# bencebecsy/pta_replicator

Hardware: AMD Instinct MI355X
Metric: realizations/sec, 68 psr x 5000 TOAs GWB+RN+WN (higher is better)
Workload: dtype f64; 1 GPU; BASELINE.json config 3: the 68 pulsars of ng15_dict.json x 5000 synthetic TOAs - HD GWB (gw_log10_A of the dict) + per-pulsar power-law RN (dict values, 30 components) + per-backend EFAC / t2EQUAD / ECORR (dict values), on-chip Philox draws, 1024 realisations per step per GPU; n_toa_total=340000, Nf=3000, npts=600, parallelism=replica-shard x1

## Files before the change

include/pta_replicator_amd.h:

```cpp
#ifndef PTA_REPLICATOR_AMD_H
#define PTA_REPLICATOR_AMD_H

#include <stdint.h>

#ifdef __cplusplus
extern "C" {
#endif

#define PTA_ABI_VERSION 8

#define PTA_OK 0
#define PTA_E_ARG (-1)
#define PTA_E_HIP (-2)
#define PTA_E_NOTPD (-3)

int pta_abi_version(void);
const char *pta_last_error(void);
int pta_device_info(int *cu_count, int *wavefront, char *arch, int arch_len);



int pta_rng_philox_raw(const uint32_t *ctr, const uint32_t *key, int n, uint32_t *out, void *stream);

int pta_rng_fill_normal(uint64_t seed, uint64_t r0, int R, uint32_t stream_id, int npairs, int interleave,
                        double *z0, double *z1, int64_t ld, int rng_fast, void *stream);
int pta_rng_fill_normal_blocks(uint64_t seed, uint64_t r0, int R, uint32_t stream_kind, int n_blocks, const int32_t *blk_n,
                               const int32_t *blk_zoff, int max_n, double *z, int64_t ld, int rng_fast, void *stream);

int pta_rn_basis(const double *t, int N, double t_ref, const double *f, const double *phase, int nmodes,
                 int cos_first, double *Ft, int64_t ldf, void *stream);

int pta_rn_synth(const double *Ft, int64_t ldf, int N, int K, const double *coef, int64_t ld_coef, int R, double *out,
                 int64_t ld_out, int accumulate, void *stream);

int pta_wn(const double *sigma, const double *efac, const double *equad, int N, int tnequad, const double *z1,
           const double *z2, int64_t ld_z, int R, double *out, int64_t ld_out, int accumulate, void *stream);

int pta_quantize_epochs(const double *times_host, int N, double dt, const int64_t *order_host,
                        int32_t *epoch_of_host, int32_t *first_index_host, int *n_epochs);

int pta_dot3_host(const double *x_host, int64_t n, const double *y_host, double *out_host);
int pta_pow_host(const double *x_host, double y, int64_t n, double *out_host);
int pta_legacy_randn(const uint32_t *seeds_host, const int64_t *counts_host, const int64_t *offsets_host, int n_streams,
                     double *out_host, uint32_t *last_key_host, int32_t *last_pos_has_host, double *last_gauss_host, int n_threads);

int pta_ecorr(const int32_t *epoch_of, const double *ecorr_epoch, int N, int E, const double *z, int64_t ld_z, int R,
              double *out, int64_t ld_out, int accumulate, void *stream);


int pta_orf_pair_arguments(const double *locs_host, int P, double *arg_host, uint8_t *same_host);

int pta_orf_hd(const double *locs, int P, double *orf, void *stream);

int pta_orf_basis(const double *locs, const double *zeta_cos, int P, int lmax, double *basis, void *stream);

int pta_orf_combine(const double *basis, const double *clm, int nbasis, int P, double *orf, void *stream);

int pta_potrf_batched(double *A, int n, int B, int32_t *info, void *stream);

#define PTA_POTRF_ZERO_UPPER 1
#define PTA_POTRF_NO_LOOKAHEAD 2
#define PTA_POTRF_NB(k) (((k) & 0xFF) << 8)
#define PTA_POTRF_CHAINS(c) (((c) & 0xF) << 16)
#define PTA_POTRF_VALU 8
#define PTA_POTRF_SUBSTITUTION 4
#define PTA_POTRF_REG_STAGING 32
#define PTA_POTRF_DIAG_AHEAD 128
#define PTA_POTRF_DIAG64 16
#define PTA_POTRF_LOCKSTEP 64
#define PTA_POTRF_EPI1 0x100000
#define PTA_POTRF_LEFT 0x200000
#define PTA_POTRF_LEFT_SPLIT 0x400000
#define PTA_POTRF_SOLVE_ROWS 0x800000
int pta_potrf_batched_ex(double *A, int n, int64_t lda, int64_t strideA, int B, int32_t *info, int flags, void *stream);

int64_t pta_potrf_workspace_doubles(int n, int B, int flags);
int pta_potrf_batched_ws(double *A, int n, int64_t lda, int64_t strideA, int B, int32_t *info, int flags, double *work,
                         int64_t work_doubles, void *stream);

int pta_potrf_warmup(int nchain);

int64_t pta_potrf_ragged_plan_words(int B);
int pta_potrf_ragged_plan(const int32_t *n, const int64_t *off, const int64_t *ld, int B, int flags, int64_t *plan_host,
                          int64_t *work_doubles);
int pta_potrf_ragged(double *A, const int64_t *plan_host, const int64_t *plan_dev, int32_t *info, double *work,
                     int64_t work_doubles, void *stream);



int pta_gwb_twiddle(const double *sqrtC, int Nf, int npts, int i0, double inv_dt, double *T, int64_t ldt, void *stream);

int pta_gwb_idft(const double *w, int64_t ldw, int M, int Nf, const double *T, int64_t ldt, int npts, double *G0,
                 int64_t ldg, int algo, void *stream);

int64_t pta_gwb_twiddle_sym_size(int Nf, int npts, int variant, int64_t *rot_doubles);
int pta_gwb_twiddle_sym(const double *sqrtC, int Nf, int npts, int i0, double inv_dt, double *Tsym, double *rot,
                        int variant, void *stream);
int pta_gwb_idft_rng(uint64_t seed, uint64_t r0, int R, int P, int Nf, const double *Tsym, const double *rot, int npts,
                     double *G0, int64_t ldg, int variant, int rng_fast, void *stream);

int pta_gwb_czt_fits(int Nf, int npts, int i0);
int pta_gwb_czt_setup(const double *sqrtC, int Nf, int npts, int i0, double inv_dt, double *pre, double *FB, double *tw,
                      double *post, void *stream);
int pta_gwb_czt(uint64_t seed, uint64_t r0, const double *w, int64_t ldw, int R, int P, int Nf, int npts, int i0,
                const double *pre, const double *FB, const double *tw, const double *post, double *G0, int64_t ldg,
                int variant, int rng_fast, void *stream);

int pta_gwb_czt_scaled(uint64_t seed, uint64_t r0, const double *w, int64_t ldw, int R, int P, int Nf, int npts, int i0,
                       const double *pre, const double *FB, const double *tw, const double *post, double *G0, int64_t ldg,
                       int variant, int rng_fast, const double *scale, int64_t ld_scale, void *stream);
int pta_gwb_idft_rng_scaled(uint64_t seed, uint64_t r0, int R, int P, int Nf, const double *Tsym, const double *rot, int npts,
                            double *G0, int64_t ldg, int variant, int rng_fast, const double *scale, int64_t ld_scale, void *stream);
int pta_gwb_spectrum_scale(const double *f, const double *hcf0, int Nf, int R, const double *log10_A, const double *gamma, int turnover,
                           double f0, double beta, double power, double *scale, int64_t ld_scale, void *stream);
int pta_gwb_spectrum_scale_user(const int32_t *seg, const double *dx, const double *dxp, const double *hcf0, int Nf, int M, int R,
                                const double *log10_hc, int64_t ld_hc, double *scale, int64_t ld_scale, void *stream);

int pta_gwb_mix(const double *Mchol, int P, const double *G0, int R, int npts, int64_t ldg, double *G, int variant, void *stream);

int pta_gwb_bracket(const double *ut, int npts, const double *toa_s, int N, int32_t *jlo, void *stream);

int pta_gwb_weights(const double *ut, int npts, const double *toa_s, const int32_t *jlo, int N, double *w, void *stream);

int pta_gwb_interp(const double *G, int64_t ldg, int P, int npts, const double *ut, const double *toa_s,
                   const int32_t *psr_of_toa, const int32_t *jlo, int N, int R, double scale, double *out,
                   int64_t ld_out, int accumulate, void *stream);

#define PTA_CGW_NPAR 18
int pta_cgw(const double *mjd, int N, const double *par_host, double *out, int accumulate, void *stream);

#define PTA_CW_NPAR 16
int pta_cw_catalog_workspace(int N, int ncw, int64_t *partial_doubles, int *nchunk);
int pta_cw_catalog(const double *mjd, int N, const double *par, int ncw, int psr_term, int mode, double tref,
                   double *partial_ws, double *out, int accumulate, void *stream);

#define PTA_ENGINE_TILE 256
#define PTA_ENGINE_EPMAX 132
typedef struct {
  int32_t n_toa;
  int32_t n_psr;
  int32_t rn_k;
  int32_t gw_npts;
  int32_t tnequad;
  int32_t n_tiles;
  const int32_t *tile_psr;
  const int32_t *tile_start;
  const int32_t *tile_count;
  const int32_t *tile_ep0;
  const int32_t *tile_epn;
  const int32_t *idx_in_psr;
  const double *Ft;
  int64_t ldf;
  const double *rn_coef;
  const double *gw_G;
  const int32_t *gw_jlo;
  const double *gw_w;
  const double *wn_a;
  const double *wn_b;
  const int32_t *epoch_of;
  const double *ecorr_toa;
  const double *det;
  const double *wn_c;
  int32_t rng_fast;
  int32_t synth_variant;
} pta_engine_plan;

int pta_engine_rn_coef(uint64_t seed, uint64_t r0, int R, int P, int K, const double *amp, double *coef, int rng_fast, void *stream);

int pta_engine_synth(const pta_engine_plan *plan_host, uint64_t seed, uint64_t r0, int R, double *out, int64_t ld_out,
                     void *stream);

typedef struct {
  const double *rn_amp;
  const double *Mchol;
  int32_t gw_nf;
  int32_t gw_i0;
  int32_t use_czt;
  int32_t czt_variant;
  const double *czt_pre, *czt_FB, *czt_tw, *czt_post;
  const double *Tsym, *rot;
  double *ws_coef;
  double *ws_G0;
  double *ws_G;
  int32_t idft_variant;
  int32_t mix_variant;
} pta_engine_tables;

int pta_engine_generate(const pta_engine_plan *plan_host, const pta_engine_tables *tables_host, uint64_t seed, uint64_t r0, int R,
                        double *out, int64_t ld_out, void *stream);

int pta_hyper_uniform(uint64_t seed, uint64_t r0, int R, int n_par, const double *lo, const double *hi, double *out, void *stream);
int pta_hyper_uniform_field(uint64_t seed, uint64_t r0, int R, int n_par, int field, const double *lo, const double *hi, double *out,
                            void *stream);

int pta_engine_rn_coef_hyper(uint64_t seed, uint64_t r0, int R, int P, int K, const double *rn_f, const double *rn_tspan,
                             const double *log10_A, const double *gamma, const double *amp_fixed, double *coef, int rng_fast,
                             void *stream);

typedef struct {
  const double *gw_scale;
  int64_t ld_gw_scale;
  const double *gw_log10_A;
  const double *gw_gamma;
  const double *gw_f;
  const double *gw_hcf0;
  int32_t gw_turnover;
  double gw_f0, gw_beta, gw_power;
  double *ws_scale;
  const double *rn_f;
  const double *rn_tspan;
  const double *rn_log10_A;
  const double *rn_gamma;
} pta_engine_hyper;

int pta_engine_generate_hyper(const pta_engine_plan *plan_host, const pta_engine_tables *tables_host, const pta_engine_hyper *hyper_host,
                              uint64_t seed, uint64_t r0, int R, double *out, int64_t ld_out, void *stream);

int pta_cw_uniform(uint64_t seed, uint64_t r0, int R, int n_par, const double *lo, const double *hi, double *out, void *stream);

#define PTA_CW_ENGINE_NPAR 16
typedef struct {
  int32_t n_psr;
  int32_t mode;
  int32_t psr_term;
  int32_t amp_is_h;
  int32_t has_pdist;
  double tref;
  const double *phat;
  const double *pdist;
  const double *toa_s;
  const double *src;
  int64_t ld_src;
  double *par;
} pta_cw_engine;

int pta_engine_cw_params(const pta_cw_engine *cw_host, int R, void *stream);

int pta_engine_cw_add(const pta_engine_plan *plan_host, const pta_cw_engine *cw_host, int R, double *out, int64_t ld_out, int accumulate,
                      void *stream);

int pta_cw_catalog_uniform(uint64_t seed, uint64_t r0, int R, int S, const double *lo, const double *hi, double *out, void *stream);

#define PTA_CW_CATALOG_NPAR_EVOLVE 16
#define PTA_CW_CATALOG_NPAR_FOLDED 8
typedef struct {
  int32_t n_psr;
  int32_t n_src;
  int32_t mode;
  int32_t psr_term;
  int32_t amp_is_h;
  int32_t has_pdist;
  double tref;
  const double *phat;
  const double *pdist;
  int64_t ld_pdist;
  const double *toa_s;
  const double *src;
  int64_t ld_src;
  const int32_t *count;
  double *par;
} pta_cw_catalog_engine;

int pta_engine_cw_catalog_params(const pta_cw_catalog_engine *cw_host, int R, void *stream);

int pta_engine_cw_catalog_add(const pta_engine_plan *plan_host, const pta_cw_catalog_engine *cw_host, int R, double *out, int64_t ld_out,
                              int accumulate, void *stream);

int pta_td_cov_assemble(const double *Ft, int64_t ldf, int N, int K, const double *phi, const double *sigma2,
                        const int32_t *epoch_of, const double *ecorr2, double *C, int64_t ldc, void *stream);

int pta_td_cov_assemble_all(const double *Ft, int64_t ldf, int K, const double *phi, const double *sigma2,
                            const int32_t *epoch_of, const double *ecorr2, double *Cbase, const int64_t *blk_pos,
                            const int32_t *blk_ld, const int32_t *blk_n, const int32_t *blk_off, int n_blocks, int max_n,
                            void *stream);

int64_t pta_td_cov_walk_items(const int32_t *blk_n_host, int n_blocks, int K, int variant, int32_t *item0_host);
int pta_td_cov_assemble_walk(const double *Ft, int64_t ldf, int K, const double *phi, const double *sigma2,
                             const int32_t *epoch_of, const double *ecorr2, double *Cbase, const int64_t *blk_pos,
                             const int32_t *blk_ld, const int32_t *blk_n, const int32_t *blk_off, int n_blocks,
                             const int32_t *item0, int64_t n_items, const int32_t *epoch_first, int variant, void *stream);

int pta_td_assemble_potrf(const double *Fr, const double *Gr, int kf, const double *sigma2, const int32_t *epoch_of, const double *ecorr2,
                          double *A, int n, int64_t lda, int64_t strideA, int B, int32_t *info, int flags, double *work,
                          int64_t work_doubles, void *stream);

int pta_td_trmm(const double *L, int64_t ldl, int N, const double *z, int64_t ld_z, int R, double *out, int64_t ld_out,
                int accumulate, int algo, void *stream);

#define PTA_TD_STRIP 256
typedef struct {
  const double *Lbase;
  const int64_t *blk_pos;
  const int32_t *blk_ld;
  const int32_t *blk_n;
  const int32_t *blk_off;
  const int32_t *item_blk;
  const int32_t *item_n0;
  int32_t n_blocks;
  int32_t n_items;
  int32_t rows_per_real;
  uint32_t stream_kind;
  int32_t rng_fast;
  int32_t gw_npts;
  const double *gw_G;
  const int32_t *gw_jlo;
  const double *gw_w;
  const double *det;
  const double *z;
  int64_t ld_z;
  const int32_t *blk_zoff;
  const int32_t *item_rows;
} pta_td_plan;

int pta_td_trmm_rng(const pta_td_plan *plan_host, uint64_t seed, uint64_t r0, int M, double *out, int64_t ld_out, void *stream);

int pta_tm_project(const double *Qt, const double *Mt, int64_t ld, int m, const int32_t *psr_off, int P, double *rows, int64_t ld_rows, int R,
                   void *stream);

int pta_os_project(const double *Wt, int64_t ldw, int C, const int32_t *psr_off, int P, const double *rows, int64_t ld_rows, int R, double *Y,
                   int64_t ld_y, void *stream);
int pta_os_pairs(const double *Y, int64_t ld_y, int P, int C, int R, const int32_t *pair_a, const int32_t *pair_b, int n_pairs, const double *wt,
                 int n_orf, double *A2, int64_t ld_a2, const double *den, double *pair_out, int64_t ld_pair, void *stream);

int pta_os_matched_prior(int R, int P, int K_rn, int C, const double *rn_f, const double *rn_tspan, const double *rn_phi, const double *rn_log10_A,
                         const double *rn_gamma, double T, const double *gw_log10_A, const double *gw_gamma, const double *s, double *b,
                         void *stream);
int pta_os_matched_prior_spec(int R, int P, int K_rn, int C, const double *rn_f, const double *rn_tspan, const double *rn_phi,
                              const double *rn_log10_A, const double *rn_gamma, double T, const int32_t *seg, const double *dx, const double *dxp,
                              int M, const double *log10_hc, int64_t ld_hc, const double *s, double *b, void *stream);
int pta_os_matched_solve(const double *A, int P, int K, int C, int R, const double *b, const double *q, int64_t ld_q, int q_block, const double *S,
                         const double *s, double *X, double *Z, void *stream);
int pta_os_matched_pairs(const double *X, const double *Z, int P, int C, int R, const int32_t *pair_a, const int32_t *pair_b, int n_pairs,
                         const double *G, const double *G2, int n_orf, double *A2, int64_t ld_a2, double *sigma, int64_t ld_sigma, double *rho,
                         double *sigma_pair, int64_t ld_pair, void *stream);

int pta_os_pairs_pf(const double *Y, int64_t ld_y, int P, int C, int R, const int32_t *pair_a, const int32_t *pair_b, int n_pairs,
                    const double *G, int n_orf, const double *op, int mode, double *a2, int64_t ld_a2, void *stream);
int pta_os_matched_pairs_pf(const double *X, const double *Z, int P, int C, int R, const int32_t *pair_a, const int32_t *pair_b, int n_pairs,
                            const double *G, const double *G2, int n_orf, int mode, double *a2, int64_t ld_a2, double *sigma,
                            int64_t ld_sigma, double *fisher, int64_t ld_fisher, void *stream);

int pta_lnl_quad(const double *rows, int64_t ld_rows, int R, const int32_t *psr_off, int P, const double *dinv, const int32_t *psr_ep,
                 const int32_t *ep_ptr, const int32_t *ep_idx, const double *ep_g, const double *q, int64_t ld_q, int q_block, int K, int m,
                 const double *Ht, int64_t ldh, double *r0, void *stream);
int pta_lnl_factor(const double *A, int P, int K, int C, int G, const double *b, double *Lt, double *logdet, void *stream);
int pta_lnl_apply(const double *Lt, const double *logdet, const double *b, int P, int K, int C, int G, const double *q, int64_t ld_q, int q_block,
                  int Kt, int R, const double *r0, const double *s, const double *c, double *lnl_pulsar, int64_t ld_g, int64_t ld_a, void *stream);
int pta_lnl_reduce(const double *lnl_pulsar, int64_t ld_g, int64_t ld_a, int P, int G, int R, double *lnl, int64_t ld_lnl, void *stream);

#define PTA_FSTAT_CMAX 4096
#define PTA_FSTAT_PMAX 128
#define PTA_FSTAT_SKY_TILE 64
int pta_fstat_project(const double *Wt, int64_t ldw, int C, const int32_t *psr_off, int P, const double *rows, int64_t ld_rows, int R, double *Q,
                      int64_t ld_q, void *stream);
int pta_fstat_fp(const double *Q, int64_t ld_q, int P, int J, int R, const double *Ginv, double *fp, int64_t ld_fp, void *stream);
int64_t pta_fstat_fe_tiles(int S);
int pta_fstat_fe(const double *Q, int64_t ld_q, int P, int J, int R, const double *phi, int S, const double *Minv, double *fe, int64_t ld_fe,
                 double *fe_max, int64_t ld_max, int32_t *fe_arg, int64_t ld_arg, double *part_val, int32_t *part_arg, void *stream);

int pta_gather_rank0(void *comm, int rank, int world, int dst, const double *local, int64_t total_rows, int64_t n_cols,
                     int64_t ld_local, double *out, int64_t ld_out, void *stream);

int pta_dgemm(int transB, int M, int N, int K, double alpha, const double *A, int64_t lda, int64_t ska,
              const double *B, int64_t ldb, double beta, double *C, int64_t ldc, int lower_only, int batch,
              int64_t strideA, int64_t strideB, int64_t strideC, int algo, void *stream);

int pta_microbench(int kind, int64_t bytes, int iters, int option, double *result_host);

int pta_clock_probe(uint64_t *samples, int max_samples, int us, int period_us, void *stream);

int pta_selftest_mfma_f64(double *max_err_host);

#ifdef __cplusplus
}
#endif
#endif
```

pta_replicator_amd/_lib.py:

```python
import ctypes
import os
from ctypes import POINTER, c_char_p, c_double, c_int, c_int32, c_int64, c_uint32, c_uint64, c_void_p

import torch

_HERE = os.path.dirname(os.path.abspath(__file__))
LIB_PATH = os.environ.get("PTA_REPLICATOR_AMD_LIB") or os.path.join(_HERE, "libpta_replicator_amd.so")


class PtaError(RuntimeError):
    """A call into libpta_replicator_amd.so returned a PTA_E_* code."""


if not os.path.exists(LIB_PATH):
    raise ImportError(
        f"{LIB_PATH} is missing: build the HIP library first (python -m pta_replicator_amd.build, or "
        "__graft_entry__.build()). pta_replicator_amd has no CPU fallback.")

lib = ctypes.CDLL(LIB_PATH)

_P = c_void_p


class EnginePlan(ctypes.Structure):
    _fields_ = [
        ("n_toa", c_int32), ("n_psr", c_int32), ("rn_k", c_int32), ("gw_npts", c_int32), ("tnequad", c_int32),
        ("n_tiles", c_int32),
        ("tile_psr", _P), ("tile_start", _P), ("tile_count", _P), ("tile_ep0", _P), ("tile_epn", _P),
        ("idx_in_psr", _P), ("Ft", _P), ("ldf", c_int64), ("rn_coef", _P), ("gw_G", _P),
        ("gw_jlo", _P), ("gw_w", _P), ("wn_a", _P), ("wn_b", _P), ("epoch_of", _P),
        ("ecorr_toa", _P), ("det", _P), ("wn_c", _P), ("rng_fast", c_int32), ("synth_variant", c_int32),
    ]


class EngineTables(ctypes.Structure):
    _fields_ = [
        ("rn_amp", _P), ("Mchol", _P), ("gw_nf", c_int32), ("gw_i0", c_int32), ("use_czt", c_int32), ("czt_variant", c_int32),
        ("czt_pre", _P), ("czt_FB", _P), ("czt_tw", _P), ("czt_post", _P), ("Tsym", _P), ("rot", _P),
        ("ws_coef", _P), ("ws_G0", _P), ("ws_G", _P), ("idft_variant", c_int32), ("mix_variant", c_int32),
    ]


class TdPlan(ctypes.Structure):
    _fields_ = [
        ("Lbase", _P), ("blk_pos", _P), ("blk_ld", _P), ("blk_n", _P), ("blk_off", _P), ("item_blk", _P), ("item_n0", _P),
        ("n_blocks", c_int32), ("n_items", c_int32), ("rows_per_real", c_int32), ("stream_kind", c_uint32),
        ("rng_fast", c_int32), ("gw_npts", c_int32),
        ("gw_G", _P), ("gw_jlo", _P), ("gw_w", _P), ("det", _P), ("z", _P), ("ld_z", c_int64), ("blk_zoff", _P), ("item_rows", _P),
    ]


class EngineHyper(ctypes.Structure):
    _fields_ = [
        ("gw_scale", _P), ("ld_gw_scale", c_int64), ("gw_log10_A", _P), ("gw_gamma", _P), ("gw_f", _P), ("gw_hcf0", _P),
        ("gw_turnover", c_int32), ("gw_f0", c_double), ("gw_beta", c_double), ("gw_power", c_double), ("ws_scale", _P),
        ("rn_f", _P), ("rn_tspan", _P), ("rn_log10_A", _P), ("rn_gamma", _P),
    ]


class CwEngine(ctypes.Structure):
    _fields_ = [
        ("n_psr", c_int32), ("mode", c_int32), ("psr_term", c_int32), ("amp_is_h", c_int32), ("has_pdist", c_int32), ("tref", c_double),
        ("phat", _P), ("pdist", _P), ("toa_s", _P), ("src", _P), ("ld_src", c_int64), ("par", _P),
    ]


class CwCatalogEngine(ctypes.Structure):
    _fields_ = [
        ("n_psr", c_int32), ("n_src", c_int32), ("mode", c_int32), ("psr_term", c_int32), ("amp_is_h", c_int32), ("has_pdist", c_int32),
        ("tref", c_double), ("phat", _P), ("pdist", _P), ("ld_pdist", c_int64), ("toa_s", _P), ("src", _P), ("ld_src", c_int64),
        ("count", _P), ("par", _P),
    ]


_SIGNATURES = {
    "pta_abi_version": (c_int, []),
    "pta_last_error": (c_char_p, []),
    "pta_device_info": (c_int, [POINTER(c_int), POINTER(c_int), c_char_p, c_int]),
    "pta_rng_philox_raw": (c_int, [_P, _P, c_int, _P, _P]),
    "pta_rng_fill_normal": (c_int, [c_uint64, c_uint64, c_int, c_uint32, c_int, c_int, _P, _P, c_int64, c_int, _P]),
    "pta_rng_fill_normal_blocks": (c_int, [c_uint64, c_uint64, c_int, c_uint32, c_int, _P, _P, c_int, _P, c_int64, c_int, _P]),
    "pta_rn_basis": (c_int, [_P, c_int, c_double, _P, _P, c_int, c_int, _P, c_int64, _P]),
    "pta_rn_synth": (c_int, [_P, c_int64, c_int, c_int, _P, c_int64, c_int, _P, c_int64, c_int, _P]),
    "pta_wn": (c_int, [_P, _P, _P, c_int, c_int, _P, _P, c_int64, c_int, _P, c_int64, c_int, _P]),
    "pta_quantize_epochs": (c_int, [_P, c_int, c_double, _P, _P, _P, POINTER(c_int)]),
    "pta_dot3_host": (c_int, [_P, c_int64, _P, _P]),
    "pta_pow_host": (c_int, [_P, c_double, c_int64, _P]),
    "pta_legacy_randn": (c_int, [_P, _P, _P, c_int, _P, _P, _P, _P, c_int]),
    "pta_ecorr": (c_int, [_P, _P, c_int, c_int, _P, c_int64, c_int, _P, c_int64, c_int, _P]),
    "pta_orf_pair_arguments": (c_int, [_P, c_int, _P, _P]),
    "pta_orf_hd": (c_int, [_P, c_int, _P, _P]),
    "pta_orf_basis": (c_int, [_P, _P, c_int, c_int, _P, _P]),
    "pta_orf_combine": (c_int, [_P, _P, c_int, c_int, _P, _P]),
    "pta_potrf_batched": (c_int, [_P, c_int, c_int, _P, _P]),
    "pta_potrf_batched_ex": (c_int, [_P, c_int, c_int64, c_int64, c_int, _P, c_int, _P]),
    "pta_potrf_workspace_doubles": (c_int64, [c_int, c_int, c_int]),
    "pta_potrf_batched_ws": (c_int, [_P, c_int, c_int64, c_int64, c_int, _P, c_int, _P, c_int64, _P]),
    "pta_potrf_warmup": (c_int, [c_int]),
    "pta_td_assemble_potrf": (c_int, [_P, _P, c_int, _P, _P, _P, _P, c_int, c_int64, c_int64, c_int, _P, c_int, _P, c_int64, _P]),
    "pta_potrf_ragged_plan_words": (c_int64, [c_int]),
    "pta_potrf_ragged_plan": (c_int, [_P, _P, _P, c_int, c_int, _P, POINTER(c_int64)]),
    "pta_potrf_ragged": (c_int, [_P, _P, _P, _P, _P, c_int64, _P]),
    "pta_gwb_twiddle": (c_int, [_P, c_int, c_int, c_int, c_double, _P, c_int64, _P]),
    "pta_gwb_idft": (c_int, [_P, c_int64, c_int, c_int, _P, c_int64, c_int, _P, c_int64, c_int, _P]),
    "pta_gwb_twiddle_sym_size": (c_int64, [c_int, c_int, c_int, POINTER(c_int64)]),
    "pta_gwb_twiddle_sym": (c_int, [_P, c_int, c_int, c_int, c_double, _P, _P, c_int, _P]),
    "pta_gwb_idft_rng": (c_int, [c_uint64, c_uint64, c_int, c_int, c_int, _P, _P, c_int, _P, c_int64, c_int, c_int, _P]),
    "pta_gwb_czt_fits": (c_int, [c_int, c_int, c_int]),
    "pta_gwb_czt_setup": (c_int, [_P, c_int, c_int, c_int, c_double, _P, _P, _P, _P, _P]),
    "pta_gwb_czt": (c_int, [c_uint64, c_uint64, _P, c_int64, c_int, c_int, c_int, c_int, c_int, _P, _P, _P, _P, _P, c_int64, c_int, c_int, _P]),
    "pta_gwb_czt_scaled": (c_int, [c_uint64, c_uint64, _P, c_int64, c_int, c_int, c_int, c_int, c_int, _P, _P, _P, _P, _P, c_int64, c_int, c_int,
                                   _P, c_int64, _P]),
    "pta_gwb_idft_rng_scaled": (c_int, [c_uint64, c_uint64, c_int, c_int, c_int, _P, _P, c_int, _P, c_int64, c_int, c_int, _P, c_int64, _P]),
    "pta_gwb_spectrum_scale": (c_int, [_P, _P, c_int, c_int, _P, _P, c_int, c_double, c_double, c_double, _P, c_int64, _P]),
    "pta_gwb_mix": (c_int, [_P, c_int, _P, c_int, c_int, c_int64, _P, c_int, _P]),
    "pta_gwb_bracket": (c_int, [_P, c_int, _P, c_int, _P, _P]),
    "pta_gwb_weights": (c_int, [_P, c_int, _P, _P, c_int, _P, _P]),
    "pta_gwb_interp": (c_int, [_P, c_int64, c_int, c_int, _P, _P, _P, _P, c_int, c_int, c_double, _P, c_int64, c_int, _P]),
    "pta_cgw": (c_int, [_P, c_int, _P, _P, c_int, _P]),
    "pta_cw_catalog_workspace": (c_int, [c_int, c_int, POINTER(c_int64), POINTER(c_int)]),
    "pta_cw_catalog": (c_int, [_P, c_int, _P, c_int, c_int, c_int, c_double, _P, _P, c_int, _P]),
    "pta_engine_rn_coef": (c_int, [c_uint64, c_uint64, c_int, c_int, c_int, _P, _P, c_int, _P]),
    "pta_engine_generate": (c_int, [POINTER(EnginePlan), POINTER(EngineTables), c_uint64, c_uint64, c_int, _P, c_int64, _P]),
    "pta_hyper_uniform": (c_int, [c_uint64, c_uint64, c_int, c_int, _P, _P, _P, _P]),
    "pta_engine_rn_coef_hyper": (c_int, [c_uint64, c_uint64, c_int, c_int, c_int, _P, _P, _P, _P, _P, _P, c_int, _P]),
    "pta_engine_generate_hyper": (c_int, [POINTER(EnginePlan), POINTER(EngineTables), POINTER(EngineHyper), c_uint64, c_uint64, c_int, _P,
                                          c_int64, _P]),
    "pta_cw_uniform": (c_int, [c_uint64, c_uint64, c_int, c_int, _P, _P, _P, _P]),
    "pta_engine_cw_params": (c_int, [POINTER(CwEngine), c_int, _P]),
    "pta_engine_cw_add": (c_int, [POINTER(EnginePlan), POINTER(CwEngine), c_int, _P, c_int64, c_int, _P]),
    "pta_cw_catalog_uniform": (c_int, [c_uint64, c_uint64, c_int, c_int, _P, _P, _P, _P]),
    "pta_engine_cw_catalog_params": (c_int, [POINTER(CwCatalogEngine), c_int, _P]),
    "pta_engine_cw_catalog_add": (c_int, [POINTER(EnginePlan), POINTER(CwCatalogEngine), c_int, _P, c_int64, c_int, _P]),
    "pta_engine_synth": (c_int, [POINTER(EnginePlan), c_uint64, c_uint64, c_int, _P, c_int64, _P]),
    "pta_td_cov_assemble": (c_int, [_P, c_int64, c_int, c_int, _P, _P, _P, _P, _P, c_int64, _P]),
    "pta_td_cov_assemble_all": (c_int, [_P, c_int64, c_int, _P, _P, _P, _P, _P, _P, _P, _P, _P, c_int, c_int, _P]),
    "pta_td_cov_walk_items": (c_int64, [_P, c_int, c_int, c_int, _P]),
    "pta_td_cov_assemble_walk": (c_int, [_P, c_int64, c_int, _P, _P, _P, _P, _P, _P, _P, _P, _P, c_int, _P, c_int64, _P, c_int, _P]),
    "pta_td_trmm": (c_int, [_P, c_int64, c_int, _P, c_int64, c_int, _P, c_int64, c_int, c_int, _P]),
    "pta_td_trmm_rng": (c_int, [POINTER(TdPlan), c_uint64, c_uint64, c_int, _P, c_int64, _P]),
    "pta_tm_project": (c_int, [_P, _P, c_int64, c_int, _P, c_int, _P, c_int64, c_int, _P]),
    "pta_os_project": (c_int, [_P, c_int64, c_int, _P, c_int, _P, c_int64, c_int, _P, c_int64, _P]),
    "pta_os_pairs": (c_int, [_P, c_int64, c_int, c_int, c_int, _P, _P, c_int, _P, c_int, _P, c_int64, _P, _P, c_int64, _P]),
    "pta_os_matched_prior": (c_int, [c_int, c_int, c_int, c_int, _P, _P, _P, _P, _P, c_double, _P, _P, _P, _P, _P]),
    "pta_os_matched_solve": (c_int, [_P, c_int, c_int, c_int, c_int, _P, _P, c_int64, c_int, _P, _P, _P, _P, _P]),
    "pta_os_matched_pairs": (c_int, [_P, _P, c_int, c_int, c_int, _P, _P, c_int, _P, _P, c_int, _P, c_int64, _P, c_int64, _P, _P, c_int64, _P]),
    "pta_os_pairs_pf": (c_int, [_P, c_int64, c_int, c_int, c_int, _P, _P, c_int, _P, c_int, _P, c_int, _P, c_int64, _P]),
    "pta_os_matched_pairs_pf": (c_int, [_P, _P, c_int, c_int, c_int, _P, _P, c_int, _P, _P, c_int, c_int, _P, c_int64, _P, c_int64, _P, c_int64, _P]),
    "pta_lnl_quad": (c_int, [_P, c_int64, c_int, _P, c_int, _P, _P, _P, _P, _P, _P, c_int64, c_int, c_int, c_int, _P, c_int64, _P, _P]),
    "pta_lnl_factor": (c_int, [_P, c_int, c_int, c_int, c_int, _P, _P, _P, _P]),
    "pta_lnl_apply": (c_int, [_P, _P, _P, c_int, c_int, c_int, c_int, _P, c_int64, c_int, c_int, c_int, _P, _P, _P, _P, c_int64, c_int64, _P]),
    "pta_lnl_reduce": (c_int, [_P, c_int64, c_int64, c_int, c_int, c_int, _P, c_int64, _P]),
    "pta_fstat_project": (c_int, [_P, c_int64, c_int, _P, c_int, _P, c_int64, c_int, _P, c_int64, _P]),
    "pta_fstat_fp": (c_int, [_P, c_int64, c_int, c_int, c_int, _P, _P, c_int64, _P]),
    "pta_fstat_fe_tiles": (c_int64, [c_int]),
    "pta_fstat_fe": (c_int, [_P, c_int64, c_int, c_int, c_int, _P, c_int, _P, _P, c_int64, _P, c_int64, _P, c_int64, _P, _P, _P]),
    "pta_gather_rank0":(c_int, [_P, c_int, c_int, c_int, _P, c_int64, c_int64, c_int64, _P, c_int64, _P]),
    "pta_dgemm": (c_int, [c_int, c_int, c_int, c_int, c_double, _P, c_int64, c_int64, _P, c_int64, c_double, _P, c_int64,
                          c_int, c_int, c_int64, c_int64, c_int64, c_int, _P]),
    "pta_microbench": (c_int, [c_int, c_int64, c_int, c_int, POINTER(c_double)]),
    "pta_clock_probe": (c_int, [_P, c_int, c_int, c_int, _P]),
    "pta_selftest_mfma_f64": (c_int, [POINTER(c_double)]),
    "pta_gwb_spectrum_scale_user": (c_int, [_P, _P, _P, _P, c_int, c_int, c_int, _P, c_int64, _P, c_int64, _P]),
    "pta_hyper_uniform_field": (c_int, [c_uint64, c_uint64, c_int, c_int, c_int, _P, _P, _P, _P]),
    "pta_os_matched_prior_spec": (c_int, [c_int, c_int, c_int, c_int, _P, _P, _P, _P, _P, c_double, _P, _P, _P, c_int, _P, c_int64, _P, _P, _P]),
}

ENGINE_TILE = 256
ENGINE_EPMAX = 132
CW_ENGINE_NPAR = 16
CW_CATALOG_NPAR = (16, 8, 8)
OS_CMAX = 64
OSM_KMAX = 128
LNL_KMAX = 128
LNL_MMAX = 16
FSTAT_CMAX = 4096
FSTAT_PMAX = 128
TD_STRIP = 256
POTRF_ZERO_UPPER, POTRF_NO_LOOKAHEAD, POTRF_SUBSTITUTION, POTRF_VALU, POTRF_REG_STAGING, POTRF_LOCKSTEP, POTRF_DIAG_AHEAD, POTRF_DIAG64 = 1, 2, 4, 8, 32, 64, 128, 16
POTRF_EPI1 = 0x100000
POTRF_LEFT, POTRF_LEFT_SPLIT, POTRF_SOLVE_ROWS = 0x200000, 0x400000, 0x800000


def POTRF_CHAINS(c):
    return (int(c) & 0xF) << 16


def POTRF_NB(k):
    return (int(k) & 0xFF) << 8

EXPORTS = tuple(_SIGNATURES)

for _name, (_res, _args) in _SIGNATURES.items():
    _fn = getattr(lib, _name)
    _fn.restype = _res
    _fn.argtypes = _args

if lib.pta_abi_version() != 8:
    raise ImportError("libpta_replicator_amd.so has an unexpected ABI version: rebuild it")


def last_error():
    msg = lib.pta_last_error()
    return msg.decode() if msg else ""


def check(rc, what=""):
    if rc != 0:
        raise PtaError(f"{what or 'libpta_replicator_amd'} failed (code {rc}): {last_error()}")


def call(name, *args):
    check(getattr(lib, name)(*args), name)
```

pta_replicator_amd/csrc/pta_czt_kernels.hip:

```cpp
#include "pta_common.h"
#include "pta_fft.h"

__global__ __launch_bounds__(PTA_FFT_THREADS) void k_czt_setup(const double *__restrict__ sqrtC, int Nf, int npts, int i0,
                                                               double inv_dt, double *__restrict__ pre,
                                                               double *__restrict__ FB, double *__restrict__ tw,
                                                               double *__restrict__ post) {
  __shared__ double re[PTA_FFT_PLANE], im[PTA_FFT_PLANE];
  const int tid = threadIdx.x;
  const int Kf = Nf - 2;
  const int64_t n = 2 * (int64_t)Nf - 2;
  for (int m = tid; m < PTA_FFT_N; m += PTA_FFT_THREADS) {
    double s, c;
    sincospi((double)(2 * m) / (double)PTA_FFT_N, &s, &c);
    tw[2 * m] = c;
    tw[2 * m + 1] = -s;
    double pr = 0.0, pi_ = 0.0;
    if (m < Kf) {
      int64_t k = m + 1, q = (k * k) % (2 * n);
      sincospi((double)q / (double)n, &s, &c);
      pr = sqrtC[k] * c;
      pi_ = sqrtC[k] * s;
    }
    pre[2 * m] = pr;
    pre[2 * m + 1] = pi_;
    int64_t u = m;
    bool used = (m <= i0 + npts - 2);
    if (!used && m >= PTA_FFT_N - (Kf - i0)) {
      u = (int64_t)m - PTA_FFT_N;
      used = true;
    }
    double br = 0.0, bi = 0.0;
    if (used) {
      int64_t q = (u * u) % (2 * n);
      sincospi((double)q / (double)n, &s, &c);
      br = c;
      bi = -s;
    }
    re[PTA_FFT_PHYS(m)] = br;
    im[PTA_FFT_PHYS(m)] = bi;
  }
  for (int jj = tid; jj < npts; jj += PTA_FFT_THREADS) {
    int64_t j = i0 + jj, q = (j * j) % (2 * n);
    double s, c;
    sincospi((double)q / (double)n, &s, &c);
    double amp = 2.0 * inv_dt / (double)n;
    post[2 * jj] = amp * c;
    post[2 * jj + 1] = amp * s;
  }
  __threadfence_block();
  __syncthreads();
  pta_fft_pass<false, 9>(re, im, tw, tid);
  __syncthreads();
  pta_fft_pass<false, 6>(re, im, tw, tid);
  __syncthreads();
  pta_fft_pass<false, 3>(re, im, tw, tid);
  __syncthreads();
  pta_fft_pass<false, 0>(re, im, tw, tid);
  __syncthreads();
  for (int m = tid; m < PTA_FFT_N; m += PTA_FFT_THREADS) {
    const int slot = (m & 7) * (PTA_FFT_N / 8) + (m >> 3);
    FB[2 * slot] = re[PTA_FFT_PHYS(m)] * (1.0 / PTA_FFT_N);
    FB[2 * slot + 1] = im[PTA_FFT_PHYS(m)] * (1.0 / PTA_FFT_N);
  }
}

static bool czt_fits(int Nf, int npts, int i0) { return Nf >= 3 && (Nf - 2) + npts - 2 < PTA_FFT_N && i0 >= 1 && (Nf - 2) <= PTA_FFT_N; }

extern "C" int pta_gwb_czt_setup(const double *sqrtC, int Nf, int npts, int i0, double inv_dt, double *pre, double *FB, double *tw,
                                 double *post, void *stream) {
  PTA_REQUIRE(sqrtC && pre && FB && tw && post, PTA_E_ARG, "pta_gwb_czt_setup: NULL argument");
  PTA_REQUIRE(czt_fits(Nf, npts, i0), PTA_E_ARG, "pta_gwb_czt_setup: Nf=%d npts=%d does not fit one 4096-point convolution", Nf, npts);
  hipLaunchKernelGGL(k_czt_setup, dim3(1), dim3(PTA_FFT_THREADS), 0, pta_stream(stream), sqrtC, Nf, npts, i0, inv_dt, pre, FB, tw, post);
  PTA_LAUNCH_CHECK();
  return PTA_OK;
}

extern "C" int pta_gwb_czt_fits(int Nf, int npts, int i0) { return czt_fits(Nf, npts, i0) ? 1 : 0; }

#define PTA_CZT_FUSE_DEFAULT (15 + 16 + 64)
static int czt_last2(int npts, int i0) { return i0 - 2 + npts < 1024 ? 1 : 0; }

template <bool RNG, bool FAST, int FUSE, bool SCALED>
__global__ __launch_bounds__(PTA_FFT_THREADS, 4) void k_gwb_czt(uint64_t seed, uint64_t r0, const double *__restrict__ w, int64_t ldw,
                                                                  int M, int P, int Nf, int npts, int i0,
                                                                  const double *__restrict__ pre, const double *__restrict__ FB,
                                                                  const double *__restrict__ tw, const double *__restrict__ post,
                                                                  double *__restrict__ G0, int64_t ldg,
                                                                  const double *__restrict__ scale, int64_t ld_scale, int last2) {
  static_assert(!(FUSE & 16) || (FUSE & 6) == 6, "bit 4 carries the twiddles from the register-fed first butterfly to the storing last one");
  static_assert(!(FUSE & 32) || (FUSE & 8), "bit 5 tabulates the squared twiddles of bit 3");
  static_assert(!(FUSE & 64) || (FUSE & 2), "bit 6 prunes the storing last butterfly");
  __shared__ double re[PTA_FFT_PLANE], im[PTA_FFT_PLANE];
  constexpr bool TAB = (FUSE & 32) != 0;
  __shared__ pta_cplx tw8[7][8];
  __shared__ pta_cplx tw64[3][64];
  const int tid = threadIdx.x;
  const int row = blockIdx.x;
  const int Kf = Nf - 2;
  if (TAB) {
    if (tid < 64) {
      pta_cplx tq[8];
      pta_fft_twiddles<6, 1>(tw, tid, tq);
      tw64[0][tid] = tq[1];
      tw64[1][tid] = tq[2];
      tw64[2][tid] = tq[4];
    } else if (tid < 72) {
      pta_cplx tq[8];
      pta_fft_twiddles<3, 1>(tw, tid - 64, tq);
#pragma unroll
      for (int q = 1; q < 8; ++q) tw8[q - 1][tid - 64] = tq[q];
    }
  }
  if (RNG) {
    pta_rng_stage_tables();
    __syncthreads();
  }
  const uint64_t real = r0 + (uint64_t)(row / P);
  const uint32_t strm = pta_stream_id(PTA_STREAM_GWB, (uint32_t)(row % P));
  const pta_cplx *pre2 = reinterpret_cast<const pta_cplx *>(pre);
  constexpr int TW = (FUSE & 8) ? 1 : 3;
  const double *twi = tw;
  asm volatile("" : "+s"(twi));
  pta_cplx tv[8];
  if (FUSE & 4) {
    int b, o;
    pta_cplx v[8];
    pta_fft_map<9>(tid, b, o);
    pta_fft_twiddles<9, TW>(tw, o, tv);
#pragma unroll
    for (int q = 0; q < 8; ++q) {
      const int t = o + 512 * q;
      v[q] = {0.0, 0.0};
      if (t < Kf) {
        double wr, wi;
        if (RNG) {
          pta_normal_pair(seed, real, strm, (uint32_t)(t + 1), wr, wi, FAST ? 1 : 0);
        } else {
          wr = w[(int64_t)row * ldw + 2 * (t + 1)];
          wi = w[(int64_t)row * ldw + 2 * (t + 1) + 1];
        }
        if (SCALED) {
          const double sc = scale[(int64_t)(row / P) * ld_scale + t + 1];
          wr *= sc;
          wi *= sc;
        }
        const pta_cplx pc = pre2[t];
        v[q] = {wr * pc.re - wi * pc.im, wr * pc.im + wi * pc.re};
      }
    }
    pta_fft_core<false, 9>(v, tv);
    pta_fft_store<9>(re, im, b, o, v);
  } else {
#pragma unroll 1
    for (int i = 0; i < PTA_FFT_N / PTA_FFT_THREADS; ++i) {
      const int t = tid + PTA_FFT_THREADS * i;
      double ar = 0.0, ai = 0.0;
      if (t < Kf) {
        double wr, wi;
        if (RNG) {
          pta_normal_pair(seed, real, strm, (uint32_t)(t + 1), wr, wi, FAST ? 1 : 0);
        } else {
          wr = w[(int64_t)row * ldw + 2 * (t + 1)];
          wi = w[(int64_t)row * ldw + 2 * (t + 1) + 1];
        }
        if (SCALED) {
          const double sc = scale[(int64_t)(row / P) * ld_scale + t + 1];
          wr *= sc;
          wi *= sc;
        }
        const pta_cplx pc = pre2[t];
        ar = wr * pc.re - wi * pc.im;
        ai = wr * pc.im + wi * pc.re;
      }
      re[PTA_FFT_PHYS(t)] = ar;
      im[PTA_FFT_PHYS(t)] = ai;
    }
    __syncthreads();
    pta_fft_pass<false, 9, TW>(re, im, tw, tid);
  }
  __syncthreads();
  auto tab64 = [&](pta_cplx *wq) {
    const int o = 8 * (tid >> 6) + (tid & 7);
    wq[1] = tw64[0][o];
    wq[2] = tw64[1][o];
    wq[4] = tw64[2][o];
    pta_fft_twiddle_products(wq);
  };
  auto tab8 = [&](pta_cplx *wq) {
#pragma unroll
    for (int q = 1; q < 8; ++q) wq[q] = tw8[q - 1][tid & 7];
  };
  if (TAB) {
    pta_cplx wq[8];
    tab64(wq);
    pta_fft_pass_w<false, 6>(re, im, tid, wq);
    __syncthreads();
    tab8(wq);
    pta_fft_pass_w<false, 3>(re, im, tid, wq);
  } else {
    pta_fft_pass<false, 6, TW>(re, im, tw, tid);
    __syncthreads();
    pta_fft_pass<false, 3, TW>(re, im, tw, tid);
  }
  __syncthreads();
  if (FUSE & 1) {
    int b, o;
    pta_cplx v[8], fv[8];
    pta_fft_map<0>(tid, b, o);
    const pta_cplx *fb = reinterpret_cast<const pta_cplx *>(FB) + b;
#pragma unroll
    for (int q = 0; q < 8; ++q) fv[q] = fb[q * (PTA_FFT_N / 8)];
    pta_fft_load<0>(re, im, b, o, v);
    pta_dft8<false>(v);
#pragma unroll
    for (int q = 0; q < 8; ++q) v[q] = pta_cmul(v[q], fv[q]);
    pta_dft8<true>(v);
    pta_fft_store<0>(re, im, b, o, v);
  } else {
    pta_fft_pass<false, 0, TW>(re, im, tw, tid);
    __syncthreads();
#pragma unroll 4
    for (int i = 0; i < PTA_FFT_N / PTA_FFT_THREADS; ++i) {
      const int t = tid + PTA_FFT_THREADS * i;
      const int p = PTA_FFT_PHYS(t);
      const int slot = (t & 7) * (PTA_FFT_N / 8) + (t >> 3);
      const double xr = re[p], xi = im[p], fr = FB[2 * slot], fi = FB[2 * slot + 1];
      re[p] = xr * fr - xi * fi;
      im[p] = xr * fi + xi * fr;
    }
    __syncthreads();
    pta_fft_pass<true, 0, TW>(re, im, twi, tid);
  }
  __syncthreads();
  if (TAB) {
    pta_cplx wq[8];
    tab8(wq);
    pta_fft_pass_w<true, 3>(re, im, tid, wq);
    __syncthreads();
    tab64(wq);
    pta_fft_pass_w<true, 6>(re, im, tid, wq);
  } else {
    pta_fft_pass<true, 3, TW>(re, im, twi, tid);
    __syncthreads();
    pta_fft_pass<true, 6, TW>(re, im, twi, tid);
  }
  __syncthreads();
  const pta_cplx *post2 = reinterpret_cast<const pta_cplx *>(post);
  if (FUSE & 2) {
    int b, o;
    pta_cplx v[8];
    pta_fft_map<9>(tid, b, o);
    if (!(FUSE & 16)) pta_fft_twiddles<9, TW>(twi, o, tv);
    pta_fft_load<9>(re, im, b, o, v);
    auto put = [&](int q) {
      const int jj = o + 512 * q - (i0 - 1);
      if (jj >= 0 && jj < npts) {
        const pta_cplx pp = post2[jj];
        G0[(int64_t)row * ldg + jj] = v[q].re * pp.re - v[q].im * pp.im;
      }
    };
    if ((FUSE & 64) && last2) {
      pta_fft_core_inv_out01<9>(v, tv);
      put(0);
      put(1);
    } else {
      pta_fft_core<true, 9>(v, tv);
#pragma unroll
      for (int q = 0; q < 8; ++q) put(q);
    }
  } else {
    pta_fft_pass<true, 9, TW>(re, im, twi, tid);
    __syncthreads();
    for (int jj = tid; jj < npts; jj += PTA_FFT_THREADS) {
      const int p = PTA_FFT_PHYS(i0 - 1 + jj);
      G0[(int64_t)row * ldg + jj] = re[p] * post2[jj].re - im[p] * post2[jj].im;
    }
  }
}

extern "C" int pta_gwb_czt(uint64_t seed, uint64_t r0, const double *w, int64_t ldw, int R, int P, int Nf, int npts, int i0,
                           const double *pre, const double *FB, const double *tw, const double *post, double *G0, int64_t ldg,
                           int variant, int rng_fast, void *stream) {
  PTA_REQUIRE(pre && FB && tw && post && G0, PTA_E_ARG, "pta_gwb_czt: NULL argument");
  PTA_REQUIRE(R > 0 && P > 0 && P < (1 << 24) && npts > 0 && ldg >= npts, PTA_E_ARG, "pta_gwb_czt: R=%d P=%d npts=%d", R, P, npts);
  PTA_REQUIRE(czt_fits(Nf, npts, i0), PTA_E_ARG, "pta_gwb_czt: Nf=%d npts=%d does not fit one 4096-point convolution", Nf, npts);
  PTA_REQUIRE(!w || ldw == 0 || ldw >= 2 * (int64_t)Nf, PTA_E_ARG, "pta_gwb_czt: ldw too small");
  int64_t M64 = (int64_t)R * P;
  PTA_REQUIRE(M64 < (1LL << 31), PTA_E_ARG, "pta_gwb_czt: R*P too large");
  const int M = (int)M64;
  const int fastm = rng_fast ? 1 : 0;
  const int fuse = variant == 0 ? PTA_CZT_FUSE_DEFAULT : (variant == 1 ? 0 : variant - 10);
  const int last2 = czt_last2(npts, i0);
#define PTA_CZT_X(RNGV, FASTV, FUSEV)                                                                                                  \
  hipLaunchKernelGGL((k_gwb_czt<RNGV, FASTV, FUSEV, false>), dim3(M), dim3(PTA_FFT_THREADS), 0, pta_stream(stream), seed, r0, w, ldw, \
                     M, P, Nf, npts, i0, pre, FB, tw, post, G0, ldg, nullptr, 0, last2)
#define PTA_CZT_XF(FUSEV)              \
  if (w)                               \
    PTA_CZT_X(false, false, FUSEV);    \
  else if (fastm)                      \
    PTA_CZT_X(true, true, FUSEV);      \
  else                                 \
    PTA_CZT_X(true, false, FUSEV)
  switch (fuse) {
    case PTA_CZT_FUSE_DEFAULT: PTA_CZT_XF(PTA_CZT_FUSE_DEFAULT); break;
    case 15 + 16 + 32 + 64: PTA_CZT_XF(15 + 16 + 32 + 64); break;
    case 15: PTA_CZT_XF(15); break;
    case 15 + 16: PTA_CZT_XF(15 + 16); break;
    case 15 + 32: PTA_CZT_XF(15 + 32); break;
    case 15 + 64: PTA_CZT_XF(15 + 64); break;
    case 0: PTA_CZT_XF(0); break;
    case 1: PTA_CZT_XF(1); break;
    case 3: PTA_CZT_XF(3); break;
    case 7: PTA_CZT_XF(7); break;
    case 8: PTA_CZT_XF(8); break;
    default: pta_set_error("pta_gwb_czt: unknown variant %d", variant); return PTA_E_ARG;
  }
#undef PTA_CZT_XF
#undef PTA_CZT_X
  PTA_LAUNCH_CHECK();
  return PTA_OK;
}

extern "C" int pta_gwb_czt_scaled(uint64_t seed, uint64_t r0, const double *w, int64_t ldw, int R, int P, int Nf, int npts, int i0,
                                  const double *pre, const double *FB, const double *tw, const double *post, double *G0, int64_t ldg,
                                  int variant, int rng_fast, const double *scale, int64_t ld_scale, void *stream) {
  PTA_REQUIRE(pre && FB && tw && post && G0 && scale, PTA_E_ARG, "pta_gwb_czt_scaled: NULL argument");
  PTA_REQUIRE(!w, PTA_E_ARG, "pta_gwb_czt_scaled: draws are generated on chip (w must be NULL)");
  (void)ldw;
  PTA_REQUIRE(R > 0 && P > 0 && P < (1 << 24) && npts > 0 && ldg >= npts, PTA_E_ARG, "pta_gwb_czt_scaled: R=%d P=%d npts=%d", R, P,
              npts);
  PTA_REQUIRE(czt_fits(Nf, npts, i0), PTA_E_ARG, "pta_gwb_czt_scaled: Nf=%d npts=%d does not fit one 4096-point convolution", Nf,
              npts);
  PTA_REQUIRE(ld_scale >= Nf - 1, PTA_E_ARG, "pta_gwb_czt_scaled: ld_scale=%lld < Nf - 1", (long long)ld_scale);
  int64_t M64 = (int64_t)R * P;
  PTA_REQUIRE(M64 < (1LL << 31), PTA_E_ARG, "pta_gwb_czt_scaled: R*P too large");
  const int M = (int)M64;
  PTA_REQUIRE(variant == 0 || variant == 1, PTA_E_ARG, "pta_gwb_czt_scaled: variant %d (0 or 1)", variant);
#define PTA_CZT_S(FASTV, FUSEV)                                                                                                     \
  hipLaunchKernelGGL((k_gwb_czt<true, FASTV, FUSEV, true>), dim3(M), dim3(PTA_FFT_THREADS), 0, pta_stream(stream), seed, r0, nullptr, \
                     0, M, P, Nf, npts, i0, pre, FB, tw, post, G0, ldg, scale, ld_scale, czt_last2(npts, i0))
  if (variant == 0) {
    if (rng_fast)
      PTA_CZT_S(true, PTA_CZT_FUSE_DEFAULT);
    else
      PTA_CZT_S(false, PTA_CZT_FUSE_DEFAULT);
  } else {
    if (rng_fast)
      PTA_CZT_S(true, 0);
    else
      PTA_CZT_S(false, 0);
  }
#undef PTA_CZT_S
  PTA_LAUNCH_CHECK();
  return PTA_OK;
}
```

pta_replicator_amd/csrc/pta_engine_kernels.hip:

```cpp
#include "pta_common.h"
#include "pta_rng.h"
#include "pta_mfma.h"

__global__ void k_engine_rn_coef(uint64_t seed, uint64_t r0, int R, int P, int K, const double *__restrict__ amp,
                                 double *__restrict__ coef, int fast) {
  pta_rng_stage_tables();
  __syncthreads();
  int idx = blockIdx.x * blockDim.x + threadIdx.x;
  int hp = K / 2;
  int total = R * P * hp;
  if (idx >= total) return;
  int p = idx % hp, ra = idx / hp;
  int a = ra % P, r = ra / P;
  double z0, z1;
  pta_normal_pair(seed, r0 + (uint64_t)r, pta_stream_id(PTA_STREAM_RN, (uint32_t)a), (uint32_t)p, z0, z1, fast);
  int64_t o = (int64_t)ra * K + 2 * p;
  coef[o] = amp[(int64_t)a * K + 2 * p] * z0;
  coef[o + 1] = amp[(int64_t)a * K + 2 * p + 1] * z1;
}

extern "C" int pta_engine_rn_coef(uint64_t seed, uint64_t r0, int R, int P, int K, const double *amp, double *coef, int rng_fast,
                                  void *stream) {
  PTA_REQUIRE(amp && coef, PTA_E_ARG, "pta_engine_rn_coef: NULL argument");
  PTA_REQUIRE(R > 0 && P > 0 && K > 0 && (K % 2) == 0, PTA_E_ARG, "pta_engine_rn_coef: R=%d P=%d K=%d (K must be even)", R, P, K);
  int64_t total = (int64_t)R * P * (K / 2);
  PTA_REQUIRE(total < (1LL << 31), PTA_E_ARG, "pta_engine_rn_coef: problem too large");
  hipLaunchKernelGGL(k_engine_rn_coef, dim3(pta_cdiv(total, 256)), dim3(256), 0, pta_stream(stream), seed, r0, R, P, K, amp, coef, rng_fast ? 1 : 0);
  PTA_LAUNCH_CHECK();
  return PTA_OK;
}

#define ENG_RB 8

template <int MINW>
__global__ __launch_bounds__(PTA_ENGINE_TILE, MINW) void k_engine_synth(pta_engine_plan pl, uint64_t seed, uint64_t r0, int R,
                                                                  double *__restrict__ out, int64_t ld_out, int fast) {
  __shared__ double zec[ENG_RB][2 * PTA_ENGINE_EPMAX];
  pta_rng_stage_tables();
  __syncthreads();
  const int tile = blockIdx.y;
  const int rb = blockIdx.x * ENG_RB;
  const int a = pl.tile_psr[tile];
  const int start = pl.tile_start[tile];
  const int count = pl.tile_count[tile];
  const int t = threadIdx.x;
  const int P = pl.n_psr;
  const bool has_ec = pl.ecorr_toa != nullptr;
  const int epn = has_ec ? pl.tile_epn[tile] : 0;
  const int ep0 = has_ec ? pl.tile_ep0[tile] : 0;
  if (epn > 0) {
    const uint32_t strm = pta_stream_id(PTA_STREAM_ECORR, (uint32_t)a);
    for (int idx = t; idx < epn * ENG_RB; idx += PTA_ENGINE_TILE) {
      int q = idx / epn, p = idx - q * epn;
      double z0, z1;
      pta_normal_pair(seed, r0 + (uint64_t)(rb + q), strm, (uint32_t)(ep0 + p), z0, z1, fast);
      zec[q][2 * p] = z0;
      zec[q][2 * p + 1] = z1;
    }
    __syncthreads();
  }
  if (t >= count) return;
  const int i = start + t;
  double v[ENG_RB];
#pragma unroll
  for (int q = 0; q < ENG_RB; ++q) v[q] = 0.0;

  if (pl.rn_k > 0) {
    const int K = pl.rn_k;
    const double *__restrict__ Fcol = pl.Ft + i;
    const double *__restrict__ cf = pl.rn_coef + ((int64_t)rb * P + a) * K;
    const int64_t rstride = (int64_t)P * K;
    for (int c = 0; c < K; ++c) {
      double fv = Fcol[(int64_t)c * pl.ldf];
#pragma unroll
      for (int q = 0; q < ENG_RB; ++q) {
        int qq = (rb + q < R) ? q : 0;
        v[q] = fma(fv, cf[qq * rstride + c], v[q]);
      }
    }
  }
  if (pl.gw_npts > 0) {
    const int j = pl.gw_jlo[i];
    const double wgt = pl.gw_w[i];
    const double *__restrict__ gbase = pl.gw_G + ((int64_t)rb * P + a) * pl.gw_npts;
    const int64_t rstride = (int64_t)P * pl.gw_npts;
#pragma unroll
    for (int q = 0; q < ENG_RB; ++q) {
      int qq = (rb + q < R) ? q : 0;
      const double *g = gbase + qq * rstride;
      v[q] = v[q] + ((g[j + 1] - g[j]) * wgt + g[j]);
    }
  }
  if (pl.wn_a) {
    const double wa = pl.wn_a[i], wb = pl.wn_b[i];
    const uint32_t strm = pta_stream_id(PTA_STREAM_WN, (uint32_t)a);
    const uint32_t pair = (uint32_t)pl.idx_in_psr[i];
#pragma unroll
    for (int q = 0; q < ENG_RB; ++q) {
      double z1, z2;
      pta_normal_pair(seed, r0 + (uint64_t)(rb + q), strm, pair, z1, z2, fast);
      v[q] = v[q] + (wa * z1 + wb * z2);
    }
  }
  if (has_ec) {
    const double ec = pl.ecorr_toa[i];
    const int e = pl.epoch_of[i];
    if (epn > 0) {
      const int o = e - 2 * ep0;
#pragma unroll
      for (int q = 0; q < ENG_RB; ++q) v[q] = v[q] + ec * zec[q][o];
    } else if (ec != 0.0) {
      const uint32_t strm = pta_stream_id(PTA_STREAM_ECORR, (uint32_t)a);
#pragma unroll
      for (int q = 0; q < ENG_RB; ++q) v[q] = v[q] + ec * pta_normal_single(seed, r0 + (uint64_t)(rb + q), strm, (uint32_t)e, fast);
    }
  }
  const double det = pl.det ? pl.det[i] : 0.0;
#pragma unroll
  for (int q = 0; q < ENG_RB; ++q)
    if (rb + q < R) out[(int64_t)(rb + q) * ld_out + i] = v[q] + det;
}

typedef double pta_f64x2_a8 __attribute__((ext_vector_type(2), aligned(8)));
#define ENG_MR 16
#define ENG_ZPITCH (2 * PTA_ENGINE_EPMAX + 8)

template <bool FAST, bool SINGLE, bool RNIDX, bool ALL>
__global__ __launch_bounds__(PTA_ENGINE_TILE, SINGLE ? 3 : 4) void k_engine_synth_mfma(pta_engine_plan pl, uint64_t seed, uint64_t r0, int R,
                                                                                     double *__restrict__ out, int64_t ld_out, int xcd_aware) {
  constexpr int fast = FAST ? 1 : 0;
  __shared__ double zec[ENG_MR][ENG_ZPITCH];
  const int nrg = (R + ENG_MR - 1) / ENG_MR;
  const int64_t total = (int64_t)nrg * pl.n_tiles, chunk = (total + 7) >> 3;
  const int64_t item = xcd_aware ? (int64_t)(blockIdx.x & 7) * chunk + (blockIdx.x >> 3) : (int64_t)blockIdx.x;
  if (item >= total) return;
  pta_rng_stage_tables();
  __syncthreads();
  const int t = threadIdx.x, l = t & 63, wv = t >> 6;
  const int P = pl.n_psr;
  const bool has_ec = ALL || pl.ecorr_toa != nullptr;
  constexpr bool wn_single = SINGLE;
  const int col = l & 15, quad = l >> 4;
  const int tbase = wv * 64 + col;
  constexpr bool WIDE = RNIDX && !SINGLE;
  const int t2 = wv * 64 + 2 * col;
  auto toa = [&](int j) { return WIDE ? t2 + 32 * (j >> 1) + (j & 1) : tbase + 16 * j; };
  const int tile = (int)(item / nrg);
  const int rb = (int)(item - (int64_t)tile * nrg) * ENG_MR;
  const int a = pl.tile_psr[tile];
  const int start = pl.tile_start[tile];
  const int count = pl.tile_count[tile];
  const int epn = has_ec ? pl.tile_epn[tile] : 0;
  const int ep0 = has_ec ? pl.tile_ep0[tile] : 0;
  if (epn > 0) {
    const uint32_t strm = pta_stream_id(PTA_STREAM_ECORR, (uint32_t)a);
    if (WIDE) {
      const int q = t >> 4;
      for (int p = t & 15; p < epn; p += PTA_ENGINE_TILE / ENG_MR) {
        double z0, z1;
        pta_normal_pair(seed, r0 + (uint64_t)(rb + q), strm, (uint32_t)(ep0 + p), z0, z1, fast);
        zec[q][2 * p] = z0;
        zec[q][2 * p + 1] = z1;
      }
    } else {
      for (int idx = t; idx < epn * ENG_MR; idx += PTA_ENGINE_TILE) {
        int q = idx / epn, p = idx - q * epn;
        double z0, z1;
        pta_normal_pair(seed, r0 + (uint64_t)(rb + q), strm, (uint32_t)(ep0 + p), z0, z1, fast);
        zec[q][2 * p] = z0;
        zec[q][2 * p + 1] = z1;
      }
    }
    __syncthreads();
  }
  if (WIDE && wv * 64 >= count) return;
  int rq[4];
#pragma unroll
  for (int g = 0; g < 4; ++g) rq[g] = min(quad + 4 * g, R - 1 - rb);
  int jl4[4];
#pragma unroll
  for (int j = 0; j < 4; ++j) jl4[j] = pl.gw_npts > 0 ? pl.gw_jlo[start + min(toa(j), count - 1)] : 0;
  pta_f64x4 acc[4];
#pragma unroll
  for (int j = 0; j < 4; ++j) acc[j] = pta_f64x4{0.0, 0.0, 0.0, 0.0};
  const bool has_gw = ALL || pl.gw_npts > 0, has_wn = ALL || pl.wn_a != nullptr || wn_single;
  if (pl.rn_k > 0) {
    const int K = pl.rn_k;
    const int ra = min(rb + col, R - 1);
    const double *__restrict__ cf = pl.rn_coef + ((int64_t)ra * P + a) * K;
    const double *__restrict__ Fb = pl.Ft + start;
    int tcl[4];
#pragma unroll
    for (int j = 0; j < 4; ++j) tcl[j] = min(toa(j), count - 1);
    auto ld = [&](int k0, double &av, double (&bv)[4]) {
      const int k = k0 + quad, kc = min(k, K - 1);
      const double a_ld = cf[kc];
      av = (k < K) ? a_ld : 0.0;
      const double *__restrict__ Fk = Fb + (int64_t)kc * pl.ldf;
#pragma unroll
      for (int j = 0; j < 4; ++j) bv[j] = Fk[tcl[j]];
    };
    auto mm = [&](double av, const double (&bv)[4]) {
#pragma unroll
      for (int j = 0; j < 4; ++j) acc[j] = pta_mfma_f64(av, bv[j], acc[j]);
    };
    auto run = [&](auto &&ldx) {
      double a0, a1, a2, b0[4], b1[4], b2[4];
      ldx(0, a0, b0);
      ldx(4, a1, b1);
      for (int k0 = 0; k0 < K; k0 += 12) {
        ldx(k0 + 8, a2, b2);
        mm(a0, b0);
        ldx(k0 + 12, a0, b0);
        mm(a1, b1);
        ldx(k0 + 16, a1, b1);
        mm(a2, b2);
      }
    };
    if (RNIDX) {
      const int klast = (K - 1) & ~3;
      const char *__restrict__ Fbytes = reinterpret_cast<const char *>(Fb);
      const char *__restrict__ cbytes = reinterpret_cast<const char *>(pl.rn_coef);
      const uint32_t ldfb = (uint32_t)pl.ldf * 8u;
      uint32_t offF[4];
#pragma unroll
      for (int j = 0; j < 4; ++j) offF[j] = (uint32_t)quad * ldfb + (uint32_t)tcl[j] * 8u;
      const uint32_t offC = (uint32_t)(((int64_t)ra * P + a) * K + quad) * 8u;
      const int kq = K - quad;
      auto ldu = [&](int k0, auto rowF, auto rowC, double &av, double (&bv)[4]) {
        const double a_ld = *reinterpret_cast<const double *>(cbytes + (uint32_t)(offC + rowC));
        av = (k0 < kq) ? a_ld : 0.0;
#pragma unroll
        for (int j = 0; j < 4; ++j) bv[j] = *reinterpret_cast<const double *>(Fbytes + (uint32_t)(offF[j] + rowF));
      };
      auto lduw = [&](int k0, auto rowF, auto rowC, double &av, double (&bv)[4]) {
        const double a_ld = *reinterpret_cast<const double *>(cbytes + (uint32_t)(offC + rowC));
        av = (k0 < kq) ? a_ld : 0.0;
        const char *__restrict__ src = Fbytes + (uint32_t)(offF[0] + rowF);
        const pta_f64x2_a8 lo = *reinterpret_cast<const pta_f64x2_a8 *>(src), hi = *reinterpret_cast<const pta_f64x2_a8 *>(src + 256);
        bv[0] = lo.x, bv[1] = lo.y, bv[2] = hi.x, bv[3] = hi.y;
      };
      auto rows = [&](auto &&ldx) {
        if ((K & 3) == 0) {
          run([&](int k0, double &av, double (&bv)[4]) {
            const uint32_t kg = (uint32_t)min(k0, klast);
            ldx(k0, kg * ldfb, kg * 8u, av, bv);
          });
        } else {
          const uint32_t dq = (uint32_t)(quad - min(quad, K - 1 - klast));
          run([&](int k0, double &av, double (&bv)[4]) {
            const uint32_t kg = (uint32_t)min(k0, klast);
            const uint32_t back = k0 >= klast ? dq : 0u;
            ldx(k0, kg * ldfb - back * ldfb, kg * 8u - back * 8u, av, bv);
          });
        }
      };
      if (WIDE && count == PTA_ENGINE_TILE) rows(lduw);
      else rows(ldu);
    } else {
      run(ld);
    }
  }
  const uint32_t strm_wn = pta_stream_id(PTA_STREAM_WN, (uint32_t)a);
  const uint32_t strm_ec = pta_stream_id(PTA_STREAM_ECORR, (uint32_t)a);
  const bool wn_share = wn_single && count == PTA_ENGINE_TILE;
  double zs[4] = {0.0, 0.0, 0.0, 0.0};
  double pend[4] = {0.0, 0.0, 0.0, 0.0};
  int pend_i = 0;
  auto store_half = [&](int j0) {
    if (count == PTA_ENGINE_TILE) {
#pragma unroll
      for (int g = 0; g < 4; ++g)
        *reinterpret_cast<pta_f64x2_a8 *>(out + (int64_t)(rb + rq[g]) * ld_out + (start + toa(j0))) = pta_f64x2_a8{acc[j0][g], acc[j0 + 1][g]};
    } else {
#pragma unroll
      for (int g = 0; g < 4; ++g) {
        out[(int64_t)(rb + rq[g]) * ld_out + (start + min(toa(j0), count - 1))] = acc[j0][g];
        out[(int64_t)(rb + rq[g]) * ld_out + (start + min(toa(j0 + 1), count - 1))] = acc[j0 + 1][g];
      }
    }
  };
#pragma unroll
  for (int j = 0; j < 4; ++j) {
    const int i = start + min(toa(j), count - 1);
    const double wgt = has_gw ? pl.gw_w[i] : 0.0;
    pta_f64x2_a8 y[4];
    const int64_t jlo = jl4[j];
    if (has_gw) {
#pragma unroll
      for (int g = 0; g < 4; ++g)
        y[g] = *reinterpret_cast<const pta_f64x2_a8 *>(pl.gw_G + ((int64_t)(rb + rq[g]) * P + a) * pl.gw_npts + jlo);
    }
    const double wa = has_wn ? (wn_single ? pl.wn_c[i] : pl.wn_a[i]) : 0.0, wb = (has_wn && !wn_single) ? pl.wn_b[i] : 0.0;
    const uint32_t pair = (uint32_t)pl.idx_in_psr[i];
    const double ec = has_ec ? pl.ecorr_toa[i] : 0.0;
    const int e = has_ec ? pl.epoch_of[i] : 0;
    const double det = pl.det ? pl.det[i] : 0.0;
    if (!WIDE && j > 0) {
#pragma unroll
      for (int g = 0; g < 4; ++g) out[(int64_t)(rb + rq[g]) * ld_out + pend_i] = pend[g];
    }
    if (WIDE && j == 2) store_half(0);
    double v[4];
#pragma unroll
    for (int g = 0; g < 4; ++g) v[g] = acc[j][g];
    if (has_gw) {
#pragma unroll
      for (int g = 0; g < 4; ++g) v[g] = v[g] + ((y[g].y - y[g].x) * wgt + y[g].x);
    }
    if (has_wn && !wn_single) {
#pragma unroll
      for (int g = 0; g < 4; ++g) {
        double z1, z2;
        pta_normal_pair(seed, r0 + (uint64_t)(rb + rq[g]), strm_wn, pair, z1, z2, fast);
        v[g] = v[g] + (wa * z1 + wb * z2);
      }
    } else if (wn_single) {
      const uint32_t pid = pair & ~16u;
      const bool br = (pair & 16u) != 0;
      const bool fresh = (j & 1) == 0 || !wn_share;
      if (fresh) {
#pragma unroll
        for (int g = 0; g < 4; ++g) {
          double z0, z1;
          pta_normal_pair(seed, r0 + (uint64_t)(rb + rq[g]), strm_wn, pid, z0, z1, fast);
          v[g] = v[g] + wa * (br ? z1 : z0);
          zs[g] = br ? z0 : z1;
        }
      } else {
#pragma unroll
        for (int g = 0; g < 4; ++g) v[g] = v[g] + wa * zs[g];
      }
    }
    if (has_ec) {
      if (epn > 0) {
        const int o = e - 2 * ep0;
#pragma unroll
        for (int g = 0; g < 4; ++g) v[g] = v[g] + ec * zec[rq[g]][o];
      }
#ifndef PTA_ISA_TABLE_MAIN_PATH_ONLY
      else if (ec != 0.0) {
#pragma unroll
        for (int g = 0; g < 4; ++g) v[g] = v[g] + ec * pta_normal_single(seed, r0 + (uint64_t)(rb + rq[g]), strm_ec, (uint32_t)e, fast);
      }
#endif
    }
    if (WIDE) {
#pragma unroll
      for (int g = 0; g < 4; ++g) acc[j][g] = v[g] + det;
    } else {
#pragma unroll
      for (int g = 0; g < 4; ++g) pend[g] = v[g] + det;
      pend_i = i;
    }
  }
  if (WIDE) {
    store_half(2);
  } else {
#pragma unroll
    for (int g = 0; g < 4; ++g) out[(int64_t)(rb + rq[g]) * ld_out + pend_i] = pend[g];
  }
}

typedef void (*pta_synth_fn)(pta_engine_plan, uint64_t, uint64_t, int, double *, int64_t, int);
static pta_synth_fn synth_kernel(bool rng_fast, bool single, bool rnidx, bool all) {
#define PTA_SYNTH_COPIES(F, S)                                                                     \
  {{k_engine_synth_mfma<F, S, false, false>, k_engine_synth_mfma<F, S, false, true>},             \
   {k_engine_synth_mfma<F, S, true, false>, k_engine_synth_mfma<F, S, true, true>}}
  static const pta_synth_fn kern[2][2][2][2] = {{PTA_SYNTH_COPIES(false, false), PTA_SYNTH_COPIES(false, true)},
                                                {PTA_SYNTH_COPIES(true, false), PTA_SYNTH_COPIES(true, true)}};
#undef PTA_SYNTH_COPIES
  return kern[rng_fast][single][rnidx][all];
}

extern "C" int pta_engine_synth(const pta_engine_plan *plan_host, uint64_t seed, uint64_t r0, int R, double *out, int64_t ld_out,
                                void *stream) {
  PTA_REQUIRE(plan_host && out, PTA_E_ARG, "pta_engine_synth: NULL argument");
  const pta_engine_plan &p = *plan_host;
  PTA_REQUIRE(p.n_toa > 0 && p.n_psr > 0 && R > 0 && ld_out >= p.n_toa, PTA_E_ARG, "pta_engine_synth: n_toa=%d n_psr=%d R=%d", p.n_toa,
              p.n_psr, R);
  PTA_REQUIRE(p.n_tiles > 0 && p.tile_psr && p.tile_start && p.tile_count && p.tile_ep0 && p.tile_epn && p.idx_in_psr, PTA_E_ARG,
              "pta_engine_synth: tile table / idx_in_psr missing");
  PTA_REQUIRE(p.rn_k == 0 || (p.Ft && p.rn_coef && p.ldf >= p.n_toa), PTA_E_ARG, "pta_engine_synth: red-noise inputs missing");
  PTA_REQUIRE(p.gw_npts == 0 || (p.gw_G && p.gw_jlo && p.gw_w && p.gw_npts >= 2), PTA_E_ARG,
              "pta_engine_synth: GWB inputs missing");
  PTA_REQUIRE(!p.wn_a || p.wn_b, PTA_E_ARG, "pta_engine_synth: wn_b missing");
  PTA_REQUIRE(!p.wn_c || !p.wn_a, PTA_E_ARG, "pta_engine_synth: wn_c (single-deviate white noise) replaces wn_a / wn_b - pass one or the other");
  PTA_REQUIRE(!p.ecorr_toa || p.epoch_of, PTA_E_ARG, "pta_engine_synth: epoch_of missing");
  const int variant = p.synth_variant;
  const bool copies = variant == 16 || variant == 32 || variant == 48 || variant == 64;
  PTA_REQUIRE(variant == 0 || variant == 1 || variant == 2 || variant == 6 || copies || (variant >= 100 && variant <= 164), PTA_E_ARG,
              "pta_engine_synth: synth_variant %d does not exist (0, 1, 2, 6, 16, 32, 48, 64, 100 .. 164)", variant);
  if (variant != 6) {
    const int xcd = variant == 1 ? 0 : 1;
    const unsigned pad = variant >= 100 ? (unsigned)(variant - 100) * 1024u : 0u;
    const int64_t total = (int64_t)pta_cdiv(R, ENG_MR) * p.n_tiles, nwg = ((total + 7) >> 3) << 3;
    PTA_REQUIRE(nwg < (1LL << 31), PTA_E_ARG, "pta_engine_synth: %lld workgroups exceed one launch", (long long)nwg);
    const bool noidx = variant == 2 || (copies && ((variant - 16) & 16));
    const bool rnidx = !noidx && p.rn_k > 0 && p.ldf < (1LL << 28) && ((int64_t)p.rn_k * p.ldf + PTA_ENGINE_TILE) * 8 + 24 < (1LL << 32) &&
                       (int64_t)R * p.n_psr * p.rn_k * 8 < (1LL << 32);
    const bool generic = variant == 2 || (copies && ((variant - 16) & 32));
    const bool all = !generic && p.gw_npts > 0 && (p.wn_a || p.wn_c) && p.ecorr_toa;
    hipLaunchKernelGGL(synth_kernel(p.rng_fast != 0, p.wn_c != nullptr, rnidx, all), dim3((unsigned)nwg), dim3(PTA_ENGINE_TILE), pad,
                       pta_stream(stream), p, seed, r0, R, out, ld_out, xcd);
    PTA_LAUNCH_CHECK();
    return PTA_OK;
  }
  PTA_REQUIRE(!p.wn_c, PTA_E_ARG, "pta_engine_synth: the single-deviate white noise exists in the MFMA kernel only");
  PTA_REQUIRE(p.n_tiles <= 65535, PTA_E_ARG, "pta_engine_synth: %d tiles exceed the 2-D launch of the all-VALU kernel", p.n_tiles);
  hipLaunchKernelGGL(k_engine_synth<6>, dim3(pta_cdiv(R, ENG_RB), p.n_tiles), dim3(PTA_ENGINE_TILE), 0, pta_stream(stream), p, seed, r0, R,
                     out, ld_out, p.rng_fast ? 1 : 0);
  PTA_LAUNCH_CHECK();
  return PTA_OK;
}

extern "C" int pta_gwb_czt(uint64_t seed, uint64_t r0, const double *w, int64_t ldw, int R, int P, int Nf, int npts, int i0,
                           const double *pre, const double *FB, const double *tw, const double *post, double *G0, int64_t ldg,
                           int variant, int rng_fast, void *stream);
extern "C" int pta_gwb_idft_rng(uint64_t seed, uint64_t r0, int R, int P, int Nf, const double *Tsym, const double *rot, int npts,
                                double *G0, int64_t ldg, int variant, int rng_fast, void *stream);
extern "C" int pta_gwb_mix(const double *Mchol, int P, const double *G0, int R, int npts, int64_t ldg, double *G, int variant,
                           void *stream);

static int engine_generate(const char *fn, const pta_engine_plan *plan_host, const pta_engine_tables *tables_host,
                           const pta_engine_hyper *hyper, uint64_t seed, uint64_t r0, int R, double *out, int64_t ld_out, void *stream) {
  PTA_REQUIRE(plan_host && tables_host && out, PTA_E_ARG, "%s: NULL argument", fn);
  const pta_engine_hyper fixed{};
  const pta_engine_hyper &h = hyper ? *hyper : fixed;
  pta_engine_plan p = *plan_host;
  const pta_engine_tables &tb = *tables_host;
  int rc;
  if (p.rn_k > 0) {
    PTA_REQUIRE(tb.rn_amp && tb.ws_coef, PTA_E_ARG, "%s: red-noise amplitudes / workspace missing", fn);
    if (h.rn_log10_A) {
      PTA_REQUIRE(h.rn_gamma && h.rn_f && h.rn_tspan, PTA_E_ARG, "%s: rn_gamma / rn_f / rn_tspan missing", fn);
      rc = pta_engine_rn_coef_hyper(seed, r0, R, p.n_psr, p.rn_k, h.rn_f, h.rn_tspan, h.rn_log10_A, h.rn_gamma, tb.rn_amp, tb.ws_coef,
                                    p.rng_fast, stream);
    } else {
      rc = pta_engine_rn_coef(seed, r0, R, p.n_psr, p.rn_k, tb.rn_amp, tb.ws_coef, p.rng_fast, stream);
    }
    if (rc != PTA_OK) return rc;
    p.rn_coef = tb.ws_coef;
  }
  if (p.gw_npts > 0) {
    PTA_REQUIRE(tb.Mchol && tb.ws_G0 && tb.ws_G, PTA_E_ARG, "%s: GWB factor / workspace missing", fn);
    const double *scale = h.gw_scale;
    if (!scale && h.gw_log10_A) {
      PTA_REQUIRE(h.gw_gamma && h.gw_f && h.gw_hcf0 && h.ws_scale, PTA_E_ARG, "%s: gw_gamma / gw_f / gw_hcf0 / ws_scale missing", fn);
      rc = pta_gwb_spectrum_scale(h.gw_f, h.gw_hcf0, tb.gw_nf, R, h.gw_log10_A, h.gw_gamma, h.gw_turnover, h.gw_f0, h.gw_beta,
                                  h.gw_power, h.ws_scale, h.ld_gw_scale, stream);
      if (rc != PTA_OK) return rc;
      scale = h.ws_scale;
    }
    if (tb.use_czt) {
      PTA_REQUIRE(tb.czt_pre && tb.czt_FB && tb.czt_tw && tb.czt_post, PTA_E_ARG, "%s: chirp-z tables missing", fn);
      rc = scale ? pta_gwb_czt_scaled(seed, r0, nullptr, 0, R, p.n_psr, tb.gw_nf, p.gw_npts, tb.gw_i0, tb.czt_pre, tb.czt_FB, tb.czt_tw,
                                      tb.czt_post, tb.ws_G0, p.gw_npts, tb.czt_variant, p.rng_fast, scale, h.ld_gw_scale, stream)
                 : pta_gwb_czt(seed, r0, nullptr, 0, R, p.n_psr, tb.gw_nf, p.gw_npts, tb.gw_i0, tb.czt_pre, tb.czt_FB, tb.czt_tw,
                               tb.czt_post, tb.ws_G0, p.gw_npts, tb.czt_variant, p.rng_fast, stream);
    } else {
      PTA_REQUIRE(tb.Tsym && tb.rot, PTA_E_ARG, "%s: DFT-GEMM tables missing", fn);
      rc = scale ? pta_gwb_idft_rng_scaled(seed, r0, R, p.n_psr, tb.gw_nf, tb.Tsym, tb.rot, p.gw_npts, tb.ws_G0, p.gw_npts, tb.idft_variant,
                                           p.rng_fast, scale, h.ld_gw_scale, stream)
                 : pta_gwb_idft_rng(seed, r0, R, p.n_psr, tb.gw_nf, tb.Tsym, tb.rot, p.gw_npts, tb.ws_G0, p.gw_npts, tb.idft_variant,
                                    p.rng_fast, stream);
    }
    if (rc != PTA_OK) return rc;
    rc = pta_gwb_mix(tb.Mchol, p.n_psr, tb.ws_G0, R, p.gw_npts, p.gw_npts, tb.ws_G, tb.mix_variant, stream);
    if (rc != PTA_OK) return rc;
    p.gw_G = tb.ws_G;
  }
  return pta_engine_synth(&p, seed, r0, R, out, ld_out, stream);
}

extern "C" int pta_engine_generate(const pta_engine_plan *plan_host, const pta_engine_tables *tables_host, uint64_t seed, uint64_t r0,
                                   int R, double *out, int64_t ld_out, void *stream) {
  return engine_generate("pta_engine_generate", plan_host, tables_host, nullptr, seed, r0, R, out, ld_out, stream);
}

extern "C" int pta_engine_generate_hyper(const pta_engine_plan *plan_host, const pta_engine_tables *tables_host,
                                         const pta_engine_hyper *hyper_host, uint64_t seed, uint64_t r0, int R, double *out,
                                         int64_t ld_out, void *stream) {
  PTA_REQUIRE(hyper_host, PTA_E_ARG, "pta_engine_generate_hyper: NULL argument");
  return engine_generate("pta_engine_generate_hyper", plan_host, tables_host, hyper_host, seed, r0, R, out, ld_out, stream);
}
```

pta_replicator_amd/csrc/pta_gwb_kernels.hip:

```cpp
#include "pta_common.h"
#include "pta_mfma.h"
#include "pta_rng.h"


__global__ void k_gwb_twiddle(const double *__restrict__ sqrtC, int Nf, int npts, int i0, double inv_dt,
                              double *__restrict__ T, int64_t ldt) {
  int jj = blockIdx.x * blockDim.x + threadIdx.x;
  int kq = blockIdx.y;
  if (jj >= ldt) return;
  const int Kf = Nf - 2;
  double c = 0.0, s = 0.0;
  if (jj < npts) {
    const int64_t n = 2 * (int64_t)Nf - 2;
    int64_t m = ((int64_t)(i0 + jj) * (int64_t)(kq + 1)) % n;
    double sn, cs;
    sincospi((double)(2 * m) / (double)n, &sn, &cs);
    double amp = 2.0 * inv_dt / (double)n * sqrtC[kq + 1];
    c = amp * cs;
    s = -(amp * sn);
  }
  T[(int64_t)kq * ldt + jj] = c;
  T[((int64_t)Kf + kq) * ldt + jj] = s;
}

extern "C" int pta_gwb_twiddle(const double *sqrtC, int Nf, int npts, int i0, double inv_dt, double *T, int64_t ldt,
                               void *stream) {
  PTA_REQUIRE(sqrtC && T, PTA_E_ARG, "pta_gwb_twiddle: NULL argument");
  PTA_REQUIRE(Nf >= 3 && Nf - 2 <= 65535 && npts > 0 && ldt >= npts && i0 >= 0, PTA_E_ARG, "pta_gwb_twiddle: Nf=%d npts=%d ldt=%lld", Nf,
              npts, (long long)ldt);
  hipLaunchKernelGGL(k_gwb_twiddle, dim3(pta_cdiv(ldt, 128), Nf - 2), dim3(128), 0, pta_stream(stream), sqrtC, Nf, npts, i0,
                     inv_dt, T, ldt);
  PTA_LAUNCH_CHECK();
  return PTA_OK;
}

extern "C" int pta_gwb_idft(const double *w, int64_t ldw, int M, int Nf, const double *T, int64_t ldt, int npts, double *G0,
                            int64_t ldg, int algo, void *stream) {
  PTA_REQUIRE(w && T && G0, PTA_E_ARG, "pta_gwb_idft: NULL argument");
  PTA_REQUIRE(M > 0 && Nf >= 3 && npts > 0 && ldw >= 2 * (int64_t)Nf && ldt >= npts && ldg >= npts, PTA_E_ARG,
              "pta_gwb_idft: M=%d Nf=%d npts=%d", M, Nf, npts);
  const int Kf = Nf - 2;
  hipStream_t s = pta_stream(stream);
  for (int m0 = 0; m0 < M; m0 += 32768) {
    int mc = (M - m0 < 32768) ? (M - m0) : 32768;
    const double *wr = w + (int64_t)m0 * ldw;
    double *g = G0 + (int64_t)m0 * ldg;
    int rc = pta_dgemm_launch(0, mc, npts, Kf, 1.0, wr + 2, ldw, 2, T, ldt, 0.0, g, ldg, 0, 1, 0, 0, 0, algo, s);
    if (rc != PTA_OK) return rc;
    rc = pta_dgemm_launch(0, mc, npts, Kf, 1.0, wr + 3, ldw, 2, T + (int64_t)Kf * ldt, ldt, 1.0, g, ldg, 0, 1, 0, 0, 0, algo, s);
    if (rc != PTA_OK) return rc;
  }
  return PTA_OK;
}

template <int NT>
struct pta_sym_cfg {
  static constexpr int COLS = NT * 16;
  static constexpr int PITCH = (NT % 2) ? COLS : COLS + 16;
  static constexpr int SLAB = 8 * PITCH;
  static constexpr int NLD = (SLAB / 2 + 255) / 256;
  static constexpr int SLAB_PAD = NLD * 512;
};

template <int NT>
__global__ void k_gwb_twiddle_sym(const double *__restrict__ sqrtC, int Nf, int npts, int i0, double inv_dt,
                                  double *__restrict__ Tsym, double *__restrict__ rot) {
  using C = pta_sym_cfg<NT>;
  const int Kf = Nf - 2, nstep = (Kf + 3) >> 2;
  const int half = (npts + 1) >> 1;
  const int col = blockIdx.x * blockDim.x + threadIdx.x;
  const int kq = blockIdx.y;
  const int chunk = blockIdx.z;
  if (col >= C::PITCH) return;
  const int64_t n = 2 * (int64_t)Nf - 2;
  const int p = chunk * C::COLS + col;
  double c = 0.0, s = 0.0;
  if (kq < Kf && col < C::COLS && p < half) {
    int64_t twoj = (npts & 1) ? 2 * (int64_t)p : 2 * (int64_t)p + 1;
    int64_t m2 = (twoj * (int64_t)(kq + 1)) % (2 * n);
    double sn, cs;
    sincospi((double)m2 / (double)n, &sn, &cs);
    double amp = 2.0 * inv_dt / (double)n * sqrtC[kq + 1];
    c = amp * cs;
    s = amp * sn;
  }
  const int ks = kq >> 2, kk = kq & 3;
  double *slab = Tsym + ((int64_t)chunk * nstep + ks) * C::SLAB_PAD;
  slab[(0 * 4 + kk) * C::PITCH + col] = c;
  slab[(1 * 4 + kk) * C::PITCH + col] = s;
  if (chunk == 0 && col == 0) {
    double sn = 0.0, cs = 0.0;
    if (kq < Kf) {
      int64_t m2 = ((2 * (int64_t)i0 + npts - 1) * (int64_t)(kq + 1)) % (2 * n);
      sincospi((double)m2 / (double)n, &sn, &cs);
    }
    rot[2 * kq] = cs;
    rot[2 * kq + 1] = sn;
  }
}

template <int NT, int MINW, bool SCALED>
__global__ __launch_bounds__(256, MINW) void k_gwb_idft_sym_rng(uint64_t seed, uint64_t r0, int M, int P, int Nf,
                                                                const double *__restrict__ Tsym,
                                                                const double *__restrict__ rot, int npts,
                                                                double *__restrict__ G0, int64_t ldg, int fast,
                                                                const double *__restrict__ scale, int64_t ld_scale) {
  using C = pta_sym_cfg<NT>;
  extern __shared__ __attribute__((aligned(16))) double lds[];
  const int t = threadIdx.x, l = t & 63, wv = t >> 6;
  const int Kf = Nf - 2, nstep = (Kf + 3) >> 2;
  const int chunk = blockIdx.y;
  const int m = blockIdx.x * 64 + wv * 16 + (l & 15);
  const int mr = min(m, M - 1);
  const uint64_t real = r0 + (uint64_t)(mr / P);
  const uint32_t strm = pta_stream_id(PTA_STREAM_GWB, (uint32_t)(mr % P));
  pta_f64x4 accE[NT], accO[NT];
#pragma unroll
  for (int i = 0; i < NT; ++i) {
    accE[i] = pta_f64x4{0.0, 0.0, 0.0, 0.0};
    accO[i] = pta_f64x4{0.0, 0.0, 0.0, 0.0};
  }
  const double2 *src = reinterpret_cast<const double2 *>(Tsym + (int64_t)chunk * nstep * C::SLAB_PAD) + t;
  double2 *lds2 = reinterpret_cast<double2 *>(lds) + t;
  double2 regs[C::NLD];
#pragma unroll
  for (int q = 0; q < C::NLD; ++q) lds2[q * 256] = src[q * 256];
  pta_rng_stage_tables();
  __syncthreads();
  const int kk = l >> 4;
  for (int ks = 0; ks < nstep; ++ks) {
    const double *cur = lds + (ks & 1) * C::SLAB_PAD;
    double2 *nxt = lds2 + ((ks + 1) & 1) * (C::SLAB_PAD / 2);
    const int ksn = min(ks + 1, nstep - 1);
#pragma unroll
    for (int q = 0; q < C::NLD; ++q) regs[q] = src[(int64_t)ksn * (C::SLAB_PAD / 2) + q * 256];
    double re, im;
    pta_normal_pair(seed, real, strm, (uint32_t)(ks * 4 + kk + 1), re, im, fast);
    if (SCALED) {
      const double sc = scale[(int64_t)(mr / P) * ld_scale + min(ks * 4 + kk + 1, Kf)];
      re *= sc;
      im *= sc;
    }
    const double2 cs = reinterpret_cast<const double2 *>(rot)[ks * 4 + kk];
    const double ar = re * cs.x - im * cs.y;
    const double br = re * cs.y + im * cs.x;
    const double *bc = cur + kk * C::PITCH + (l & 15);
    const double *bs = bc + 4 * C::PITCH;
#pragma unroll
    for (int i = 0; i < NT; ++i) accE[i] = pta_mfma_f64(ar, bc[i * 16], accE[i]);
#pragma unroll
    for (int i = 0; i < NT; ++i) accO[i] = pta_mfma_f64(br, bs[i * 16], accO[i]);
#pragma unroll
    for (int q = 0; q < C::NLD; ++q) nxt[q * 256] = regs[q];
    __syncthreads();
  }
  const int half = (npts + 1) >> 1;
  const int hi0 = npts >> 1;
  const int lo0 = (npts & 1) ? hi0 : hi0 - 1;
#pragma unroll
  for (int i = 0; i < NT; ++i) {
#pragma unroll
    for (int r = 0; r < 4; ++r) {
      int row = blockIdx.x * 64 + wv * 16 + pta_mfma_row(l, r);
      int p = chunk * C::COLS + i * 16 + pta_mfma_col(l);
      if (row < M && p < half) {
        double e = accE[i][r], o = accO[i][r];
        G0[(int64_t)row * ldg + hi0 + p] = e - o;
        G0[(int64_t)row * ldg + lo0 - p] = e + o;
      }
    }
  }
}

static int sym_nt(int variant) { return variant == 1 ? 10 : (variant == 2 ? 7 : 19); }
static int sym_pitch(int nt) { return (nt % 2) ? nt * 16 : nt * 16 + 16; }
static int sym_slab_pad(int nt) { return ((8 * sym_pitch(nt) / 2 + 255) / 256) * 512; }

extern "C" int64_t pta_gwb_twiddle_sym_size(int Nf, int npts, int variant, int64_t *rot_doubles) {
  const int nt = sym_nt(variant);
  const int nstep = (Nf - 2 + 3) >> 2;
  const int half = (npts + 1) >> 1;
  const int nchunk = (half + nt * 16 - 1) / (nt * 16);
  if (rot_doubles) *rot_doubles = (int64_t)nstep * 8;
  return (int64_t)nchunk * nstep * sym_slab_pad(nt);
}

extern "C" int pta_gwb_twiddle_sym(const double *sqrtC, int Nf, int npts, int i0, double inv_dt, double *Tsym, double *rot,
                                   int variant, void *stream) {
  PTA_REQUIRE(sqrtC && Tsym && rot, PTA_E_ARG, "pta_gwb_twiddle_sym: NULL argument");
  PTA_REQUIRE(Nf >= 3 && npts > 0 && i0 >= 0, PTA_E_ARG, "pta_gwb_twiddle_sym: Nf=%d npts=%d", Nf, npts);
  const int nt = sym_nt(variant);
  const int nstep = (Nf - 2 + 3) >> 2;
  const int half = (npts + 1) >> 1;
  const int nchunk = (half + nt * 16 - 1) / (nt * 16);
  PTA_REQUIRE(nstep * 4 <= 65535 && nchunk <= 65535, PTA_E_ARG, "pta_gwb_twiddle_sym: problem too large");
  dim3 g(pta_cdiv(sym_pitch(nt), 64), nstep * 4, nchunk);
  if (nt == 19)
    hipLaunchKernelGGL(k_gwb_twiddle_sym<19>, g, dim3(64), 0, pta_stream(stream), sqrtC, Nf, npts, i0, inv_dt, Tsym, rot);
  else if (nt == 10)
    hipLaunchKernelGGL(k_gwb_twiddle_sym<10>, g, dim3(64), 0, pta_stream(stream), sqrtC, Nf, npts, i0, inv_dt, Tsym, rot);
  else
    hipLaunchKernelGGL(k_gwb_twiddle_sym<7>, g, dim3(64), 0, pta_stream(stream), sqrtC, Nf, npts, i0, inv_dt, Tsym, rot);
  PTA_LAUNCH_CHECK();
  return PTA_OK;
}

static int idft_rng_launch(uint64_t seed, uint64_t r0, int R, int P, int Nf, const double *Tsym, const double *rot, int npts, double *G0,
                           int64_t ldg, int variant, int rng_fast, const double *scale, int64_t ld_scale, void *stream) {
  const int M = R * P;
  const int nt = sym_nt(variant);
  rng_fast = rng_fast ? 1 : 0;
  const int half = (npts + 1) >> 1;
  const int nchunk = (half + nt * 16 - 1) / (nt * 16);
  const size_t shmem = 2 * (size_t)sym_slab_pad(nt) * sizeof(double);
  dim3 g(pta_cdiv(M, 64), nchunk);
#define PTA_IDFT_X(NTV, MINWV, SCV)                                                                                                     \
  do {                                                                                                                                 \
    auto kern = k_gwb_idft_sym_rng<NTV, MINWV, SCV>;                                                                                  \
    PTA_HIP(hipFuncSetAttribute((const void *)kern, hipFuncAttributeMaxDynamicSharedMemorySize, (int)shmem));                          \
    hipLaunchKernelGGL(kern, g, dim3(256), shmem, pta_stream(stream), seed, r0, M, P, Nf, Tsym, rot, npts, G0, ldg, rng_fast, scale, \
                       ld_scale);                                                                                                      \
  } while (0)
  if (scale) {
    if (nt == 19)
      PTA_IDFT_X(19, 1, true);
    else if (nt == 10)
      PTA_IDFT_X(10, 2, true);
    else
      PTA_IDFT_X(7, 2, true);
  } else {
    if (nt == 19)
      PTA_IDFT_X(19, 1, false);
    else if (nt == 10)
      PTA_IDFT_X(10, 2, false);
    else
      PTA_IDFT_X(7, 2, false);
  }
#undef PTA_IDFT_X
  PTA_LAUNCH_CHECK();
  return PTA_OK;
}

extern "C" int pta_gwb_idft_rng(uint64_t seed, uint64_t r0, int R, int P, int Nf, const double *Tsym, const double *rot,
                                int npts, double *G0, int64_t ldg, int variant, int rng_fast, void *stream) {
  PTA_REQUIRE(Tsym && rot && G0, PTA_E_ARG, "pta_gwb_idft_rng: NULL argument");
  PTA_REQUIRE(R > 0 && P > 0 && P < (1 << 24) && Nf >= 3 && npts > 0 && ldg >= npts, PTA_E_ARG,
              "pta_gwb_idft_rng: R=%d P=%d Nf=%d npts=%d", R, P, Nf, npts);
  int64_t M64 = (int64_t)R * P;
  PTA_REQUIRE(M64 < (1LL << 31), PTA_E_ARG, "pta_gwb_idft_rng: R*P too large");
  return idft_rng_launch(seed, r0, R, P, Nf, Tsym, rot, npts, G0, ldg, variant, rng_fast, nullptr, 0, stream);
}

extern "C" int pta_gwb_idft_rng_scaled(uint64_t seed, uint64_t r0, int R, int P, int Nf, const double *Tsym, const double *rot,
                                       int npts, double *G0, int64_t ldg, int variant, int rng_fast, const double *scale,
                                       int64_t ld_scale, void *stream) {
  PTA_REQUIRE(Tsym && rot && G0 && scale, PTA_E_ARG, "pta_gwb_idft_rng_scaled: NULL argument");
  PTA_REQUIRE(R > 0 && P > 0 && P < (1 << 24) && Nf >= 3 && npts > 0 && ldg >= npts, PTA_E_ARG,
              "pta_gwb_idft_rng_scaled: R=%d P=%d Nf=%d npts=%d", R, P, Nf, npts);
  PTA_REQUIRE(ld_scale >= Nf - 1, PTA_E_ARG, "pta_gwb_idft_rng_scaled: ld_scale=%lld < Nf - 1", (long long)ld_scale);
  int64_t M64 = (int64_t)R * P;
  PTA_REQUIRE(M64 < (1LL << 31), PTA_E_ARG, "pta_gwb_idft_rng_scaled: R*P too large");
  return idft_rng_launch(seed, r0, R, P, Nf, Tsym, rot, npts, G0, ldg, variant, rng_fast, scale, ld_scale, stream);
}

#define MIX_JT 64
template <int NTA>
__global__ __launch_bounds__(256) void k_gwb_mix_small(const double *__restrict__ Mchol, int P, const double *__restrict__ G0, int R,
                                                       int npts, int64_t ldg, double *__restrict__ G, int rpw) {
  extern __shared__ double Ms[];
  constexpr int MP = NTA * 16;
  const int KP = (P + 3) & ~3;
  const int t = threadIdx.x, l = t & 63, wv = t >> 6;
  for (int idx = t; idx < KP * MP; idx += 256) {
    const int b = idx / MP, a = idx - b * MP;
    Ms[idx] = (a < P && b < P) ? Mchol[(int64_t)a * P + b] : 0.0;
  }
  __syncthreads();
  const int col = l & 15, quad = l >> 4;
  const int jj = blockIdx.x * MIX_JT + wv * 16 + col;
  const bool jin = jj < npts;
  for (int rr = 0; rr < rpw; ++rr) {
    const int r = blockIdx.y * rpw + rr;
    if (r >= R) break;
    const double *__restrict__ g0 = G0 + (int64_t)r * P * ldg;
    pta_f64x4 acc[NTA];
#pragma unroll
    for (int i = 0; i < NTA; ++i) acc[i] = pta_f64x4{0.0, 0.0, 0.0, 0.0};
    double bv[NTA * 4];
#pragma unroll
    for (int s4 = 0; s4 < NTA * 4; ++s4) {
      const int b = 4 * s4 + quad;
      bv[s4] = (b < P && jin) ? g0[(int64_t)b * ldg + jj] : 0.0;
    }
#pragma unroll
    for (int s4 = 0; s4 < NTA * 4; ++s4) {
      if (4 * s4 < KP) {
        const int b = 4 * s4 + quad;
#pragma unroll
        for (int i = 0; i < NTA; ++i) acc[i] = pta_mfma_f64(Ms[b * MP + i * 16 + col], bv[s4], acc[i]);
      }
    }
    if (jin) {
#pragma unroll
      for (int i = 0; i < NTA; ++i)
#pragma unroll
        for (int rg = 0; rg < 4; ++rg) {
          const int a = i * 16 + pta_mfma_row(l, rg);
          if (a < P) G[((int64_t)r * P + a) * ldg + jj] = acc[i][rg];
        }
    }
  }
}

extern "C" int pta_gwb_mix(const double *Mchol, int P, const double *G0, int R, int npts, int64_t ldg, double *G, int variant,
                           void *stream) {
  PTA_REQUIRE(Mchol && G0 && G, PTA_E_ARG, "pta_gwb_mix: NULL argument");
  PTA_REQUIRE(P > 0 && R > 0 && npts > 0 && ldg >= npts, PTA_E_ARG, "pta_gwb_mix: P=%d R=%d npts=%d", P, R, npts);
  const int64_t sr = (int64_t)P * ldg;
  if (variant == 0 && P <= 80) {
    const int nta = (P + 15) / 16, kp = (P + 3) & ~3;
    const int rpw = 4;
    const size_t shmem = (size_t)kp * nta * 16 * sizeof(double);
    dim3 g(pta_cdiv(npts, MIX_JT), pta_cdiv(R, rpw));
    PTA_REQUIRE(g.y <= 65535u, PTA_E_ARG, "pta_gwb_mix: R=%d too large for one launch", R);
#define PTA_MIX(N) hipLaunchKernelGGL(k_gwb_mix_small<N>, g, dim3(256), shmem, pta_stream(stream), Mchol, P, G0, R, npts, ldg, G, rpw)
    switch (nta) {
      case 1: PTA_MIX(1); break;
      case 2: PTA_MIX(2); break;
      case 3: PTA_MIX(3); break;
      case 4: PTA_MIX(4); break;
      default: PTA_MIX(5); break;
    }
#undef PTA_MIX
    PTA_LAUNCH_CHECK();
    return PTA_OK;
  }
  for (int rb = 0; rb < R; rb += 32768) {
    int rc_ = (R - rb < 32768) ? (R - rb) : 32768;
    int rc = pta_dgemm_launch(0, P, npts, P, 1.0, Mchol, P, 1, G0 + rb * sr, ldg, 0.0, G + rb * sr, ldg, 0, rc_, 0, sr, sr,
                              variant == 2 ? 0 : 1, pta_stream(stream));
    if (rc != PTA_OK) return rc;
  }
  return PTA_OK;
}

__global__ void k_gwb_bracket(const double *__restrict__ ut, int npts, const double *__restrict__ toa_s, int N,
                              int32_t *__restrict__ jlo) {
  int i = blockIdx.x * blockDim.x + threadIdx.x;
  if (i >= N) return;
  double x = toa_s[i];
  double step = (ut[npts - 1] - ut[0]) / (double)(npts - 1);
  int j = (int)floor((x - ut[0]) / step);
  j = max(0, min(j, npts - 2));
  while (j > 0 && ut[j] > x) --j;
  while (j < npts - 2 && ut[j + 1] <= x) ++j;
  jlo[i] = j;
}

extern "C" int pta_gwb_bracket(const double *ut, int npts, const double *toa_s, int N, int32_t *jlo, void *stream) {
  PTA_REQUIRE(ut && toa_s && jlo, PTA_E_ARG, "pta_gwb_bracket: NULL argument");
  PTA_REQUIRE(npts >= 2 && N > 0, PTA_E_ARG, "pta_gwb_bracket: npts=%d N=%d", npts, N);
  hipLaunchKernelGGL(k_gwb_bracket, dim3(pta_cdiv(N, 256)), dim3(256), 0, pta_stream(stream), ut, npts, toa_s, N, jlo);
  PTA_LAUNCH_CHECK();
  return PTA_OK;
}

__global__ void k_gwb_weights(const double *__restrict__ ut, int npts, const double *__restrict__ toa_s,
                              const int32_t *__restrict__ jlo, int N, double *__restrict__ w) {
  int i = blockIdx.x * blockDim.x + threadIdx.x;
  if (i >= N) return;
  int j = max(0, min(jlo[i], npts - 2));
  w[i] = (toa_s[i] - ut[j]) / (ut[j + 1] - ut[j]);
}

extern "C" int pta_gwb_weights(const double *ut, int npts, const double *toa_s, const int32_t *jlo, int N, double *w, void *stream) {
  PTA_REQUIRE(ut && toa_s && jlo && w, PTA_E_ARG, "pta_gwb_weights: NULL argument");
  PTA_REQUIRE(npts >= 2 && N > 0, PTA_E_ARG, "pta_gwb_weights: npts=%d N=%d", npts, N);
  hipLaunchKernelGGL(k_gwb_weights, dim3(pta_cdiv(N, 256)), dim3(256), 0, pta_stream(stream), ut, npts, toa_s, jlo, N, w);
  PTA_LAUNCH_CHECK();
  return PTA_OK;
}

__device__ __forceinline__ double pta_lerp(const double *__restrict__ g, const double *__restrict__ ut, int j, double x) {
  double slope = (g[j + 1] - g[j]) / (ut[j + 1] - ut[j]);
  return slope * (x - ut[j]) + g[j];
}

__global__ void k_gwb_interp(const double *__restrict__ G, int64_t ldg, int P, const double *__restrict__ ut,
                             const double *__restrict__ toa_s, const int32_t *__restrict__ psr_of_toa,
                             const int32_t *__restrict__ jlo, int N, double scale, double *__restrict__ out, int64_t ld_out,
                             int accumulate) {
  int i = blockIdx.x * blockDim.x + threadIdx.x;
  int r = blockIdx.y;
  if (i >= N) return;
  const double *g = G + ((int64_t)r * P + psr_of_toa[i]) * ldg;
  double v = pta_lerp(g, ut, jlo[i], toa_s[i]);
  if (scale != 1.0) v = v * scale;
  int64_t o = (int64_t)r * ld_out + i;
  out[o] = accumulate ? out[o] + v : v;
}

extern "C" int pta_gwb_interp(const double *G, int64_t ldg, int P, int npts, const double *ut, const double *toa_s,
                              const int32_t *psr_of_toa, const int32_t *jlo, int N, int R, double scale, double *out,
                              int64_t ld_out, int accumulate, void *stream) {
  PTA_REQUIRE(G && ut && toa_s && psr_of_toa && jlo && out, PTA_E_ARG, "pta_gwb_interp: NULL argument");
  PTA_REQUIRE(P > 0 && npts >= 2 && N > 0 && R > 0 && R <= 65535 && ldg >= npts && ld_out >= N, PTA_E_ARG,
              "pta_gwb_interp: P=%d npts=%d N=%d R=%d", P, npts, N, R);
  hipLaunchKernelGGL(k_gwb_interp, dim3(pta_cdiv(N, 256), R), dim3(256), 0, pta_stream(stream), G, ldg, P, ut, toa_s,
                     psr_of_toa, jlo, N, scale, out, ld_out, accumulate);
  PTA_LAUNCH_CHECK();
  return PTA_OK;
}
```

pta_replicator_amd/engine.py:

```python
import ctypes

import numpy as np
import torch

from . import _cw, _hyper, _lib, device as dv
from . import deterministic as det
from . import red_noise as rn
from . import white_noise as wn
from ._position import ra_dec
from .constants import DAY_IN_SEC, YEAR_IN_SEC
from .engine_fstat import FStatisticMixin
from .engine_lnl import LikelihoodMixin
from .engine_os import OptimalStatisticMixin
from .engine_td import TimeDomainMixin

STREAM_GWB, STREAM_RN, STREAM_WN, STREAM_ECORR, STREAM_TD, STREAM_TDGW = 1, 2, 3, 4, 5, 6
STREAM_HYPER = 7
STREAM_CW = 8


def stream_id(kind, pulsar):
    return ((kind << 24) | (pulsar & 0xFFFFFF)) & 0xFFFFFFFF


class ReplicaEngine(TimeDomainMixin, OptimalStatisticMixin, LikelihoodMixin, FStatisticMixin):
    def __init__(self, psrs, seed=0):
        from .simulate import as_simulated
        self.psrs = [as_simulated(p) for p in psrs]
        self.P = len(self.psrs)
        self.seed = int(seed) & 0xFFFFFFFFFFFFFFFF
        self.names = [p.name for p in self.psrs]
        self.mjd = [np.asarray(p.toas.get_mjds().value, dtype=np.float64) for p in self.psrs]
        self.tdb_s = [np.array(p.toas.table["tdbld"], dtype="float64") * DAY_IN_SEC for p in self.psrs]
        self.sigma_s = [np.asarray(p.toas.get_errors().to("s").value, dtype=np.float64) for p in self.psrs]
        self.counts = np.array([len(m) for m in self.mjd])
        self.off = np.concatenate([[0], np.cumsum(self.counts)]).astype(np.int64)
        self.n_toa = int(self.off[-1])
        self._rn = None
        self._wn = None
        self._ec = None
        self._gw = None
        self._det = None
        self._delays = None
        self._cw = None
        self._prepared = False
        self.gwb_transform = "auto"
        self.rng_fast = 0
        self.synth_variant = 0
        self.czt_variant = 0
        self.mix_variant = 0
        self.idft_variant = 1
        self.gwb_mode = "fourier"
        self.wn_mode = "reference"
        self.workspace_bytes = 8 << 30

    def set_red_noise(self, log10_amplitude, spectral_index, components=30, libstempo_convention=False):
        self._rn = dict(A=list(np.broadcast_to(np.asarray(log10_amplitude, dtype=object), (self.P,))),
                        g=list(np.broadcast_to(np.asarray(spectral_index, dtype=object), (self.P,))),
                        components=int(components), libstempo=bool(libstempo_convention))
        self._prepared = False

    def set_white_noise(self, efac=1.0, log10_equad=None, flagid="f", flags=None, tnequad=False):
        self._wn = dict(efac=efac, log10_equad=log10_equad, flagid=flagid, flags=flags, tnequad=bool(tnequad))
        self._prepared = False

    def set_jitter(self, log10_ecorr, flagid="f", flags=None, coarsegrain=0.1):
        self._ec = dict(log10_ecorr=log10_ecorr, flagid=flagid, flags=flags, coarsegrain=float(coarsegrain))
        self._prepared = False

    def set_gwb(self, log10_amplitude, spectral_index, no_correlations=False, turnover=False,
                clm=(np.sqrt(4.0 * np.pi),), lmax=0, f0=1e-9, beta=1, power=1, userSpec=None, npts=600, howml=10):
        self._gw = dict(A=log10_amplitude, g=spectral_index, no_correlations=no_correlations, turnover=turnover, clm=clm,
                        lmax=lmax, f0=f0, beta=beta, power=power, userSpec=userSpec, npts=npts, howml=howml)
        self._prepared = False

    def add_cgw(self, **kw):
        self._det = (self._det or []) + [kw]
        self._prepared = False

    def set_cw(self, psrTerm=True, evolve=True, phase_approx=False, tref=0.0, pdist=1.0):
        self._cw = _cw.make_config(self.P, psrTerm, evolve, phase_approx, tref, pdist)
        self._cwt = None
        return self

    def add_delays(self, delays):
        d = np.concatenate([np.asarray(x, dtype=np.float64).ravel() for x in delays]) if isinstance(delays, (list, tuple)) \
            else np.asarray(delays, dtype=np.float64).ravel()
        if d.shape != (self.n_toa,):
            raise ValueError("delays must cover all {} TOAs, got {}".format(self.n_toa, d.shape))
        self._delays = d if getattr(self, "_delays", None) is None else self._delays + d
        self._prepared = False

    def _flag_array(self, a, flagid):
        return np.array([f[flagid] for f in self.psrs[a].toas.table["flags"].data])

    def prepare(self):
        dev = dv.require_gpu()
        self._ws = None
        self._hy = None
        self._td_prepared = False
        self._gw_grid_ready = False
        s = dv.stream_ptr()
        P, N = self.P, self.n_toa
        self.d_psr_of = dv.i32(np.repeat(np.arange(P), self.counts))
        self.d_idx_in = dv.i32(np.concatenate([np.arange(c) for c in self.counts]))
        self.d_toa_s = dv.f64(np.concatenate([m.astype(float) * 86400 for m in self.mjd]))
        self.plan = _lib.EnginePlan()
        pl = self.plan
        pl.n_toa, pl.n_psr = N, P
        pl.idx_in_psr = self.d_idx_in.data_ptr()

        pl.rn_k = 0
        if self._rn is not None:
            nm = self._rn["components"]
            K = 2 * nm
            self.K = K
            self.d_Ft = dv.zeros((K, N))
            amp = np.zeros((P, K))
            self.rn_freqs = []
            for a in range(P):
                lA, g = self._rn["A"][a], self._rn["g"][a]
                toas = self.tdb_s[a]
                Tspan = toas.max() - toas.min()
                f = 1.0 * np.arange(1, nm + 1) / Tspan
                self.rn_freqs.append(f)
                if lA is None or g is None:
                    continue
                freqs = np.repeat(f, 2)
                fyr = 1 / YEAR_IN_SEC
                prior = (10 ** lA) ** 2 * (freqs / fyr) ** (-g) / (12 * np.pi ** 2 * Tspan) * YEAR_IN_SEC ** 3
                amp[a] = np.sqrt(prior)
                t_d, f_d = dv.f64(toas), dv.f64(f)
                lib_conv = self._rn["libstempo"]
                t_ref = float(toas[0]) if lib_conv else 0.0
                _lib.call("pta_rn_basis", dv.ptr(t_d), len(toas), ctypes.c_double(t_ref), dv.ptr(f_d), None, nm,
                          1 if lib_conv else 0, ctypes.c_void_p(self.d_Ft.data_ptr() + 8 * int(self.off[a])), N, s)
            torch.cuda.current_stream().synchronize()
            self.rn_amp = amp
            self.d_amp = dv.f64(amp)
            pl.rn_k, pl.Ft, pl.ldf = K, self.d_Ft.data_ptr(), N

        pl.wn_a = pl.wn_b = pl.wn_c = None
        if self._wn is not None:
            c = self._wn
            wa, wb = np.zeros(N), np.zeros(N)
            self.efacvec, self.equadvec = [], []
            for a in range(P):
                n = self.counts[a]
                efac = self._pick(c["efac"], a)
                l10 = self._pick(c["log10_equad"], a)
                flags = self._pick_flags(c["flags"], a)
                equad = 10 ** np.asarray(l10, dtype=float) if l10 is not None else 0.0
                if flags is None:
                    if not np.isscalar(efac) or np.ndim(equad) != 0:
                        raise ValueError("ERROR: If flags is None, efac and equad must be a scalar")
                    ev, qv = np.ones(n) * efac, np.ones(n) * float(equad)
                else:
                    ev, qv = np.zeros(n), np.zeros(n)
                    if not (len(efac) == len(flags) and len(equad) == len(flags)):
                        raise ValueError("ERROR: flags must be same length as efac and log10_equad")
                    tf = self._flag_array(a, c["flagid"])
                    for ct, flag in enumerate(flags):
                        ev[flag == tf] = efac[ct]
                        qv[flag == tf] = equad[ct]
                self.efacvec.append(ev)
                self.equadvec.append(qv)
                sl = slice(self.off[a], self.off[a + 1])
                wa[sl] = ev * self.sigma_s[a]
                wb[sl] = qv if c["tnequad"] else ev * qv
            self.d_wn_a, self.d_wn_b, self.d_wn_c = dv.f64(wa), dv.f64(wb), dv.f64(np.hypot(wa, wb))
            pl.wn_a, pl.wn_b, pl.tnequad = self.d_wn_a.data_ptr(), self.d_wn_b.data_ptr(), int(c["tnequad"])

        pl.epoch_of = pl.ecorr_toa = None
        if self._ec is not None:
            c = self._ec
            ep_all, ec_all = np.zeros(N, dtype=np.int32), np.zeros(N)
            self.epoch_of, self.ecorrvec = [], []
            for a in range(P):
                l10 = self._pick(c["log10_ecorr"], a)
                flags = self._pick_flags(c["flags"], a)
                epoch_of, first = wn.epoch_map(self.mjd[a], c["coarsegrain"])
                ne = len(first)
                if l10 is None:
                    vec = np.zeros(ne)
                elif flags is None:
                    if not np.isscalar(l10):
                        raise ValueError("ERROR: If flags is None, jitter must be a scalar")
                    vec = np.ones(ne) * 10 ** l10
                else:
                    ecorr = 10 ** np.asarray(l10, dtype=float)
                    if len(ecorr) != len(flags):
                        raise ValueError("ERROR: flags must be same length as jitter")
                    aveflags = self._flag_array(a, c["flagid"])[first]
                    vec = np.zeros(ne)
                    for ct, flag in enumerate(flags):
                        vec[flag == aveflags] = ecorr[ct]
                self.epoch_of.append(epoch_of)
                self.ecorrvec.append(vec)
                sl = slice(self.off[a], self.off[a + 1])
                ep_all[sl] = epoch_of
                ec_all[sl] = vec[epoch_of]
            self.d_epoch_of, self.d_ecorr_toa = dv.i32(ep_all), dv.f64(ec_all)
            pl.epoch_of, pl.ecorr_toa = self.d_epoch_of.data_ptr(), self.d_ecorr_toa.data_ptr()

        T = _lib.ENGINE_TILE
        t_psr, t_start, t_count, t_ep0, t_epn = [], [], [], [], []
        for a in range(P):
            for s0 in range(0, int(self.counts[a]), T):
                cnt = min(T, int(self.counts[a]) - s0)
                t_psr.append(a); t_start.append(int(self.off[a]) + s0); t_count.append(cnt)
                if self._ec is not None:
                    e = self.epoch_of[a][s0:s0 + cnt]
                    p0, p1 = int(e.min()) >> 1, int(e.max()) >> 1
                    t_ep0.append(p0); t_epn.append(p1 - p0 + 1 if p1 - p0 + 1 <= _lib.ENGINE_EPMAX else 0)
                else:
                    t_ep0.append(0); t_epn.append(0)
        self.d_tiles = [dv.i32(x) for x in (t_psr, t_start, t_count, t_ep0, t_epn)]
        pl.n_tiles = len(t_psr)
        pl.tile_psr, pl.tile_start, pl.tile_count, pl.tile_ep0, pl.tile_epn = [x.data_ptr() for x in self.d_tiles]

        pl.gw_npts = 0
        if self._gw is not None:
            c = self._gw
            grid = rn.gwb_time_grid(self.psrs_ideal_view(), c["npts"], c["howml"])
            self.grid = grid
            npts, Nf = grid["npts"], grid["Nf"]
            ORF = rn.gwb_orf_device(self.psrs, c["no_correlations"], c["clm"], c["lmax"])
            self.ORF = ORF.clone()
            self.d_M = rn.cholesky_device(ORF)
            self.C = rn.gwb_spectrum(grid["f"], grid["dur"], c["howml"], c["A"], c["g"], c["turnover"], c["f0"], c["beta"],
                                     c["power"], c["userSpec"])
            self.ldt = rn.pad16(npts)
            self.d_T = dv.empty((2 * (Nf - 2), self.ldt))
            sqrtC = dv.f64(self.C ** 0.5)
            _lib.call("pta_gwb_twiddle", dv.ptr(sqrtC), Nf, npts, 10, ctypes.c_double(1.0 / grid["dt"]), dv.ptr(self.d_T), self.ldt, s)
            nrot = ctypes.c_int64(0)
            nsym = _lib.lib.pta_gwb_twiddle_sym_size(Nf, npts, self.idft_variant, ctypes.byref(nrot))
            self._idft_variant_built = self.idft_variant
            self.d_Tsym, self.d_rot = dv.empty((nsym,)), dv.empty((nrot.value,))
            _lib.call("pta_gwb_twiddle_sym", dv.ptr(sqrtC), Nf, npts, 10, ctypes.c_double(1.0 / grid["dt"]), dv.ptr(self.d_Tsym),
                      dv.ptr(self.d_rot), self.idft_variant, s)
            self.use_czt = bool(_lib.lib.pta_gwb_czt_fits(Nf, npts, 10)) and self.gwb_transform != "gemm"
            self.d_czt = None
            if self.use_czt:
                self.d_czt = [dv.empty((2 * 4096,)), dv.empty((2 * 4096,)), dv.empty((2 * 4096,)), dv.empty((2 * npts,))]
                _lib.call("pta_gwb_czt_setup", dv.ptr(sqrtC), Nf, npts, 10, ctypes.c_double(1.0 / grid["dt"]),
                          *[dv.ptr(x) for x in self.d_czt], s)
            self.d_ut = dv.f64(grid["ut"])
            self.d_jlo = dv.empty((N,), dtype=torch.int32)
            _lib.call("pta_gwb_bracket", dv.ptr(self.d_ut), npts, dv.ptr(self.d_toa_s), N, dv.ptr(self.d_jlo), s)
            torch.cuda.current_stream().synchronize()
            self.d_gw_w = dv.empty((N,))
            _lib.call("pta_gwb_weights", dv.ptr(self.d_ut), npts, dv.ptr(self.d_toa_s), dv.ptr(self.d_jlo), N, dv.ptr(self.d_gw_w), s)
            torch.cuda.current_stream().synchronize()
            pl.gw_npts, pl.gw_jlo, pl.gw_w = npts, self.d_jlo.data_ptr(), self.d_gw_w.data_ptr()

        pl.det = None
        extra = getattr(self, "_delays", None)
        if self._det or extra is not None:
            self.d_det = dv.zeros((N,)) if extra is None else dv.f64(extra)
            mjd_all = dv.f64(np.concatenate(self.mjd)) if self._det else None
            for kw in self._det or []:
                for a in range(P):
                    ra, dec = ra_dec(self.psrs[a])
                    par, _, _, _ = det.cgw_parameters(np.pi / 2 - dec, ra, **{k: v for k, v in kw.items() if k != "signal_name"})
                    par = np.ascontiguousarray(par)
                    o = int(self.off[a])
                    _lib.call("pta_cgw", ctypes.c_void_p(mjd_all.data_ptr() + 8 * o), len(self.mjd[a]), dv.hptr(par),
                              ctypes.c_void_p(self.d_det.data_ptr() + 8 * o), 1, s)
            if self._det:
                torch.cuda.current_stream().synchronize()
            pl.det = self.d_det.data_ptr()
        self._prepared = True
        if self._wn is not None and getattr(self, "td_warmup", True):
            _lib.call("pta_potrf_warmup", 2)
        return self

    def psrs_ideal_view(self):
        class _V:
            pass
        out = []
        for m in self.mjd:
            v = _V()
            v.toas = _V()
            v.toas.first_MJD = _V()
            v.toas.last_MJD = _V()
            v.toas.first_MJD.value = float(m.min())
            v.toas.last_MJD.value = float(m.max())
            out.append(v)
        return out

    def _pick(self, val, a):
        if val is None or np.isscalar(val):
            return val
        if len(val) != self.P:
            raise ValueError(f"expected a scalar or one entry per pulsar ({self.P}), got {len(val)}")
        return val[a]

    def _pick_flags(self, flags, a):
        if flags is None:
            return None
        if len(flags) != self.P:
            raise ValueError("flags must be a per-pulsar list of flag lists")
        return flags[a]

    def workspace(self, R):
        ws = getattr(self, "_ws", None)
        if ws is None or ws["R"] < R:
            ws = {"R": R}
            tb = _lib.EngineTables()
            if self.plan.rn_k:
                ws["coef"] = dv.empty((R, self.P, self.K))
                tb.rn_amp, tb.ws_coef = self.d_amp.data_ptr(), ws["coef"].data_ptr()
            if self.plan.gw_npts:
                ws["G0"] = dv.empty((R, self.P, self.plan.gw_npts))
                ws["G"] = dv.empty((R, self.P, self.plan.gw_npts))
                tb.Mchol, tb.ws_G0, tb.ws_G = self.d_M.data_ptr(), ws["G0"].data_ptr(), ws["G"].data_ptr()
                tb.gw_nf, tb.gw_i0 = self.grid["Nf"], 10
                if getattr(self, "d_czt", None) is not None:
                    tb.czt_pre, tb.czt_FB, tb.czt_tw, tb.czt_post = (x.data_ptr() for x in self.d_czt)
                tb.Tsym, tb.rot = self.d_Tsym.data_ptr(), self.d_rot.data_ptr()
                tb.idft_variant = self._idft_variant_built
            ws["tables"] = tb
            self._ws = ws
        ws["tables"].czt_variant, ws["tables"].mix_variant = int(self.czt_variant), int(self.mix_variant)
        if self.plan.gw_npts:
            if self.use_czt and getattr(self, "d_czt", None) is None:
                raise ValueError("use_czt was switched on after prepare(): the chirp-z tables were not built")
            ws["tables"].use_czt = 1 if self.use_czt else 0
        self.plan.rng_fast, self.plan.synth_variant = int(self.rng_fast), int(self.synth_variant)
        return ws

    def max_batch(self, hyper=False, cw=False):
        per_real = 8 * self.P * ((self.K if self.plan.rn_k else 0) + 2 * self.plan.gw_npts)
        if hyper and self.plan.gw_npts:
            per_real += 8 * self.grid["Nf"]
        cap = 65536
        if cw:
            S = 1 if cw is True else int(cw)
            if S < 1:
                raise ValueError(f"max_batch: cw must be True, False or a source count >= 1, got {cw!r}")
            per_real += 8 * (self.P * S * _lib.CW_ENGINE_NPAR + _cw.N_SRC * S + self.P)
            cap = min(cap, ((1 << 31) - 1) // (self.P * S))
        return int(max(1 if cap < 16 else 16, min(cap, self.workspace_bytes // max(per_real, 1))))

    def generate(self, R, r0=0, out=None, theta=None):
        hyper, cw = self._theta_parts(theta, R)
        return self._generate(R, r0, out, hyper, cw)

    def _theta_parts(self, theta, R, td=False, check_values=True):
        if theta is None:
            return None, {}
        rest, cw = _cw.split(theta)
        if td and (rest or not cw):
            raise ValueError("per-realisation theta is not supported in TD mode (the dense factors are built for one covariance; only "
                             "cw_* keys are): use generate(theta=...) or generate_sampled()")
        cw = _cw.check_theta(cw, R, self.P, self._cw, check_values)
        if cw and not rest:
            return None, cw
        return _hyper.check_theta(rest, R, self.P, self._gw, self._rn, self.gwb_mode, check_values), cw

    def _generate(self, R, r0, out, hyper, cw, mask_unconfigured=True):
        if not self._prepared:
            self.prepare()
        dev = None if hyper is None else self._theta_device(hyper, R, mask_unconfigured)
        if out is None:
            out = dv.empty((R, self.n_toa))
        step = self.max_batch(hyper=hyper is not None, cw=_cw.n_sources(cw))
        ws = self.workspace(min(R, step))
        hy = None if dev is None else self._hyper_tables()
        gw_theta = dev is not None and dev["gwb_log10_A"] is not None
        spec = None if dev is None else dev[_hyper.SPEC_KEY]
        if (gw_theta or spec is not None) and ("scale" not in ws or ws["scale"].shape[0] < ws["R"]):
            ws["scale"] = dv.empty((ws["R"], self.grid["Nf"]))
        grid_mode = self.gwb_mode == "grid" and self.plan.gw_npts
        if grid_mode:
            self._prepare_gw_grid_factor()
            self.tdgw_plan.rng_fast = int(self.rng_fast)
            self.tdgw_plan.z, self.tdgw_plan.ld_z, self.tdgw_plan.blk_zoff = None, 0, None
        s = dv.stream_ptr()
        P = self.P
        at = dv.row_ptr
        for lo in range(0, R, step):
            n = min(step, R - lo)
            optr = at(out, lo)
            h = None
            if dev is not None:
                h = _lib.EngineHyper()
                if self.plan.rn_k:
                    h.rn_f, h.rn_tspan = hy["rn_f"].data_ptr(), hy["rn_tspan"].data_ptr()
                    h.rn_log10_A, h.rn_gamma = at(dev["rn_log10_A"], lo), at(dev["rn_gamma"], lo)
                if gw_theta:
                    h.ld_gw_scale, h.ws_scale = self.grid["Nf"], ws["scale"].data_ptr()
                    h.gw_log10_A, h.gw_gamma = at(dev["gwb_log10_A"], lo), at(dev["gwb_gamma"], lo)
                    h.gw_f, h.gw_hcf0 = hy["gw_f"].data_ptr(), hy["gw_hcf0"].data_ptr()
                    c = self._gw
                    h.gw_turnover, h.gw_f0, h.gw_beta, h.gw_power = int(bool(c["turnover"])), float(c["f0"]), float(c["beta"]), float(c["power"])
                if spec is not None:
                    Nf, M = self.grid["Nf"], spec.shape[1]
                    _lib.call("pta_gwb_spectrum_scale_user", dv.ptr(hy["spec_seg"]), dv.ptr(hy["spec_dx"]), dv.ptr(hy["spec_dxp"]),
                              dv.ptr(hy["gw_hcf0"]), Nf, M, n, at(spec, lo), M, dv.ptr(ws["scale"]), Nf, s)
                    h.gw_scale, h.ld_gw_scale = ws["scale"].data_ptr(), Nf
            if not grid_mode:
                args = (self.seed, r0 + lo, n, optr, out.stride(0), s)
                if h is None:
                    _lib.call("pta_engine_generate", ctypes.byref(self._plan_for_mode()), ctypes.byref(ws["tables"]), *args)
                else:
                    _lib.call("pta_engine_generate_hyper", ctypes.byref(self._plan_for_mode()), ctypes.byref(ws["tables"]), ctypes.byref(h), *args)
                continue
            pl = _lib.EnginePlan.from_buffer_copy(self._plan_for_mode())
            if pl.rn_k:
                if h is not None and h.rn_log10_A:
                    _lib.call("pta_engine_rn_coef_hyper", self.seed, r0 + lo, n, P, self.K, h.rn_f, h.rn_tspan, h.rn_log10_A, h.rn_gamma,
                              dv.ptr(self.d_amp), dv.ptr(ws["coef"]), int(self.rng_fast), s)
                else:
                    _lib.call("pta_engine_rn_coef", self.seed, r0 + lo, n, P, self.K, dv.ptr(self.d_amp), dv.ptr(ws["coef"]), int(self.rng_fast), s)
                pl.rn_coef = ws["coef"].data_ptr()
            _lib.call("pta_td_trmm_rng", ctypes.byref(self.tdgw_plan), self.seed, r0 + lo, n * P, dv.ptr(ws["G0"]), pl.gw_npts, s)
            _lib.call("pta_gwb_mix", dv.ptr(self.d_M), P, dv.ptr(ws["G0"]), n, pl.gw_npts, pl.gw_npts, dv.ptr(ws["G"]), int(self.mix_variant), s)
            pl.gw_G = ws["G"].data_ptr()
            _lib.call("pta_engine_synth", ctypes.byref(pl), self.seed, r0 + lo, n, optr, out.stride(0), s)
        if self.plan.rn_k:
            self.plan.rn_coef = ws["coef"].data_ptr()
        if self.plan.gw_npts:
            self.plan.gw_G = ws["G"].data_ptr()
        if dev is not None:
            self._theta_keep = dev
        return self._cw_apply(cw, R, out) if cw else out

    def _theta_device(self, th, R, mask_unconfigured=True):
        dev = dict.fromkeys(_hyper.ALL_KEYS)
        if _hyper.SPEC_KEY in th:
            dev[_hyper.SPEC_KEY] = self._spec_theta_device(th)
        if any(k in th for k in _hyper.GWB_KEYS):
            for k, conf in (("gwb_log10_A", self._gw["A"]), ("gwb_gamma", self._gw["g"])):
                dev[k] = dv.as_f64(th[k]) if k in th else torch.full((R,), float(conf), dtype=torch.float64, device=dv.require_gpu())
        if any(k in th for k in _hyper.RN_KEYS) and self.plan.rn_k:
            self._rn_theta_device(th, R, dev, mask_unconfigured)
        return dev

    def _spec_theta_device(self, th):
        y = dv.as_f64(th[_hyper.SPEC_KEY])
        order = self._hyper_tables()["spec_order"]
        return y if order is None else y.index_select(1, order).contiguous()

    def _rn_theta_device(self, th, R, dev, mask_unconfigured=True):
        for k, c in zip(_hyper.RN_KEYS, _hyper.configured_rn(self._rn)):
            dev[k] = dv.as_f64(th[k]) if k in th else dv.f64(np.ascontiguousarray(np.broadcast_to(c, (R, self.P))))
        none = self._hyper_tables()["rn_none"]
        if mask_unconfigured and len(none):
            dev["rn_log10_A"] = dev["rn_log10_A"].clone()
            dev["rn_log10_A"][:, none] = float("nan")

    def _hyper_tables(self):
        if self._hy is not None:
            return self._hy
        hy = {}
        if self.plan.gw_npts:
            c = self._gw
            hy["gw_f"] = dv.f64(self.grid["f"])
            if c["userSpec"] is None:
                hy["gw_hcf0"] = dv.f64(rn.gwb_spectrum_hcf(self.grid["f"], c["A"], c["g"], c["turnover"], c["f0"], c["beta"], c["power"]))
            else:
                try:
                    order, xp = _hyper.spec_nodes(c["userSpec"])
                except ValueError:
                    order = None
                else:
                    seg, dx, dxp = _hyper.spec_tables(self.grid["f"], xp)
                    hy["spec_seg"], hy["spec_dx"], hy["spec_dxp"] = dv.i32(seg), dv.f64(dx), dv.f64(dxp)
                    hy["gw_hcf0"] = dv.f64(rn.gwb_spectrum_hcf(self.grid["f"], c["A"], c["g"], userSpec=np.asarray(c["userSpec"], dtype=np.float64)))
                    order = None if np.array_equal(order, np.arange(len(order))) else dv.i64(order)
                hy["spec_order"] = order
        if self.plan.rn_k:
            hy["rn_f"] = dv.f64(np.stack(self.rn_freqs))
            hy["rn_tspan"] = dv.f64(np.array([t.max() - t.min() for t in self.tdb_s]))
            hy["rn_none"] = dv.i64(np.flatnonzero(np.isnan(_hyper.configured_rn(self._rn)[0])))
        self._hy = hy
        return hy

    def _cw_tables(self):
        if self._cwt is None:
            phat = _cw.pulsar_vectors([ra_dec(p) for p in self.psrs])
            self._cwt = {"phat": dv.f64(phat), "pdist": dv.f64(self._cw["pdist"])}
        return self._cwt

    def _cw_apply(self, cw, R, out, accumulate=True):
        if _cw.is_catalog(cw):
            return self._cw_catalog_apply(cw, R, out, accumulate)
        if not self._prepared:
            self.prepare()
        P = self.P
        amp = _cw.amp_key(cw)
        cols = [dv.as_f64(cw[amp if c == "amp" else "cw_" + c]).reshape(R, 1) for c in _cw.COLUMNS]
        has_pd = _cw.PDIST_KEY in cw
        if has_pd:
            cols.append(dv.as_f64(cw[_cw.PDIST_KEY]).reshape(R, P))
        src = torch.cat(cols, dim=1).contiguous()
        conf, tb = self._cw, self._cw_tables()
        step = min(R, self.max_batch(hyper=True, cw=True))
        par = getattr(self, "_cw_par", None)
        if par is None or par.shape[0] < step:
            self._cw_par = None
            par = self._cw_par = dv.empty((step, P, _lib.CW_ENGINE_NPAR))
        c = _lib.CwEngine()
        c.n_psr, c.mode, c.psr_term, c.amp_is_h, c.has_pdist = P, _cw.mode(conf), int(conf["psrTerm"]), int(amp == "cw_log10_h"), int(has_pd)
        c.tref, c.phat, c.pdist, c.toa_s = conf["tref"], tb["phat"].data_ptr(), tb["pdist"].data_ptr(), self.d_toa_s.data_ptr()
        c.ld_src, c.par = src.stride(0), par.data_ptr()
        s = dv.stream_ptr()
        for lo in range(0, R, step):
            n = min(step, R - lo)
            c.src = src.data_ptr() + 8 * lo * src.stride(0)
            _lib.call("pta_engine_cw_params", ctypes.byref(c), n, s)
            _lib.call("pta_engine_cw_add", ctypes.byref(self.plan), ctypes.byref(c), n, ctypes.c_void_p(out.data_ptr() + 8 * lo * out.stride(0)),
                      out.stride(0), 1 if accumulate else 0, s)
        self._cw_keep = src
        return out

    def _cw_catalog_apply(self, cw, R, out, accumulate=True):
        if not self._prepared:
            self.prepare()
        dev = dv.require_gpu()
        P, S = self.P, _cw.n_sources(cw)
        amp = _cw.amp_key(cw)
        src = torch.stack([dv.as_f64(cw[amp if c == "amp" else "cw_" + c]).reshape(R, S) for c in _cw.COLUMNS], dim=2).contiguous()
        has_pd = _cw.PDIST_KEY in cw
        conf, tb = self._cw, self._cw_tables()
        pdist = dv.as_f64(cw[_cw.PDIST_KEY]).reshape(R, P) if has_pd else tb["pdist"]
        count = cw.get(_cw.COUNT_KEY)
        if count is not None:
            count = (count.to(device=dev, dtype=torch.int32) if hasattr(count, "data_ptr") else dv.i32(count)).reshape(R).contiguous()
        mode = _cw.mode(conf)
        npar = _lib.CW_CATALOG_NPAR[mode]
        step = min(R, self.max_batch(hyper=True, cw=S))
        par = getattr(self, "_cwc_par", None)
        if par is None or par.numel() < step * P * S * npar:
            self._cwc_par = None
            par = self._cwc_par = dv.empty((step * P * S * npar,))
        c = _lib.CwCatalogEngine()
        c.n_psr, c.n_src, c.mode, c.psr_term, c.amp_is_h, c.has_pdist = P, S, mode, int(conf["psrTerm"]), int(amp == "cw_log10_h"), int(has_pd)
        c.tref, c.phat, c.toa_s = conf["tref"], tb["phat"].data_ptr(), self.d_toa_s.data_ptr()
        c.ld_src, c.ld_pdist, c.par = src.stride(0), (pdist.stride(0) if has_pd else 0), par.data_ptr()
        s = dv.stream_ptr()
        for lo in range(0, R, step):
            n = min(step, R - lo)
            c.src = src.data_ptr() + 8 * lo * src.stride(0)
            c.pdist = pdist.data_ptr() + (8 * lo * pdist.stride(0) if has_pd else 0)
            c.count = None if count is None else count.data_ptr() + 4 * lo
            _lib.call("pta_engine_cw_catalog_params", ctypes.byref(c), n, s)
            _lib.call("pta_engine_cw_catalog_add", ctypes.byref(self.plan), ctypes.byref(c), n,
                      ctypes.c_void_p(out.data_ptr() + 8 * lo * out.stride(0)), out.stride(0), 1 if accumulate else 0, s)
        self._cw_keep = (src, pdist, count)
        return out

    def set_cw_prior(self, log10_mc=None, log10_fgw=None, log10_h=None, log10_dist=None, cos_gwtheta=None, gwphi=None, phase0=None,
                     psi=None, cos_inc=None, pdist=None, n_sources=None):
        self._cw_prior = _cw.make_prior(self.P, n_sources=n_sources, log10_mc=log10_mc, log10_fgw=log10_fgw, log10_h=log10_h, log10_dist=log10_dist,
                                        cos_gwtheta=cos_gwtheta, gwphi=gwphi, phase0=phase0, psi=psi, cos_inc=cos_inc, pdist=pdist)
        self._cw_prior_dev = None
        return self

    def set_hyper_prior(self, gwb_log10_A=None, gwb_gamma=None, rn_log10_A=None, rn_gamma=None, gwb_log10_hc=None):
        self._prior = _hyper.make_prior(self.P, _hyper._n_nodes(self._gw), gwb_log10_A=gwb_log10_A, gwb_gamma=gwb_gamma, rn_log10_A=rn_log10_A,
                                        rn_gamma=rn_gamma, gwb_log10_hc=gwb_log10_hc)
        self._prior_dev = None
        self._spec_prior_dev = None
        return self

    def generate_sampled(self, R, r0=0, out=None):
        prior, cw_prior = getattr(self, "_prior", None), getattr(self, "_cw_prior", None)
        if prior is None and cw_prior is None:
            raise ValueError("generate_sampled: no prior (set_hyper_prior / set_cw_prior first)")
        if prior is not None:
            _hyper.check_config(prior.keys(), self._gw, self._rn, self.gwb_mode)
        if cw_prior is not None and self._cw is None:
            raise ValueError("generate_sampled: no per-realisation CW configured (set_cw)")
        if not self._prepared:
            self.prepare()
        theta = self.sample_theta(R, r0)
        hyper, cw = self._theta_parts(theta, R, check_values=False)
        return self._generate(R, r0, out, hyper, cw, mask_unconfigured=False), theta

    def sample_theta(self, R, r0=0):
        prior, cw_prior = getattr(self, "_prior", None), getattr(self, "_cw_prior", None)
        if prior is None and cw_prior is None:
            raise ValueError("sample_theta: no prior (set_hyper_prior / set_cw_prior first)")
        if not self._prepared:
            self.prepare()
        theta = {}
        if cw_prior is not None:
            if self._cw_prior_dev is None:
                self._cw_prior_dev = [dv.f64(x) for x in _cw.prior_bounds(cw_prior, self.P)]
            S = cw_prior["n_sources"]
            table = catalog = None
            if S is None or "pdist" in cw_prior:
                table = self._uniform_table("pta_cw_uniform", self._cw_prior_dev, R, r0)
            if S is not None:
                catalog = dv.empty((R, S, _cw.N_SRC))
                d_lo, d_hi = self._cw_prior_dev
                _lib.call("pta_cw_catalog_uniform", self.seed, r0, R, S, dv.ptr(d_lo), dv.ptr(d_hi), dv.ptr(catalog), dv.stream_ptr())
            theta.update(_cw.labels(table, cw_prior, self.P, catalog))
        if prior is None:
            return theta
        box = _hyper.spec_bounds(prior)
        if box is not None:
            if getattr(self, "_spec_prior_dev", None) is None:
                self._spec_prior_dev = [dv.f64(x) for x in box]
            d_lo, d_hi = self._spec_prior_dev
            nodes = dv.empty((R, d_lo.shape[0]))
            _lib.call("pta_hyper_uniform_field", self.seed, r0, R, nodes.shape[1], _hyper.SPEC_FIELD, dv.ptr(d_lo), dv.ptr(d_hi), dv.ptr(nodes),
                      dv.stream_ptr())
            theta[_hyper.SPEC_KEY] = nodes
            if len(prior) == 1:
                return theta
        if self._prior_dev is None:
            self._prior_dev = [dv.f64(x) for x in _hyper.prior_bounds(prior, self.P)]
        table = self._uniform_table("pta_hyper_uniform", self._prior_dev, R, r0)
        cols = _hyper.columns(self.P)
        for k in _hyper.KEYS:
            if k in prior:
                c0, c1 = cols[k]
                theta[k] = table[:, c0].contiguous() if k in _hyper.GWB_KEYS else table[:, c0:c1].contiguous()
        if self.plan.rn_k:
            none = self._hyper_tables()["rn_none"]
            for k in _hyper.RN_KEYS:
                if k in theta and len(none):
                    theta[k][:, none] = float("nan")
        return theta

    def _uniform_table(self, kernel, bounds, R, r0):
        d_lo, d_hi = bounds
        table = dv.empty((R, d_lo.shape[0]))
        _lib.call(kernel, self.seed, r0, R, table.shape[1], dv.ptr(d_lo), dv.ptr(d_hi), dv.ptr(table), dv.stream_ptr())
        return table

    def _plan_for_mode(self):
        if self.wn_mode == "reference" or not self.plan.wn_a:
            return self.plan
        if self.wn_mode != "single":
            raise ValueError(f"wn_mode={self.wn_mode!r} must be 'reference' or 'single'")
        pl = _lib.EnginePlan.from_buffer_copy(self.plan)
        pl.wn_a = pl.wn_b = None
        pl.wn_c = self.d_wn_c.data_ptr()
        return pl

    def _require_reference_draws(self, what):
        if self.wn_mode != "reference" and self._wn is not None:
            raise ValueError(f"{what}() describes the reference-order draws; wn_mode={self.wn_mode!r} realisations are not replayable "
                             "(use dump_draws_wn_single / generate_per_signal, or set wn_mode = 'reference')")

    def dump_draws_wn_single(self, r):
        s = dv.stream_ptr()
        out = []
        for a in range(self.P):
            n = int(self.counts[a])
            z0, z1 = dv.empty((n,)), dv.empty((n,))
            _lib.call("pta_rng_fill_normal", self.seed, r, 1, stream_id(STREAM_WN, a), n, 0, dv.ptr(z0), dv.ptr(z1), n, int(self.rng_fast), s)
            idx = np.arange(n)
            z0, z1 = z0.cpu().numpy(), z1.cpu().numpy()
            out.append(np.where((idx >> 4) & 1, z1[idx & ~16], z0[idx & ~16]))
        return out

    def generate_per_signal(self, R, r0=0, theta=None):
        hyper, cw = self._theta_parts(theta, R)
        if not self._prepared:
            self.prepare()
        step = self.max_batch(hyper=theta is not None, cw=_cw.n_sources(cw))
        if R > step:
            raise ValueError(f"generate_per_signal: at most {step} realisations per call (one workspace batch)")
        total = self._generate(R, r0, None, hyper, cw)
        s = dv.stream_ptr()
        base = self._plan_for_mode()
        keep = (self.plan.rn_k, self.plan.gw_npts, base.wn_a, base.wn_b, self.plan.ecorr_toa, self.plan.epoch_of, self.plan.det, base.wn_c)
        out = {"total": total}

        def one(name, **on):
            pl = _lib.EnginePlan.from_buffer_copy(self.plan)
            pl.rn_k, pl.gw_npts, pl.wn_a, pl.wn_b, pl.ecorr_toa, pl.epoch_of, pl.det, pl.wn_c = (
                on.get("rn_k", 0), on.get("gw_npts", 0), on.get("wn_a"), on.get("wn_b"), on.get("ecorr_toa"),
                on.get("epoch_of"), on.get("det"), on.get("wn_c"))
            buf = dv.empty((R, self.n_toa))
            _lib.call("pta_engine_synth", ctypes.byref(pl), self.seed, r0, R, dv.ptr(buf), buf.stride(0), s)
            out[name] = buf
        if keep[0]:
            one("rn", rn_k=keep[0])
        if keep[1]:
            one("gwb", gw_npts=keep[1])
        if keep[2] or keep[7]:
            one("wn", wn_a=keep[2], wn_b=keep[3], wn_c=keep[7])
        if keep[4]:
            one("ecorr", ecorr_toa=keep[4], epoch_of=keep[5])
        if keep[6]:
            out["det"] = self.d_det.unsqueeze(0).expand(R, self.n_toa)
        if cw:
            out["cw"] = self._cw_apply(cw, R, dv.empty((R, self.n_toa)), accumulate=False)
        return out

    def stream_to_host(self, total, chunk=480, r0=0):
        if not self._prepared:
            self.prepare()
        chunk = int(min(chunk, total))
        dev = [dv.empty((chunk, self.n_toa)) for _ in range(2)]
        host = [torch.empty((chunk, self.n_toa), dtype=torch.float64).pin_memory() for _ in range(2)]
        copy_stream = torch.cuda.Stream()
        filled = [torch.cuda.Event(), torch.cuda.Event()]
        copied = [torch.cuda.Event(), torch.cuda.Event()]
        main = torch.cuda.current_stream()
        pending = []
        done = 0
        while done < total or pending:
            if done < total:
                b = (done // chunk) & 1
                n = min(chunk, total - done)
                if done >= 2 * chunk:
                    main.wait_event(copied[b])
                self.generate(n, r0=r0 + done, out=dev[b][:n])
                filled[b].record(main)
                with torch.cuda.stream(copy_stream):
                    copy_stream.wait_event(filled[b])
                    host[b][:n].copy_(dev[b][:n], non_blocking=True)
                    copied[b].record(copy_stream)
                pending.append((b, r0 + done, n))
                done += n
            if len(pending) == 2 or done >= total:
                b, first, n = pending.pop(0)
                copied[b].synchronize()
                yield first, host[b][:n].numpy()

    def dump_draws(self, r):
        self._require_reference_draws("dump_draws")
        if not self._prepared:
            self.prepare()
        s = dv.stream_ptr()
        d = {}
        if self.plan.gw_npts:
            Nf = self.grid["Nf"]
            buf = dv.empty((self.P, 2 * Nf))
            for a in range(self.P):
                _lib.call("pta_rng_fill_normal", self.seed, r, 1, stream_id(STREAM_GWB, a), Nf, 1,
                          ctypes.c_void_p(buf.data_ptr() + 16 * Nf * a), None, 2 * Nf, int(self.rng_fast), s)
            w = buf.cpu().numpy().reshape(self.P, Nf, 2)
            d["gwb"] = w[:, :, 0] + 1j * w[:, :, 1]
        if self.plan.rn_k:
            d["rn"] = []
            for a in range(self.P):
                buf = dv.empty((self.K,))
                _lib.call("pta_rng_fill_normal", self.seed, r, 1, stream_id(STREAM_RN, a), self.K // 2, 1, dv.ptr(buf), None, self.K, int(self.rng_fast), s)
                d["rn"].append(buf.cpu().numpy())
        if self.plan.wn_a:
            d["wn"] = []
            for a in range(self.P):
                n = int(self.counts[a])
                z1, z2 = dv.empty((n,)), dv.empty((n,))
                _lib.call("pta_rng_fill_normal", self.seed, r, 1, stream_id(STREAM_WN, a), n, 0, dv.ptr(z1), dv.ptr(z2), n, int(self.rng_fast), s)
                d["wn"].append((z1.cpu().numpy(), z2.cpu().numpy()))
        if self.plan.ecorr_toa:
            d["ecorr"] = []
            for a in range(self.P):
                ne = len(self.ecorrvec[a])
                npair = (ne + 1) // 2
                buf = dv.empty((2 * npair,))
                _lib.call("pta_rng_fill_normal", self.seed, r, 1, stream_id(STREAM_ECORR, a), npair, 1, dv.ptr(buf), None, 2 * npair, int(self.rng_fast), s)
                d["ecorr"].append(buf.cpu().numpy()[:ne])
        return d

    def replay(self, draws_list, per_signal=False):
        self._require_reference_draws("replay")
        if not self._prepared:
            self.prepare()
        s = dv.stream_ptr()
        R, P, N = len(draws_list), self.P, self.n_toa
        sig = {}
        pl = self.plan
        if pl.rn_k:
            coef = np.zeros((R, P, self.K))
            for r, d in enumerate(draws_list):
                for a in range(P):
                    coef[r, a] = self.rn_amp[a] * d["rn"][a]
            coef_d = dv.f64(coef)
            out = dv.zeros((R, N))
            for a in range(P):
                n = int(self.counts[a])
                _lib.call("pta_rn_synth", ctypes.c_void_p(self.d_Ft.data_ptr() + 8 * int(self.off[a])), N, n, self.K,
                          ctypes.c_void_p(coef_d.data_ptr() + 8 * a * self.K), P * self.K, R,
                          ctypes.c_void_p(out.data_ptr() + 8 * int(self.off[a])), N, 0, s)
            sig["rn"] = out
        if pl.gw_npts:
            Nf, npts = self.grid["Nf"], pl.gw_npts
            w = np.zeros((R, P, Nf, 2))
            for r, d in enumerate(draws_list):
                w[r, :, :, 0], w[r, :, :, 1] = d["gwb"].real, d["gwb"].imag
            w_d = dv.f64(w)
            G0, G = dv.empty((R * P, npts)), dv.empty((R * P, npts))
            _lib.call("pta_gwb_idft", dv.ptr(w_d), 2 * Nf, R * P, Nf, dv.ptr(self.d_T), self.ldt, npts, dv.ptr(G0), npts, 1, s)
            _lib.call("pta_gwb_mix", dv.ptr(self.d_M), P, dv.ptr(G0), R, npts, npts, dv.ptr(G), int(self.mix_variant), s)
            out = dv.empty((R, N))
            _lib.call("pta_gwb_interp", dv.ptr(G), npts, P, npts, dv.ptr(self.d_ut), dv.ptr(self.d_toa_s), dv.ptr(self.d_psr_of),
                      dv.ptr(self.d_jlo), N, R, ctypes.c_double(1.0), dv.ptr(out), N, 0, s)
            sig["gwb"] = out
            self._last_G = G
        if pl.wn_a:
            z1 = np.zeros((R, N)); z2 = np.zeros((R, N))
            for r, d in enumerate(draws_list):
                z1[r] = np.concatenate([x[0] for x in d["wn"]]); z2[r] = np.concatenate([x[1] for x in d["wn"]])
            sg, ef, eq = dv.f64(np.concatenate(self.sigma_s)), dv.f64(np.concatenate(self.efacvec)), dv.f64(np.concatenate(self.equadvec))
            z1_d, z2_d = dv.f64(z1), dv.f64(z2)
            out = dv.empty((R, N))
            _lib.call("pta_wn", dv.ptr(sg), dv.ptr(ef), dv.ptr(eq), N, int(self._wn["tnequad"]), dv.ptr(z1_d), dv.ptr(z2_d), N, R,
                      dv.ptr(out), N, 0, s)
            sig["wn"] = out
        if pl.ecorr_toa:
            out = dv.zeros((R, N))
            keep = []
            for a in range(P):
                ne, n = len(self.ecorrvec[a]), int(self.counts[a])
                z = np.zeros((R, ne))
                for r, d in enumerate(draws_list):
                    z[r] = d["ecorr"][a]
                z_d, ep_d, ec_d = dv.f64(z), dv.i32(self.epoch_of[a]), dv.f64(self.ecorrvec[a])
                keep += [z_d, ep_d, ec_d]
                _lib.call("pta_ecorr", dv.ptr(ep_d), dv.ptr(ec_d), n, ne, dv.ptr(z_d), ne, R,
                          ctypes.c_void_p(out.data_ptr() + 8 * int(self.off[a])), N, 0, s)
            torch.cuda.current_stream().synchronize()
            del keep
            sig["ecorr"] = out
        total = dv.zeros((R, N))
        for k in ("rn", "gwb", "wn", "ecorr"):
            if k in sig:
                total += sig[k]
        if pl.det:
            sig["det"] = self.d_det.unsqueeze(0).expand(R, N)
            total += self.d_det
        torch.cuda.current_stream().synchronize()
        if per_signal:
            sig["total"] = total
            return sig
        return total

    def inject(self, r, signal_name="engine_realisation"):
        from ._compat import TimeDelta, u
        row = self.generate(1, r0=r)[0].cpu().numpy()
        for a, psr in enumerate(self.psrs):
            dt = row[self.off[a]:self.off[a + 1]] * u.s
            psr.update_added_signals("{}_{}".format(psr.name, signal_name), {"seed": self.seed, "realisation": int(r)}, dt)
            psr.toas.adjust_TOAs(TimeDelta(dt.to("day")))
            psr.update_residuals()
        return row

    def prepare_timing_projection(self, model="spin"):
        from .simulate import timing_design_matrix
        dv.require_gpu()
        Mt = Qt = None
        for a in range(self.P):
            M, names = timing_design_matrix(self.mjd[a] * 86400.0, model=model)
            w = 1.0 / self.sigma_s[a] ** 2
            w = w / w.mean()
            A = M.T @ (M * w[:, None])
            Q = np.linalg.solve(A, M.T * w[None, :])
            if Mt is None:
                m = M.shape[1]
                Mt, Qt = np.zeros((m, self.n_toa)), np.zeros((m, self.n_toa))
            Mt[:, self.off[a]:self.off[a + 1]] = M.T
            Qt[:, self.off[a]:self.off[a + 1]] = Q
        self._tm = dict(model=model, m=Mt.shape[0], names=names, Mt=dv.f64(Mt), Qt=dv.f64(Qt), off=dv.i32(self.off), Mt_host=Mt, Qt_host=Qt)
        return self

    def project_timing_model(self, rows, model="spin"):
        if getattr(self, "_tm", None) is None or self._tm["model"] != model:
            self.prepare_timing_projection(model)
        tm = self._tm
        assert rows.dim() == 2 and rows.shape[1] == self.n_toa and rows.stride(1) == 1
        _lib.call("pta_tm_project", dv.ptr(tm["Qt"]), dv.ptr(tm["Mt"]), self.n_toa, tm["m"], dv.ptr(tm["off"]), self.P,
                  ctypes.c_void_p(rows.data_ptr()), rows.stride(0), int(rows.shape[0]), dv.stream_ptr())
        return rows

    def to_enterprise(self, rows, subtract_mean=True, timing_model="spin", fitted=False):
        from .simulate import ArrayEnterprisePulsar
        from ._position import ra_dec
        if fitted:
            dev = rows.detach().clone() if hasattr(rows, "detach") else dv.f64(np.atleast_2d(np.asarray(rows)))
            if dev.dim() == 1:
                dev = dev[None, :].contiguous()
            rows = self.project_timing_model(dev, timing_model)
            subtract_mean = False
        arr = rows.detach().cpu().numpy() if hasattr(rows, "detach") else np.asarray(rows)
        if arr.ndim == 1:
            arr = arr[None, :]
        meta = []
        for a, psr in enumerate(self.psrs):
            toas = psr.toas
            flags = list(toas.table["flags"].data)
            freq = getattr(toas, "freqs_mhz", None)
            if freq is None:
                try:
                    freq = np.asarray(toas.get_freqs().to("MHz").value, dtype=np.float64)
                except AttributeError:
                    freq = 1440.0
            meta.append((flags, np.asarray(freq, dtype=np.float64) * np.ones(int(self.counts[a])), ra_dec(psr, default=(0.0, 0.0))))
        out = []
        for row in arr:
            psrs = []
            for a, psr in enumerate(self.psrs):
                x = row[self.off[a]:self.off[a + 1]]
                res = x
                if subtract_mean:
                    w = 1.0 / self.sigma_s[a] ** 2
                    res = x - np.sum(x * w) / np.sum(w)
                flags, freq, (ra, dec) = meta[a]
                mjd = self.mjd[a].astype(np.longdouble) + (x / 86400.0).astype(np.longdouble)
                psrs.append(ArrayEnterprisePulsar(psr.name, np.asarray(mjd, dtype=np.float64), res, self.sigma_s[a] * 1e6, freq, flags, ra, dec,
                                                  timing_model=timing_model))
            out.append(psrs)
        return out

    def write_tim_ensemble(self, rows, outdir, r0=0):
        import os
        from .simulate import ArrayTOAs, minimal_par, write_tim
        arr = rows.detach().cpu().numpy() if hasattr(rows, "detach") else np.asarray(rows)
        if arr.ndim == 1:
            arr = arr[None, :]
        for psr in self.psrs:
            if not isinstance(psr.toas, ArrayTOAs):
                raise NotImplementedError("write_tim_ensemble needs array-backed pulsars (PINT-backed: use inject() + write_partim)")
        os.makedirs(os.path.join(outdir, "par"), exist_ok=True)
        for psr in self.psrs:
            with open(os.path.join(outdir, "par", f"{psr.name}.par"), "w") as fh:
                fh.write(psr.par_text if getattr(psr, "par_text", None) else minimal_par(psr.name, psr.loc))
        paths = []
        for k, row in enumerate(arr):
            d = os.path.join(outdir, f"real_{r0 + k:06d}")
            os.makedirs(d, exist_ok=True)
            for a, psr in enumerate(self.psrs):
                mjd = psr.toas.mjd0_ld + (row[self.off[a]:self.off[a + 1]] / 86400.0).astype(np.longdouble)
                path = os.path.join(d, f"{psr.name}.tim")
                write_tim(path, psr.name, mjd, psr.toas.errors_us, psr.toas.freqs_mhz, psr.toas.flags)
                paths.append(path)
        return paths

    def split(self, arr):
        return [arr[..., self.off[a]:self.off[a + 1]] for a in range(self.P)]
```

Baseline: 222,000 realizations/s.

## Fuse the ORF Cholesky mix into the chirp-z kernel and skip triangle zeros

Adds an optional fused path in which the last chirp-z block of each realisation, found with a per-realisation atomic arrival counter, loads the Cholesky factor into the FFT planes in LDS and applies the MFMA mix there. This removes the separate mix launch and the second pass over G0. It also adds a triangular mode that skips MFMA k-steps above the diagonal when the factor is lower-triangular, and this applies to the standalone mix kernel too. The fused path is off by default (fuse_mix=0), so the default change is the triangle skip plus some reworked load addressing in the shared mix routine.

```diff
diff --git a/include/pta_replicator_amd.h b/include/pta_replicator_amd.h
--- a/include/pta_replicator_amd.h
+++ b/include/pta_replicator_amd.h
@@ -117,6 +117,15 @@
                                 const double *log10_hc, int64_t ld_hc, double *scale, int64_t ld_scale, void *stream);
 
 int pta_gwb_mix(const double *Mchol, int P, const double *G0, int R, int npts, int64_t ldg, double *G, int variant, void *stream);
+int pta_gwb_mix_ksteps(const double *Mchol, int P, const double *G0, int R, int npts, int64_t ldg, double *G, int variant, int ksteps,
+                       void *stream);
+int pta_gwb_czt_mix(uint64_t seed, uint64_t r0, const double *w, int64_t ldw, int R, int P, int Nf, int npts, int i0,
+                    const double *pre, const double *FB, const double *tw, const double *post, double *G0, int64_t ldg,
+                    int variant, int rng_fast, const double *Mchol, double *G, int32_t *cnt, int ksteps, void *stream);
+int pta_gwb_czt_mix_scaled(uint64_t seed, uint64_t r0, const double *w, int64_t ldw, int R, int P, int Nf, int npts, int i0,
+                           const double *pre, const double *FB, const double *tw, const double *post, double *G0, int64_t ldg,
+                           int variant, int rng_fast, const double *scale, int64_t ld_scale, const double *Mchol, double *G,
+                           int32_t *cnt, int ksteps, void *stream);
 
 int pta_gwb_bracket(const double *ut, int npts, const double *toa_s, int N, int32_t *jlo, void *stream);
 
@@ -184,6 +193,9 @@
   double *ws_G;
   int32_t idft_variant;
   int32_t mix_variant;
+  int32_t *ws_mix_count;
+  int32_t fuse_mix;
+  int32_t mix_ksteps;
 } pta_engine_tables;
 
 int pta_engine_generate(const pta_engine_plan *plan_host, const pta_engine_tables *tables_host, uint64_t seed, uint64_t r0, int R,
diff --git a/pta_replicator_amd/_lib.py b/pta_replicator_amd/_lib.py
--- a/pta_replicator_amd/_lib.py
+++ b/pta_replicator_amd/_lib.py
@@ -38,6 +38,7 @@
         ("rn_amp", _P), ("Mchol", _P), ("gw_nf", c_int32), ("gw_i0", c_int32), ("use_czt", c_int32), ("czt_variant", c_int32),
         ("czt_pre", _P), ("czt_FB", _P), ("czt_tw", _P), ("czt_post", _P), ("Tsym", _P), ("rot", _P),
         ("ws_coef", _P), ("ws_G0", _P), ("ws_G", _P), ("idft_variant", c_int32), ("mix_variant", c_int32),
+        ("ws_mix_count", _P), ("fuse_mix", c_int32), ("mix_ksteps", c_int32),
     ]
 
 
@@ -114,6 +115,11 @@
     "pta_gwb_idft_rng_scaled": (c_int, [c_uint64, c_uint64, c_int, c_int, c_int, _P, _P, c_int, _P, c_int64, c_int, c_int, _P, c_int64, _P]),
     "pta_gwb_spectrum_scale": (c_int, [_P, _P, c_int, c_int, _P, _P, c_int, c_double, c_double, c_double, _P, c_int64, _P]),
     "pta_gwb_mix": (c_int, [_P, c_int, _P, c_int, c_int, c_int64, _P, c_int, _P]),
+    "pta_gwb_mix_ksteps": (c_int, [_P, c_int, _P, c_int, c_int, c_int64, _P, c_int, c_int, _P]),
+    "pta_gwb_czt_mix": (c_int, [c_uint64, c_uint64, _P, c_int64, c_int, c_int, c_int, c_int, c_int, _P, _P, _P, _P, _P, c_int64, c_int, c_int,
+                                _P, _P, _P, c_int, _P]),
+    "pta_gwb_czt_mix_scaled": (c_int, [c_uint64, c_uint64, _P, c_int64, c_int, c_int, c_int, c_int, c_int, _P, _P, _P, _P, _P, c_int64, c_int,
+                                       c_int, _P, c_int64, _P, _P, _P, c_int, _P]),
     "pta_gwb_bracket": (c_int, [_P, c_int, _P, c_int, _P, _P]),
     "pta_gwb_weights": (c_int, [_P, c_int, _P, _P, c_int, _P, _P]),
     "pta_gwb_interp": (c_int, [_P, c_int64, c_int, c_int, _P, _P, _P, _P, c_int, c_int, c_double, _P, c_int64, c_int, _P]),
diff --git a/pta_replicator_amd/_mix.py b/pta_replicator_amd/_mix.py
--- /dev/null
+++ b/pta_replicator_amd/_mix.py
@@ -0,0 +1,22 @@
+import numpy as np
+
+TILE = 16
+KSTEP = 4
+TILE_KSTEPS = TILE // KSTEP
+PMAX = 80
+
+
+def ksteps_for(M):
+    M = np.asarray(M)
+    if M.ndim != 2 or M.shape[0] != M.shape[1]:
+        raise ValueError(f"expected a square factor, got shape {M.shape}")
+    return 0 if np.any(np.triu(M, 1) != 0) else TILE_KSTEPS
+
+
+def tile_ksteps(P, ksteps):
+    if not 1 <= P <= PMAX:
+        raise ValueError(f"the LDS-resident mix takes 1 <= P <= {PMAX}, got {P}")
+    if ksteps not in (0, TILE_KSTEPS):
+        raise ValueError(f"ksteps is 0 or {TILE_KSTEPS}, got {ksteps}")
+    kp = (P + KSTEP - 1) // KSTEP
+    return [kp if ksteps == 0 else min(kp, ksteps * (i + 1)) for i in range((P + TILE - 1) // TILE)]
diff --git a/pta_replicator_amd/csrc/pta_czt_kernels.hip b/pta_replicator_amd/csrc/pta_czt_kernels.hip
--- a/pta_replicator_amd/csrc/pta_czt_kernels.hip
+++ b/pta_replicator_amd/csrc/pta_czt_kernels.hip
@@ -1,5 +1,7 @@
 #include "pta_common.h"
 #include "pta_fft.h"
+#include "pta_gwb_mix.h"
+#include <type_traits>
 
 __global__ __launch_bounds__(PTA_FFT_THREADS) void k_czt_setup(const double *__restrict__ sqrtC, int Nf, int npts, int i0,
                                                                double inv_dt, double *__restrict__ pre,
@@ -80,17 +82,22 @@
 #define PTA_CZT_FUSE_DEFAULT (15 + 16 + 64)
 static int czt_last2(int npts, int i0) { return i0 - 2 + npts < 1024 ? 1 : 0; }
 
-template <bool RNG, bool FAST, int FUSE, bool SCALED>
+template <bool RNG, bool FAST, int FUSE, bool SCALED, bool MIX>
 __global__ __launch_bounds__(PTA_FFT_THREADS, 4) void k_gwb_czt(uint64_t seed, uint64_t r0, const double *__restrict__ w, int64_t ldw,
                                                                   int M, int P, int Nf, int npts, int i0,
                                                                   const double *__restrict__ pre, const double *__restrict__ FB,
                                                                   const double *__restrict__ tw, const double *__restrict__ post,
                                                                   double *__restrict__ G0, int64_t ldg,
-                                                                  const double *__restrict__ scale, int64_t ld_scale, int last2) {
+                                                                  const double *__restrict__ scale, int64_t ld_scale, int last2,
+                                                                  const double *__restrict__ Mchol, double *__restrict__ G,
+                                                                  int *__restrict__ cnt, int ksteps) {
   static_assert(!(FUSE & 16) || (FUSE & 6) == 6, "bit 4 carries the twiddles from the register-fed first butterfly to the storing last one");
   static_assert(!(FUSE & 32) || (FUSE & 8), "bit 5 tabulates the squared twiddles of bit 3");
   static_assert(!(FUSE & 64) || (FUSE & 2), "bit 6 prunes the storing last butterfly");
-  __shared__ double re[PTA_FFT_PLANE], im[PTA_FFT_PLANE];
+  static_assert(!MIX || (FUSE & 2), "the mix follows the storing last butterfly");
+  static_assert(2 * PTA_FFT_PLANE > PTA_MIX_PMAX * PTA_MIX_PMAX, "Mchol and the last-arriver word fit the planes");
+  __shared__ double planes[2 * PTA_FFT_PLANE];
+  double *const re = planes, *const im = planes + PTA_FFT_PLANE;
   constexpr bool TAB = (FUSE & 32) != 0;
   __shared__ pta_cplx tw8[7][8];
   __shared__ pta_cplx tw64[3][64];
@@ -256,7 +263,12 @@
       const int jj = o + 512 * q - (i0 - 1);
       if (jj >= 0 && jj < npts) {
         const pta_cplx pp = post2[jj];
-        G0[(int64_t)row * ldg + jj] = v[q].re * pp.re - v[q].im * pp.im;
+        const double x = v[q].re * pp.re - v[q].im * pp.im;
+        if (MIX)
+          __hip_atomic_store((__attribute__((address_space(1))) double *)(G0 + (int64_t)row * ldg + jj), x, __ATOMIC_RELAXED,
+                             __HIP_MEMORY_SCOPE_AGENT);
+        else
+          G0[(int64_t)row * ldg + jj] = x;
       }
     };
     if ((FUSE & 64) && last2) {
@@ -276,24 +288,84 @@
       G0[(int64_t)row * ldg + jj] = re[p] * post2[jj].re - im[p] * post2[jj].im;
     }
   }
-}
-
-extern "C" int pta_gwb_czt(uint64_t seed, uint64_t r0, const double *w, int64_t ldw, int R, int P, int Nf, int npts, int i0,
-                           const double *pre, const double *FB, const double *tw, const double *post, double *G0, int64_t ldg,
-                           int variant, int rng_fast, void *stream) {
-  PTA_REQUIRE(pre && FB && tw && post && G0, PTA_E_ARG, "pta_gwb_czt: NULL argument");
-  PTA_REQUIRE(R > 0 && P > 0 && P < (1 << 24) && npts > 0 && ldg >= npts, PTA_E_ARG, "pta_gwb_czt: R=%d P=%d npts=%d", R, P, npts);
-  PTA_REQUIRE(czt_fits(Nf, npts, i0), PTA_E_ARG, "pta_gwb_czt: Nf=%d npts=%d does not fit one 4096-point convolution", Nf, npts);
-  PTA_REQUIRE(!w || ldw == 0 || ldw >= 2 * (int64_t)Nf, PTA_E_ARG, "pta_gwb_czt: ldw too small");
+  if (MIX) {
+    const int r = row / P;
+    int *const arrived = reinterpret_cast<int *>(planes + 2 * PTA_FFT_PLANE - 1);
+    asm volatile("s_waitcnt vmcnt(0)" ::: "memory");
+    __syncthreads();
+    if (tid == 0) {
+      const int before = __hip_atomic_fetch_add((__attribute__((address_space(1))) int *)(cnt + r), 1, __ATOMIC_RELAXED,
+                                                __HIP_MEMORY_SCOPE_AGENT);
+      if (before == P - 1) {
+        __builtin_amdgcn_fence(__ATOMIC_ACQUIRE, "agent");
+        asm volatile("s_waitcnt vmcnt(0)" ::: "memory");
+      }
+      *arrived = before;
+    }
+    __syncthreads();
+    if (*arrived != P - 1) return;
+    const double *g0 = G0 + (int64_t)r * P * ldg;
+    double *g = G + (int64_t)r * P * ldg;
+    const int l = tid & 63, j0 = (tid >> 6) * 16 + (l & 15);
+    auto mix = [&](auto nta) {
+      constexpr int NTA = decltype(nta)::value;
+      pta_mix_stage<NTA>(planes, Mchol, P, tid, PTA_FFT_THREADS);
+      __syncthreads();
+      for (int jb = 0; jb < npts; jb += 16 * (PTA_FFT_THREADS / 64)) pta_mix_wave<NTA, true>(planes, P, ksteps, g0, npts, ldg, g, jb + j0, l);
+    };
+    switch ((P + 15) / 16) {
+      case 1: mix(std::integral_constant<int, 1>{}); break;
+      case 2: mix(std::integral_constant<int, 2>{}); break;
+      case 3: mix(std::integral_constant<int, 3>{}); break;
+      case 4: mix(std::integral_constant<int, 4>{}); break;
+      default: mix(std::integral_constant<int, 5>{}); break;
+    }
+    if (tid == 0) __hip_atomic_store((__attribute__((address_space(1))) int *)(cnt + r), 0, __ATOMIC_RELAXED, __HIP_MEMORY_SCOPE_AGENT);
+  }
+}
+
+struct czt_mix_args {
+  const double *Mchol;
+  double *G;
+  int *cnt;
+  int ksteps;
+};
+
+static int czt_mix_check(const char *fn, const czt_mix_args &mx, int P, int variant) {
+  PTA_REQUIRE(mx.Mchol && mx.G && mx.cnt, PTA_E_ARG, "%s: NULL argument", fn);
+  PTA_REQUIRE(variant == 0, PTA_E_ARG, "%s: variant %d (the mix is fused into the default kernel, variant 0, only)", fn, variant);
+  PTA_REQUIRE(P <= PTA_MIX_PMAX, PTA_E_ARG, "%s: P=%d exceeds the %d pulsars of the LDS-resident mix", fn, P, PTA_MIX_PMAX);
+  PTA_REQUIRE(mx.ksteps == 0 || mx.ksteps == PTA_MIX_TILE_KSTEPS, PTA_E_ARG, "%s: ksteps=%d (0 or %d)", fn, mx.ksteps, PTA_MIX_TILE_KSTEPS);
+  return PTA_OK;
+}
+
+static int czt_launch(const char *fn, uint64_t seed, uint64_t r0, const double *w, int64_t ldw, int R, int P, int Nf, int npts, int i0,
+                      const double *pre, const double *FB, const double *tw, const double *post, double *G0, int64_t ldg, int variant,
+                      int rng_fast, const czt_mix_args &mx, void *stream) {
+  PTA_REQUIRE(pre && FB && tw && post && G0, PTA_E_ARG, "%s: NULL argument", fn);
+  PTA_REQUIRE(R > 0 && P > 0 && P < (1 << 24) && npts > 0 && ldg >= npts, PTA_E_ARG, "%s: R=%d P=%d npts=%d", fn, R, P, npts);
+  PTA_REQUIRE(czt_fits(Nf, npts, i0), PTA_E_ARG, "%s: Nf=%d npts=%d does not fit one 4096-point convolution", fn, Nf, npts);
+  PTA_REQUIRE(!w || ldw == 0 || ldw >= 2 * (int64_t)Nf, PTA_E_ARG, "%s: ldw too small", fn);
   int64_t M64 = (int64_t)R * P;
-  PTA_REQUIRE(M64 < (1LL << 31), PTA_E_ARG, "pta_gwb_czt: R*P too large");
+  PTA_REQUIRE(M64 < (1LL << 31), PTA_E_ARG, "%s: R*P too large", fn);
   const int M = (int)M64;
   const int fastm = rng_fast ? 1 : 0;
   const int fuse = variant == 0 ? PTA_CZT_FUSE_DEFAULT : (variant == 1 ? 0 : variant - 10);
   const int last2 = czt_last2(npts, i0);
-#define PTA_CZT_X(RNGV, FASTV, FUSEV)                                                                                                  \
-  hipLaunchKernelGGL((k_gwb_czt<RNGV, FASTV, FUSEV, false>), dim3(M), dim3(PTA_FFT_THREADS), 0, pta_stream(stream), seed, r0, w, ldw, \
-                     M, P, Nf, npts, i0, pre, FB, tw, post, G0, ldg, nullptr, 0, last2)
+#define PTA_CZT_XM(RNGV, FASTV, FUSEV, MIXV)                                                                                          \
+  hipLaunchKernelGGL((k_gwb_czt<RNGV, FASTV, FUSEV, false, MIXV>), dim3(M), dim3(PTA_FFT_THREADS), 0, pta_stream(stream), seed, r0, w, \
+                     ldw, M, P, Nf, npts, i0, pre, FB, tw, post, G0, ldg, nullptr, 0, last2, mx.Mchol, mx.G, mx.cnt, mx.ksteps)
+#define PTA_CZT_X(RNGV, FASTV, FUSEV) PTA_CZT_XM(RNGV, FASTV, FUSEV, false)
+  if (mx.Mchol) {
+    if (w)
+      PTA_CZT_XM(false, false, PTA_CZT_FUSE_DEFAULT, true);
+    else if (fastm)
+      PTA_CZT_XM(true, true, PTA_CZT_FUSE_DEFAULT, true);
+    else
+      PTA_CZT_XM(true, false, PTA_CZT_FUSE_DEFAULT, true);
+    PTA_LAUNCH_CHECK();
+    return PTA_OK;
+  }
 #define PTA_CZT_XF(FUSEV)              \
   if (w)                               \
     PTA_CZT_X(false, false, FUSEV);    \
@@ -313,33 +385,54 @@
     case 3: PTA_CZT_XF(3); break;
     case 7: PTA_CZT_XF(7); break;
     case 8: PTA_CZT_XF(8); break;
-    default: pta_set_error("pta_gwb_czt: unknown variant %d", variant); return PTA_E_ARG;
+    default: pta_set_error("%s: unknown variant %d", fn, variant); return PTA_E_ARG;
   }
 #undef PTA_CZT_XF
 #undef PTA_CZT_X
+#undef PTA_CZT_XM
   PTA_LAUNCH_CHECK();
   return PTA_OK;
 }
 
-extern "C" int pta_gwb_czt_scaled(uint64_t seed, uint64_t r0, const double *w, int64_t ldw, int R, int P, int Nf, int npts, int i0,
-                                  const double *pre, const double *FB, const double *tw, const double *post, double *G0, int64_t ldg,
-                                  int variant, int rng_fast, const double *scale, int64_t ld_scale, void *stream) {
-  PTA_REQUIRE(pre && FB && tw && post && G0 && scale, PTA_E_ARG, "pta_gwb_czt_scaled: NULL argument");
-  PTA_REQUIRE(!w, PTA_E_ARG, "pta_gwb_czt_scaled: draws are generated on chip (w must be NULL)");
-  (void)ldw;
-  PTA_REQUIRE(R > 0 && P > 0 && P < (1 << 24) && npts > 0 && ldg >= npts, PTA_E_ARG, "pta_gwb_czt_scaled: R=%d P=%d npts=%d", R, P,
-              npts);
-  PTA_REQUIRE(czt_fits(Nf, npts, i0), PTA_E_ARG, "pta_gwb_czt_scaled: Nf=%d npts=%d does not fit one 4096-point convolution", Nf,
-              npts);
-  PTA_REQUIRE(ld_scale >= Nf - 1, PTA_E_ARG, "pta_gwb_czt_scaled: ld_scale=%lld < Nf - 1", (long long)ld_scale);
+extern "C" int pta_gwb_czt(uint64_t seed, uint64_t r0, const double *w, int64_t ldw, int R, int P, int Nf, int npts, int i0,
+                           const double *pre, const double *FB, const double *tw, const double *post, double *G0, int64_t ldg,
+                           int variant, int rng_fast, void *stream) {
+  return czt_launch("pta_gwb_czt", seed, r0, w, ldw, R, P, Nf, npts, i0, pre, FB, tw, post, G0, ldg, variant, rng_fast, czt_mix_args{},
+                    stream);
+}
+
+extern "C" int pta_gwb_czt_mix(uint64_t seed, uint64_t r0, const double *w, int64_t ldw, int R, int P, int Nf, int npts, int i0,
+                               const double *pre, const double *FB, const double *tw, const double *post, double *G0, int64_t ldg,
+                               int variant, int rng_fast, const double *Mchol, double *G, int32_t *cnt, int ksteps, void *stream) {
+  const czt_mix_args mx{Mchol, G, cnt, ksteps};
+  const int rc = czt_mix_check("pta_gwb_czt_mix", mx, P, variant);
+  if (rc != PTA_OK) return rc;
+  return czt_launch("pta_gwb_czt_mix", seed, r0, w, ldw, R, P, Nf, npts, i0, pre, FB, tw, post, G0, ldg, variant, rng_fast, mx, stream);
+}
+
+static int czt_scaled_launch(const char *fn, uint64_t seed, uint64_t r0, const double *w, int R, int P, int Nf, int npts, int i0,
+                             const double *pre, const double *FB, const double *tw, const double *post, double *G0, int64_t ldg,
+                             int variant, int rng_fast, const double *scale, int64_t ld_scale, const czt_mix_args &mx, void *stream) {
+  PTA_REQUIRE(pre && FB && tw && post && G0 && scale, PTA_E_ARG, "%s: NULL argument", fn);
+  PTA_REQUIRE(!w, PTA_E_ARG, "%s: draws are generated on chip (w must be NULL)", fn);
+  PTA_REQUIRE(R > 0 && P > 0 && P < (1 << 24) && npts > 0 && ldg >= npts, PTA_E_ARG, "%s: R=%d P=%d npts=%d", fn, R, P, npts);
+  PTA_REQUIRE(czt_fits(Nf, npts, i0), PTA_E_ARG, "%s: Nf=%d npts=%d does not fit one 4096-point convolution", fn, Nf, npts);
+  PTA_REQUIRE(ld_scale >= Nf - 1, PTA_E_ARG, "%s: ld_scale=%lld < Nf - 1", fn, (long long)ld_scale);
   int64_t M64 = (int64_t)R * P;
-  PTA_REQUIRE(M64 < (1LL << 31), PTA_E_ARG, "pta_gwb_czt_scaled: R*P too large");
+  PTA_REQUIRE(M64 < (1LL << 31), PTA_E_ARG, "%s: R*P too large", fn);
   const int M = (int)M64;
-  PTA_REQUIRE(variant == 0 || variant == 1, PTA_E_ARG, "pta_gwb_czt_scaled: variant %d (0 or 1)", variant);
-#define PTA_CZT_S(FASTV, FUSEV)                                                                                                     \
-  hipLaunchKernelGGL((k_gwb_czt<true, FASTV, FUSEV, true>), dim3(M), dim3(PTA_FFT_THREADS), 0, pta_stream(stream), seed, r0, nullptr, \
-                     0, M, P, Nf, npts, i0, pre, FB, tw, post, G0, ldg, scale, ld_scale, czt_last2(npts, i0))
-  if (variant == 0) {
+  PTA_REQUIRE(variant == 0 || variant == 1, PTA_E_ARG, "%s: variant %d (0 or 1)", fn, variant);
+#define PTA_CZT_SM(FASTV, FUSEV, MIXV)                                                                                                 \
+  hipLaunchKernelGGL((k_gwb_czt<true, FASTV, FUSEV, true, MIXV>), dim3(M), dim3(PTA_FFT_THREADS), 0, pta_stream(stream), seed, r0,      \
+                     nullptr, 0, M, P, Nf, npts, i0, pre, FB, tw, post, G0, ldg, scale, ld_scale, czt_last2(npts, i0), mx.Mchol, mx.G, \
+                     mx.cnt, mx.ksteps)
+#define PTA_CZT_S(FASTV, FUSEV) PTA_CZT_SM(FASTV, FUSEV, false)
+  if (mx.Mchol) {
+    if (rng_fast)
+      PTA_CZT_SM(true, PTA_CZT_FUSE_DEFAULT, true);
+    else
+      PTA_CZT_SM(false, PTA_CZT_FUSE_DEFAULT, true);
+  } else if (variant == 0) {
     if (rng_fast)
       PTA_CZT_S(true, PTA_CZT_FUSE_DEFAULT);
     else
@@ -351,6 +444,27 @@
       PTA_CZT_S(false, 0);
   }
 #undef PTA_CZT_S
+#undef PTA_CZT_SM
   PTA_LAUNCH_CHECK();
   return PTA_OK;
 }
+
+extern "C" int pta_gwb_czt_scaled(uint64_t seed, uint64_t r0, const double *w, int64_t ldw, int R, int P, int Nf, int npts, int i0,
+                                  const double *pre, const double *FB, const double *tw, const double *post, double *G0, int64_t ldg,
+                                  int variant, int rng_fast, const double *scale, int64_t ld_scale, void *stream) {
+  (void)ldw;
+  return czt_scaled_launch("pta_gwb_czt_scaled", seed, r0, w, R, P, Nf, npts, i0, pre, FB, tw, post, G0, ldg, variant, rng_fast, scale,
+                           ld_scale, czt_mix_args{}, stream);
+}
+
+extern "C" int pta_gwb_czt_mix_scaled(uint64_t seed, uint64_t r0, const double *w, int64_t ldw, int R, int P, int Nf, int npts, int i0,
+                                      const double *pre, const double *FB, const double *tw, const double *post, double *G0,
+                                      int64_t ldg, int variant, int rng_fast, const double *scale, int64_t ld_scale,
+                                      const double *Mchol, double *G, int32_t *cnt, int ksteps, void *stream) {
+  (void)ldw;
+  const czt_mix_args mx{Mchol, G, cnt, ksteps};
+  const int rc = czt_mix_check("pta_gwb_czt_mix_scaled", mx, P, variant);
+  if (rc != PTA_OK) return rc;
+  return czt_scaled_launch("pta_gwb_czt_mix_scaled", seed, r0, w, R, P, Nf, npts, i0, pre, FB, tw, post, G0, ldg, variant, rng_fast,
+                           scale, ld_scale, mx, stream);
+}
diff --git a/pta_replicator_amd/csrc/pta_engine_kernels.hip b/pta_replicator_amd/csrc/pta_engine_kernels.hip
--- a/pta_replicator_amd/csrc/pta_engine_kernels.hip
+++ b/pta_replicator_amd/csrc/pta_engine_kernels.hip
@@ -419,8 +419,15 @@
                            int variant, int rng_fast, void *stream);
 extern "C" int pta_gwb_idft_rng(uint64_t seed, uint64_t r0, int R, int P, int Nf, const double *Tsym, const double *rot, int npts,
                                 double *G0, int64_t ldg, int variant, int rng_fast, void *stream);
-extern "C" int pta_gwb_mix(const double *Mchol, int P, const double *G0, int R, int npts, int64_t ldg, double *G, int variant,
-                           void *stream);
+extern "C" int pta_gwb_mix_ksteps(const double *Mchol, int P, const double *G0, int R, int npts, int64_t ldg, double *G, int variant,
+                                  int ksteps, void *stream);
+extern "C" int pta_gwb_czt_mix(uint64_t seed, uint64_t r0, const double *w, int64_t ldw, int R, int P, int Nf, int npts, int i0,
+                               const double *pre, const double *FB, const double *tw, const double *post, double *G0, int64_t ldg,
+                               int variant, int rng_fast, const double *Mchol, double *G, int32_t *cnt, int ksteps, void *stream);
+extern "C" int pta_gwb_czt_mix_scaled(uint64_t seed, uint64_t r0, const double *w, int64_t ldw, int R, int P, int Nf, int npts, int i0,
+                                      const double *pre, const double *FB, const double *tw, const double *post, double *G0,
+                                      int64_t ldg, int variant, int rng_fast, const double *scale, int64_t ld_scale,
+                                      const double *Mchol, double *G, int32_t *cnt, int ksteps, void *stream);
 
 static int engine_generate(const char *fn, const pta_engine_plan *plan_host, const pta_engine_tables *tables_host,
                            const pta_engine_hyper *hyper, uint64_t seed, uint64_t r0, int R, double *out, int64_t ld_out, void *stream) {
@@ -452,7 +459,17 @@
       if (rc != PTA_OK) return rc;
       scale = h.ws_scale;
     }
-    if (tb.use_czt) {
+    const bool fused = tb.use_czt && tb.fuse_mix && tb.czt_variant == 0 && tb.mix_variant == 0 && p.n_psr <= 80;
+    if (fused) {
+      PTA_REQUIRE(tb.czt_pre && tb.czt_FB && tb.czt_tw && tb.czt_post, PTA_E_ARG, "%s: chirp-z tables missing", fn);
+      PTA_REQUIRE(tb.ws_mix_count, PTA_E_ARG, "%s: fuse_mix without the arrival counters (ws_mix_count)", fn);
+      rc = scale ? pta_gwb_czt_mix_scaled(seed, r0, nullptr, 0, R, p.n_psr, tb.gw_nf, p.gw_npts, tb.gw_i0, tb.czt_pre, tb.czt_FB,
+                                          tb.czt_tw, tb.czt_post, tb.ws_G0, p.gw_npts, 0, p.rng_fast, scale, h.ld_gw_scale, tb.Mchol,
+                                          tb.ws_G, tb.ws_mix_count, tb.mix_ksteps, stream)
+                 : pta_gwb_czt_mix(seed, r0, nullptr, 0, R, p.n_psr, tb.gw_nf, p.gw_npts, tb.gw_i0, tb.czt_pre, tb.czt_FB, tb.czt_tw,
+                                   tb.czt_post, tb.ws_G0, p.gw_npts, 0, p.rng_fast, tb.Mchol, tb.ws_G, tb.ws_mix_count, tb.mix_ksteps,
+                                   stream);
+    } else if (tb.use_czt) {
       PTA_REQUIRE(tb.czt_pre && tb.czt_FB && tb.czt_tw && tb.czt_post, PTA_E_ARG, "%s: chirp-z tables missing", fn);
       rc = scale ? pta_gwb_czt_scaled(seed, r0, nullptr, 0, R, p.n_psr, tb.gw_nf, p.gw_npts, tb.gw_i0, tb.czt_pre, tb.czt_FB, tb.czt_tw,
                                       tb.czt_post, tb.ws_G0, p.gw_npts, tb.czt_variant, p.rng_fast, scale, h.ld_gw_scale, stream)
@@ -466,7 +483,7 @@
                                     p.rng_fast, stream);
     }
     if (rc != PTA_OK) return rc;
-    rc = pta_gwb_mix(tb.Mchol, p.n_psr, tb.ws_G0, R, p.gw_npts, p.gw_npts, tb.ws_G, tb.mix_variant, stream);
+    if (!fused) rc = pta_gwb_mix_ksteps(tb.Mchol, p.n_psr, tb.ws_G0, R, p.gw_npts, p.gw_npts, tb.ws_G, tb.mix_variant, tb.mix_ksteps, stream);
     if (rc != PTA_OK) return rc;
     p.gw_G = tb.ws_G;
   }
diff --git a/pta_replicator_amd/csrc/pta_gwb_kernels.hip b/pta_replicator_amd/csrc/pta_gwb_kernels.hip
--- a/pta_replicator_amd/csrc/pta_gwb_kernels.hip
+++ b/pta_replicator_amd/csrc/pta_gwb_kernels.hip
@@ -1,5 +1,6 @@
 #include "pta_common.h"
 #include "pta_mfma.h"
+#include "pta_gwb_mix.h"
 #include "pta_rng.h"
 
 
@@ -266,64 +267,33 @@
 #define MIX_JT 64
 template <int NTA>
 __global__ __launch_bounds__(256) void k_gwb_mix_small(const double *__restrict__ Mchol, int P, const double *__restrict__ G0, int R,
-                                                       int npts, int64_t ldg, double *__restrict__ G, int rpw) {
+                                                       int npts, int64_t ldg, double *__restrict__ G, int rpw, int ksteps) {
   extern __shared__ double Ms[];
-  constexpr int MP = NTA * 16;
-  const int KP = (P + 3) & ~3;
   const int t = threadIdx.x, l = t & 63, wv = t >> 6;
-  for (int idx = t; idx < KP * MP; idx += 256) {
-    const int b = idx / MP, a = idx - b * MP;
-    Ms[idx] = (a < P && b < P) ? Mchol[(int64_t)a * P + b] : 0.0;
-  }
+  pta_mix_stage<NTA>(Ms, Mchol, P, t, 256);
   __syncthreads();
-  const int col = l & 15, quad = l >> 4;
-  const int jj = blockIdx.x * MIX_JT + wv * 16 + col;
-  const bool jin = jj < npts;
+  const int jj = blockIdx.x * MIX_JT + wv * 16 + (l & 15);
   for (int rr = 0; rr < rpw; ++rr) {
     const int r = blockIdx.y * rpw + rr;
     if (r >= R) break;
-    const double *__restrict__ g0 = G0 + (int64_t)r * P * ldg;
-    pta_f64x4 acc[NTA];
-#pragma unroll
-    for (int i = 0; i < NTA; ++i) acc[i] = pta_f64x4{0.0, 0.0, 0.0, 0.0};
-    double bv[NTA * 4];
-#pragma unroll
-    for (int s4 = 0; s4 < NTA * 4; ++s4) {
-      const int b = 4 * s4 + quad;
-      bv[s4] = (b < P && jin) ? g0[(int64_t)b * ldg + jj] : 0.0;
-    }
-#pragma unroll
-    for (int s4 = 0; s4 < NTA * 4; ++s4) {
-      if (4 * s4 < KP) {
-        const int b = 4 * s4 + quad;
-#pragma unroll
-        for (int i = 0; i < NTA; ++i) acc[i] = pta_mfma_f64(Ms[b * MP + i * 16 + col], bv[s4], acc[i]);
-      }
-    }
-    if (jin) {
-#pragma unroll
-      for (int i = 0; i < NTA; ++i)
-#pragma unroll
-        for (int rg = 0; rg < 4; ++rg) {
-          const int a = i * 16 + pta_mfma_row(l, rg);
-          if (a < P) G[((int64_t)r * P + a) * ldg + jj] = acc[i][rg];
-        }
-    }
-  }
-}
-
-extern "C" int pta_gwb_mix(const double *Mchol, int P, const double *G0, int R, int npts, int64_t ldg, double *G, int variant,
-                           void *stream) {
+    pta_mix_wave<NTA, false>(Ms, P, ksteps, G0 + (int64_t)r * P * ldg, npts, ldg, G + (int64_t)r * P * ldg, jj, l);
+  }
+}
+
+extern "C" int pta_gwb_mix_ksteps(const double *Mchol, int P, const double *G0, int R, int npts, int64_t ldg, double *G, int variant,
+                                  int ksteps, void *stream) {
   PTA_REQUIRE(Mchol && G0 && G, PTA_E_ARG, "pta_gwb_mix: NULL argument");
   PTA_REQUIRE(P > 0 && R > 0 && npts > 0 && ldg >= npts, PTA_E_ARG, "pta_gwb_mix: P=%d R=%d npts=%d", P, R, npts);
+  PTA_REQUIRE(ksteps == 0 || ksteps == PTA_MIX_TILE_KSTEPS, PTA_E_ARG, "pta_gwb_mix_ksteps: ksteps=%d (0 or %d)", ksteps, PTA_MIX_TILE_KSTEPS);
   const int64_t sr = (int64_t)P * ldg;
-  if (variant == 0 && P <= 80) {
+  if (variant == 0 && P <= PTA_MIX_PMAX) {
     const int nta = (P + 15) / 16, kp = (P + 3) & ~3;
     const int rpw = 4;
     const size_t shmem = (size_t)kp * nta * 16 * sizeof(double);
     dim3 g(pta_cdiv(npts, MIX_JT), pta_cdiv(R, rpw));
     PTA_REQUIRE(g.y <= 65535u, PTA_E_ARG, "pta_gwb_mix: R=%d too large for one launch", R);
-#define PTA_MIX(N) hipLaunchKernelGGL(k_gwb_mix_small<N>, g, dim3(256), shmem, pta_stream(stream), Mchol, P, G0, R, npts, ldg, G, rpw)
+#define PTA_MIX(N) \
+  hipLaunchKernelGGL(k_gwb_mix_small<N>, g, dim3(256), shmem, pta_stream(stream), Mchol, P, G0, R, npts, ldg, G, rpw, ksteps)
     switch (nta) {
       case 1: PTA_MIX(1); break;
       case 2: PTA_MIX(2); break;
@@ -342,6 +312,11 @@
     if (rc != PTA_OK) return rc;
   }
   return PTA_OK;
+}
+
+extern "C" int pta_gwb_mix(const double *Mchol, int P, const double *G0, int R, int npts, int64_t ldg, double *G, int variant,
+                           void *stream) {
+  return pta_gwb_mix_ksteps(Mchol, P, G0, R, npts, ldg, G, variant, 0, stream);
 }
 
 __global__ void k_gwb_bracket(const double *__restrict__ ut, int npts, const double *__restrict__ toa_s, int N,
diff --git a/pta_replicator_amd/csrc/pta_gwb_mix.h b/pta_replicator_amd/csrc/pta_gwb_mix.h
--- /dev/null
+++ b/pta_replicator_amd/csrc/pta_gwb_mix.h
@@ -0,0 +1,67 @@
+#pragma once
+#include "pta_common.h"
+#include "pta_mfma.h"
+
+#define PTA_MIX_PMAX 80
+
+template <int NTA>
+__device__ __forceinline__ void pta_mix_stage(double *Ms, const double *__restrict__ Mchol, int P, int t, int nthreads) {
+  constexpr int MP = NTA * 16;
+  const int KP = (P + 3) & ~3;
+  for (int idx = t; idx < KP * MP; idx += nthreads) {
+    const int b = idx / MP, a = idx - b * MP;
+    Ms[idx] = (a < P && b < P) ? Mchol[(int64_t)a * P + b] : 0.0;
+  }
+}
+
+#define PTA_MIX_TILE_KSTEPS 4
+template <int NTA, bool AGENT, bool TRI>
+__device__ __forceinline__ void pta_mix_wave(const double *Ms, int P, const double *g0, int npts, int64_t ldg, double *g, int jj, int l) {
+  constexpr int MP = NTA * 16;
+  const int KP = (P + 3) & ~3;
+  asm volatile("" : "+v"(l));
+  const int col = l & 15, quad = l >> 4;
+  const bool jin = jj < npts;
+  pta_f64x4 acc[NTA];
+#pragma unroll
+  for (int i = 0; i < NTA; ++i) acc[i] = pta_f64x4{0.0, 0.0, 0.0, 0.0};
+  double bv[NTA * 4];
+  const double *gj = g0 + (jin ? jj : npts - 1);
+#pragma unroll
+  for (int s4 = 0; s4 < NTA * 4; ++s4) {
+    const int b = 4 * s4 + quad;
+    const double *gp = gj + (int64_t)min(b, P - 1) * ldg;
+    const double x = AGENT ? __hip_atomic_load((const __attribute__((address_space(1))) double *)gp, __ATOMIC_RELAXED,
+                                               __HIP_MEMORY_SCOPE_AGENT)
+                           : *gp;
+    bv[s4] = (b < P && jin) ? x : 0.0;
+  }
+  const double *mp = Ms + quad * MP + col;
+#pragma unroll
+  for (int s4 = 0; s4 < NTA * 4; ++s4) {
+    if (4 * s4 < KP) {
+#pragma unroll
+      for (int i = TRI ? s4 / PTA_MIX_TILE_KSTEPS : 0; i < NTA; ++i) acc[i] = pta_mfma_f64(mp[s4 * 4 * MP + i * 16], bv[s4], acc[i]);
+      __builtin_amdgcn_sched_barrier(0);
+    }
+  }
+  if (jin) {
+    double *gq = g + (int64_t)quad * ldg + jj;
+#pragma unroll
+    for (int i = 0; i < NTA; ++i)
+#pragma unroll
+      for (int rg = 0; rg < 4; ++rg) {
+        if (i * 16 + 4 * rg + quad < P) *gq = acc[i][rg];
+        gq += 4 * ldg;
+      }
+  }
+}
+
+template <int NTA, bool AGENT>
+__device__ __forceinline__ void pta_mix_wave(const double *Ms, int P, int ksteps, const double *g0, int npts, int64_t ldg, double *g, int jj,
+                                             int l) {
+  if (ksteps)
+    pta_mix_wave<NTA, AGENT, true>(Ms, P, g0, npts, ldg, g, jj, l);
+  else
+    pta_mix_wave<NTA, AGENT, false>(Ms, P, g0, npts, ldg, g, jj, l);
+}
diff --git a/pta_replicator_amd/engine.py b/pta_replicator_amd/engine.py
--- a/pta_replicator_amd/engine.py
+++ b/pta_replicator_amd/engine.py
@@ -3,7 +3,7 @@
 import numpy as np
 import torch
 
-from . import _cw, _hyper, _lib, device as dv
+from . import _cw, _hyper, _lib, _mix, device as dv
 from . import deterministic as det
 from . import red_noise as rn
 from . import white_noise as wn
@@ -49,6 +49,7 @@
         self.synth_variant = 0
         self.czt_variant = 0
         self.mix_variant = 0
+        self.fuse_mix = 0
         self.idft_variant = 1
         self.gwb_mode = "fourier"
         self.wn_mode = "reference"
@@ -228,6 +229,7 @@
             ORF = rn.gwb_orf_device(self.psrs, c["no_correlations"], c["clm"], c["lmax"])
             self.ORF = ORF.clone()
             self.d_M = rn.cholesky_device(ORF)
+            self.mix_ksteps = _mix.ksteps_for(self.d_M.cpu().numpy())
             self.C = rn.gwb_spectrum(grid["f"], grid["dur"], c["howml"], c["A"], c["g"], c["turnover"], c["f0"], c["beta"],
                                      c["power"], c["userSpec"])
             self.ldt = rn.pad16(npts)
@@ -316,6 +318,8 @@
                 ws["G0"] = dv.empty((R, self.P, self.plan.gw_npts))
                 ws["G"] = dv.empty((R, self.P, self.plan.gw_npts))
                 tb.Mchol, tb.ws_G0, tb.ws_G = self.d_M.data_ptr(), ws["G0"].data_ptr(), ws["G"].data_ptr()
+                ws["mix_count"] = torch.zeros((R,), dtype=torch.int32, device=ws["G0"].device)
+                tb.ws_mix_count, tb.mix_ksteps = ws["mix_count"].data_ptr(), int(self.mix_ksteps)
                 tb.gw_nf, tb.gw_i0 = self.grid["Nf"], 10
                 if getattr(self, "d_czt", None) is not None:
                     tb.czt_pre, tb.czt_FB, tb.czt_tw, tb.czt_post = (x.data_ptr() for x in self.d_czt)
@@ -324,6 +328,7 @@
             ws["tables"] = tb
             self._ws = ws
         ws["tables"].czt_variant, ws["tables"].mix_variant = int(self.czt_variant), int(self.mix_variant)
+        ws["tables"].fuse_mix = int(self.fuse_mix)
         if self.plan.gw_npts:
             if self.use_czt and getattr(self, "d_czt", None) is None:
                 raise ValueError("use_czt was switched on after prepare(): the chirp-z tables were not built")
```

Measured after the change: 221,200 realizations/s. No clear change (-0.4%).
